# bioinfo-pf-curie/mpiBWA

Hardware: AMD Instinct MI355X
Metric: Mreads/s (whole node) 2x150 bp PE vs GRCh38-size reference; SAM bit-match (higher is better)
Workload: dtype int32

## Files before the change

include/mpibwa_amd.h:

```cpp
#ifndef MPIBWA_AMD_H
#define MPIBWA_AMD_H

#include <stdint.h>
#include <stddef.h>
#include <stdio.h>

#ifdef __cplusplus
extern "C" {
#endif

#define MEM_F_PE             0x2
#define MEM_F_NOPAIRING      0x4
#define MEM_F_ALL            0x8
#define MEM_F_NO_MULTI       0x10
#define MEM_F_NO_RESCUE      0x20
#define MEM_F_REF_HDR        0x100
#define MEM_F_SOFTCLIP       0x200
#define MEM_F_SMARTPE        0x400
#define MEM_F_PRIMARY5       0x800
#define MEM_F_KEEP_SUPP_MAPQ 0x1000

typedef uint64_t bwtint_t;

typedef struct {
	int a, b;
	int o_del, e_del;
	int o_ins, e_ins;
	int pen_unpaired;
	int pen_clip5, pen_clip3;
	int w;
	int zdrop;
	uint64_t max_mem_intv;
	int T;
	int flag;
	int min_seed_len;
	int min_chain_weight;
	int max_chain_extend;
	float split_factor;
	int split_width;
	int max_occ;
	int max_chain_gap;
	int n_threads;
	int chunk_size;
	float mask_level;
	float drop_ratio;
	float XA_drop_ratio;
	float mask_level_redun;
	float mapQ_coef_len;
	int mapQ_coef_fac;
	int max_ins;
	int max_matesw;
	int max_XA_hits, max_XA_hits_alt;
	int8_t mat[25];
} mem_opt_t;

typedef struct {
	int low, high;
	int failed;
	double avg, std;
} mem_pestat_t;

typedef struct {
	int l_seq, id;
	char *name, *comment, *seq, *qual, *sam;
} bseq1_t;

typedef struct {
	bwtint_t primary;
	bwtint_t L2[5];
	bwtint_t seq_len;
	bwtint_t bwt_size;
	uint32_t *bwt;
	uint32_t cnt_table[256];
	int sa_intv;
	bwtint_t n_sa;
	bwtint_t *sa;
} bwt_t;

typedef struct {
	int64_t offset;
	int32_t len;
	int32_t n_ambs;
	uint32_t gi;
	int32_t is_alt;
	char *name, *anno;
} bntann1_t;

typedef struct {
	int64_t offset;
	int32_t len;
	char amb;
} bntamb1_t;

typedef struct {
	int64_t l_pac;
	int32_t n_seqs;
	uint32_t seed;
	bntann1_t *anns;
	int32_t n_holes;
	bntamb1_t *ambs;
	FILE *fp_pac;
} bntseq_t;

typedef struct {
	bwt_t    *bwt;
	bntseq_t *bns;
	uint8_t  *pac;
	int       is_shm;
	int64_t   l_mem;
	uint8_t  *mem;
} bwaidx_t;

void mem_process_seqs(const mem_opt_t *opt, const bwt_t *bwt, const bntseq_t *bns, const uint8_t *pac,
                      int64_t n_processed, int n, bseq1_t *seqs, const mem_pestat_t *pes0);

mem_opt_t *mem_opt_init(void);
void bwa_fill_scmat(int a, int b, int8_t mat[25]);
extern int  bwa_verbose;
extern char bwa_rg_id[256];
char *bwa_set_rg(const char *s);
char *bwa_insert_header(const char *s, char *hdr);

bwaidx_t *bwa_idx_load_from_disk(const char *prefix, int which);
int       bwa_mem2idx(int64_t l_mem, uint8_t *mem, bwaidx_t *idx);
void      bwa_idx_destroy(bwaidx_t *idx);
int       bwa_idx2mem(bwaidx_t *idx);
int       mi355x_write_map(const char *prefix, const char *map_path);


int  mi355x_index_upload(int local_rank, const bwt_t *bwt, const bntseq_t *bns, const uint8_t *pac);
int  mi355x_index_alloc(int local_rank, const bwt_t *bwt_meta, const bntseq_t *bns);
int  mi355x_index_buffers(void **d_bwt, size_t *bwt_bytes, void **d_sa, size_t *sa_bytes, void **d_pac, size_t *pac_bytes);
int  mi355x_index_d2d(int which, void *ext_device_ptr, size_t bytes, int to_index);
int  mi355x_index_commit(void);
void mi355x_finalize(void);

typedef struct {
	int rank, size;
	void (*bcast)(void *buf, size_t bytes, int root, void *user);
	void *user;
} mi355x_comm_t;
int  mi355x_init(int local_rank, const bwaidx_t *idx, const mi355x_comm_t *comm);
int  mi355x_device_count(void);
int  mi355x_device_memory(size_t *free_bytes, size_t *total_bytes);
unsigned long long mi355x_buffer_growths(void);
int  mi355x_rank_host_threads(int *ranks_on_node);
int  mi355x_index_checksums(uint64_t out[3]);
int  mi355x_max_calls(void);
double mi355x_prewarm(const mem_opt_t *opt, const bwt_t *bwt, const bntseq_t *bns, const uint8_t *pac, int n_reads, int read_len, int n_calls);
double mi355x_init_bcast_seconds(void);

int  mi355x_index_build(const char *fasta, const char *prefix);
int  mi355x_index_build_gpu(int device, const uint8_t *pac, int64_t l_pac, const char *prefix, double *seconds);


int mi355x_smem_batch(const mem_opt_t *opt, int n, const uint8_t *seqs, const int64_t *off,
                      int cap, uint64_t *intv_out, int *n_out, double *kernel_ms, uint64_t *algo_bytes);
int mi355x_sa_batch(int n, const uint64_t *k, uint64_t *sa_out, double *kernel_ms, uint64_t *algo_bytes);
int mi355x_sa_batch2(int n, const uint64_t *k, uint64_t *sa_out, double *kernel_ms, int dense);
double mi355x_sa_dense_info(size_t *bytes);
int mi355x_extend_batch(const mem_opt_t *opt, int n, const uint8_t *q, const int64_t *qoff,
                        const uint8_t *t, const int64_t *toff, const int *w, const int *h0,
                        const int *end_bonus, int *out6, double *kernel_ms, uint64_t *cells);

int64_t mi355x_chain_batch(const mem_opt_t *opt, const bntseq_t *bns, int n_reads, const int *lens, const int *l_rep,
                           const int64_t *seed_off, const uint64_t *rbeg, const int32_t *qbeg_len, int which,
                           int64_t *out, int64_t out_cap, int64_t *out_off);

int64_t mi355x_c2a_batch(const mem_opt_t *opt, const bntseq_t *bns, int n_reads, const uint8_t *reads, const int64_t *off,
                         const int *n_chains, const int *chain_rid, const float *chain_frac, const int *chain_nseeds,
                         const int64_t *seed_rbeg, const int *seed_qbeg, const int *seed_len, const int *seed_score,
                         int heavy_t, int early, int layout, int64_t *out, int64_t out_cap, int64_t *out_off,
                         uint64_t *stat4, int *n_units);

int mi355x_global_batch(const mem_opt_t *opt, int64_t l_pac, const uint8_t *pac, int n_reads, const uint8_t *reads,
                        const int64_t *off, int n_req, const int64_t *rb, const int64_t *re, const int *read,
                        const int *qb, const int *qe, const int *w, const int *truesc, int which,
                        int *out_hdr5, uint32_t *cigar_out, int cigar_cap, char *md_out, int md_cap, double *kernel_ms);

int mi355x_pair_maxreg(void);
int mi355x_pair_batch(const mem_opt_t *opt, const bntseq_t *bns, const mem_pestat_t pes[4], int64_t n_processed, int n_pairs,
                      const void *regs, const int *n_regs, int max_len, uint8_t *status, void *desc, void *req);

int mi355x_pair_wave_maxreg(void);
int mi355x_pair_wave_batch(const mem_opt_t *opt, const bntseq_t *bns, const uint8_t *pac, const mem_pestat_t pes[4], int64_t n_processed,
                           int n_pairs, const uint8_t *reads, const int64_t *off, const void *regs, const int *reg_off, uint8_t *status,
                           void *desc, void *req, int *n_align);

int mi355x_pair_wave_xa_cap(void);
int mi355x_pair_wave_xa_batch(const mem_opt_t *opt, const bntseq_t *bns, const uint8_t *pac, const mem_pestat_t pes[4], int64_t n_processed,
                              int n_pairs, const uint8_t *reads, const int64_t *off, const void *regs, const int *reg_off, uint8_t *status,
                              void *desc, void *req, int *n_align, void *xa_req, uint8_t *xa_cnt);

size_t mi355x_sam_arena_bytes(int n_reads, int max_len);
int mi355x_sam_batch(const mem_opt_t *opt, const bntseq_t *bns, const uint8_t *pac, int n_pairs, const uint8_t *reads, const int64_t *off,
                     const uint8_t *quals, const char *names, const int *name_off, const void *desc, const void *reqs, const int *req_base,
                     size_t arena_bytes, int grid_blocks, int *out_len, unsigned long long *out_off, uint8_t *arena_out,
                     unsigned long long *cursor, void *hdr_out);

int mi355x_se_batch(const mem_opt_t *opt, const bntseq_t *bns, int64_t n_processed, int n_reads, const void *regs, const int *n_regs,
                    int max_len, uint8_t *status, void *desc, void *req);

int mi355x_sam_se_batch(const mem_opt_t *opt, const bntseq_t *bns, const uint8_t *pac, int n_reads, const uint8_t *reads, const int64_t *off,
                        const uint8_t *quals, const char *names, const int *name_off, const void *desc, const void *reqs, const int *req_base,
                        size_t arena_bytes, int grid_blocks, int *out_len, unsigned long long *out_off, uint8_t *arena_out,
                        unsigned long long *cursor, void *hdr_out);

int64_t mi355x_seed_batch(int n_reads, int cap, int max_occ, uint64_t *intv, const int *n_intv, int *n_seeds, int *l_rep,
                          int64_t *seed_off, uint64_t *rows, int32_t *qbeg_len, int64_t seed_cap);

int mi355x_matesw_batch(const mem_opt_t *opt, int64_t l_pac, const uint8_t *pac, int n_reads, const uint8_t *reads,
                        const int64_t *off, int n_req, const int64_t *rb, const int64_t *re, const int *read,
                        const int *is_rev, int *out8, double *kernel_ms);

int64_t mi355x_fastq_scan(const char *buf, int64_t len, int64_t cap, int64_t *rec_off, int32_t *rec_bases);
int64_t mi355x_fastq_chunks(const int32_t *bases1, const int32_t *bases2, int64_t n, int64_t maxsiz, int64_t cap,
                            int64_t *chunk_first);
int64_t mi355x_fastq_fill(char *buf1, const int64_t *off1, char *buf2, const int64_t *off2, int64_t first, int64_t count,
                          int copy_comment, int lockstep, bseq1_t *seqs);

typedef struct {
	double total_ms, h2d_ms, smem_ms, sa_ms, chain_ms, ext_ms, regs_ms, pestat_ms, sam_ms;
	double k_smem_ms, k_sa_ms, k_ext_ms;
	uint64_t smem_bytes, sa_bytes, ext_cells;
	uint64_t n_reads, n_intv, n_seeds, n_chains, n_ext;
	double plan_ms, aln_ms, k_aln_ms;
	uint64_t n_aln;
	double phase1_ms;
	double msw_ms, k_msw_ms;
	uint64_t n_msw;
	double emit_ms;
	uint64_t n_sub;
	uint64_t smem_tab_bytes;
	uint64_t n_sam_dev;
	uint64_t n_pair_dev;
	uint64_t n_se_dev;
	uint64_t n_pair_wave_dev;
	uint64_t n_pair_xa_dev;
} mi355x_stats_t;
void mi355x_last_stats(mi355x_stats_t *st);

void mi355x_host_ksw_align2(int qlen, const uint8_t *query, int tlen, const uint8_t *target, const int8_t *mat, int o_del,
                            int e_del, int o_ins, int e_ins, int xtra, int portable, int out7[7]);

int   mi355x_host_sam_pe(const mem_opt_t *opt, const bntseq_t *bns, const uint8_t *pac, const mem_pestat_t pes[4], uint64_t id, bseq1_t s[2],
                         const void *regs0, int n0, const void *regs1, int n1);
int   mi355x_host_sort_dedup_patch(const mem_opt_t *opt, const bntseq_t *bns, const uint8_t *pac, uint8_t *query, void *regs, int n);
void  mi355x_host_reg2sam_se(const mem_opt_t *opt, const bntseq_t *bns, const uint8_t *pac, bseq1_t *s, const void *regs, int n, int64_t id);
void  mi355x_host_pestat(const mem_opt_t *opt, int64_t l_pac, int n, const void *regs, const int *n_regs, mem_pestat_t pes[4], int n_threads);
void  mi355x_host_flt_chained_seeds(const mem_opt_t *opt, const bntseq_t *bns, const uint8_t *pac, int l_query, const uint8_t *query, int n_chains,
                                    void *seeds, int *n_seeds);

int   mi355x_host_cpus(void);
char *mi355x_collect_sam(bseq1_t *seqs, int n, size_t *total_len);
size_t mi355x_collect_sam_into(bseq1_t *seqs, int n, char **buf, size_t *cap);

int     mi355x_fixmate_pair(bseq1_t *s1, bseq1_t *s2, const bntseq_t *bns);
int64_t mi355x_fixmate(bseq1_t *seqs, int n, const bntseq_t *bns);
size_t  mi355x_bgzf_bound(size_t len);
size_t  mi355x_bgzf_compress(const char *text, size_t len, int level, uint8_t *out, size_t cap);
size_t  mi355x_bgzf_eof(uint8_t out[28]);
int64_t mi355x_route_by_chr(const char *sam, size_t len, const bntseq_t *bns, int discordant, char **out_text, size_t *out_len);

#ifdef __cplusplus
}
#endif
#endif
```

mpibwa_amd/api.py:

```python
import ctypes as C
import os

import numpy as np

from . import abi

HERE = os.path.dirname(os.path.abspath(__file__))
_LIB = None

libc = C.CDLL(None if os.environ.get("MPIBWA_SANITIZER_LIB") else "libc.so.6")
libc.free.argtypes = [C.c_void_p]

EXPORTS = [
    "mem_process_seqs", "mem_opt_init", "bwa_fill_scmat", "bwa_idx_load_from_disk", "bwa_mem2idx", "bwa_idx_destroy",
    "mi355x_index_upload", "mi355x_index_alloc", "mi355x_index_buffers", "mi355x_index_d2d", "mi355x_index_commit",
    "mi355x_finalize", "mi355x_index_build", "mi355x_index_build_gpu",
    "mi355x_smem_batch", "mi355x_sa_batch", "mi355x_sa_batch2", "mi355x_sa_dense_info", "mi355x_extend_batch", "mi355x_matesw_batch", "mi355x_chain_batch", "mi355x_c2a_batch", "mi355x_pair_batch", "mi355x_pair_maxreg", "mi355x_fastq_scan", "mi355x_fastq_chunks", "mi355x_fastq_fill", "mi355x_last_stats", "mi355x_host_cpus", "mi355x_collect_sam", "mi355x_collect_sam_into", "mi355x_host_ksw_align2",
    "bwa_set_rg", "bwa_insert_header", "bwa_idx2mem", "mi355x_write_map", "mi355x_init", "mi355x_rank_host_threads", "mi355x_index_checksums", "mi355x_init_bcast_seconds", "mi355x_global_batch", "mi355x_device_count", "mi355x_device_memory", "mi355x_buffer_growths", "mi355x_prewarm", "mi355x_max_calls",
    "mi355x_sam_batch", "mi355x_sam_arena_bytes", "mi355x_se_batch", "mi355x_sam_se_batch", "mi355x_seed_batch", "mi355x_pair_wave_batch", "mi355x_pair_wave_maxreg",
    "mi355x_pair_wave_xa_batch", "mi355x_pair_wave_xa_cap",
]


class mi355x_comm_t(C.Structure):
    BCAST = C.CFUNCTYPE(None, C.c_void_p, C.c_size_t, C.c_int, C.c_void_p)
    _fields_ = [("rank", C.c_int), ("size", C.c_int), ("bcast", BCAST), ("user", C.c_void_p)]



def load_library(build_if_missing=True):
    global _LIB
    if _LIB is not None:
        return _LIB
    path = os.path.join(HERE, "libmpibwa_amd.so")
    host_only = os.environ.get("MPIBWA_SANITIZER_LIB")
    if host_only:
        path = host_only
    if not os.path.exists(path):
        if not build_if_missing or host_only:
            raise RuntimeError("%s is missing: run python -m mpibwa_amd.build" % path)
        from .build import build
        build()
    lib = C.CDLL(path)
    P = C.POINTER

    def sig(name, restype, argtypes):
        try:
            fn = getattr(lib, name)
        except AttributeError:
            if host_only:
                return
            raise
        fn.restype = restype
        fn.argtypes = argtypes

    sig("mem_opt_init", P(abi.mem_opt_t), [])
    sig("bwa_idx_load_from_disk", P(abi.bwaidx_t), [C.c_char_p, C.c_int])
    sig("mi355x_index_build", C.c_int, [C.c_char_p, C.c_char_p])
    sig("mi355x_index_build_gpu", C.c_int, [C.c_int, C.c_void_p, C.c_int64, C.c_char_p, P(C.c_double)])
    sig("mem_process_seqs", None, [P(abi.mem_opt_t), P(abi.bwt_t), P(abi.bntseq_t), P(C.c_uint8), C.c_int64, C.c_int,
                                   P(abi.bseq1_t), P(abi.mem_pestat_t)])
    sig("mi355x_index_upload", C.c_int, [C.c_int, P(abi.bwt_t), P(abi.bntseq_t), P(C.c_uint8)])
    sig("mi355x_index_alloc", C.c_int, [C.c_int, P(abi.bwt_t), P(abi.bntseq_t)])
    sig("mi355x_index_buffers", C.c_int, [P(C.c_void_p), P(C.c_size_t)] * 3)
    sig("mi355x_index_d2d", C.c_int, [C.c_int, C.c_void_p, C.c_size_t, C.c_int])
    sig("mi355x_index_commit", C.c_int, [])
    sig("mi355x_smem_batch", C.c_int, [P(abi.mem_opt_t), C.c_int, C.c_void_p, C.c_void_p, C.c_int, C.c_void_p,
                                       C.c_void_p, P(C.c_double), P(C.c_uint64)])
    sig("mi355x_sa_batch", C.c_int, [C.c_int, C.c_void_p, C.c_void_p, P(C.c_double), P(C.c_uint64)])
    sig("mi355x_sa_batch2", C.c_int, [C.c_int, C.c_void_p, C.c_void_p, P(C.c_double), C.c_int])
    sig("mi355x_sa_dense_info", C.c_double, [P(C.c_size_t)])
    sig("mi355x_extend_batch", C.c_int, [P(abi.mem_opt_t), C.c_int] + [C.c_void_p] * 8 + [P(C.c_double), P(C.c_uint64)])
    sig("mi355x_chain_batch", C.c_int64, [P(abi.mem_opt_t), C.c_void_p, C.c_int] + [C.c_void_p] * 5 + [C.c_int, C.c_void_p, C.c_int64, C.c_void_p])
    sig("mi355x_c2a_batch", C.c_int64, [P(abi.mem_opt_t), C.c_void_p, C.c_int] + [C.c_void_p] * 10 + [C.c_int] * 3 +
        [C.c_void_p, C.c_int64, C.c_void_p, C.c_void_p, C.c_void_p])
    sig("mi355x_fastq_scan", C.c_int64, [C.c_void_p, C.c_int64, C.c_int64, C.c_void_p, C.c_void_p])
    sig("mi355x_fastq_chunks", C.c_int64, [C.c_void_p, C.c_void_p, C.c_int64, C.c_int64, C.c_int64, C.c_void_p])
    sig("mi355x_fastq_fill", C.c_int64, [C.c_void_p, C.c_void_p, C.c_void_p, C.c_void_p, C.c_int64, C.c_int64, C.c_int, C.c_int, C.c_void_p])
    sig("mi355x_matesw_batch", C.c_int, [P(abi.mem_opt_t), C.c_int64, C.c_void_p, C.c_int, C.c_void_p, C.c_void_p, C.c_int] + [C.c_void_p] * 5 + [P(C.c_double)])
    sig("mi355x_last_stats", None, [P(abi.mi355x_stats_t)])
    sig("mi355x_finalize", None, [])
    sig("mi355x_host_ksw_align2", None, [C.c_int, C.c_void_p, C.c_int, C.c_void_p, C.c_void_p] + [C.c_int] * 6 + [C.c_void_p])
    sig("mi355x_host_cpus", C.c_int, [])
    sig("mi355x_host_sort_dedup_patch", C.c_int, [P(abi.mem_opt_t), P(abi.bntseq_t), C.c_void_p, C.c_void_p, C.c_void_p, C.c_int])
    sig("mi355x_host_reg2sam_se", None, [P(abi.mem_opt_t), P(abi.bntseq_t), C.c_void_p, P(abi.bseq1_t), C.c_void_p, C.c_int, C.c_int64])
    sig("mi355x_host_pestat", None, [P(abi.mem_opt_t), C.c_int64, C.c_int, C.c_void_p, C.c_void_p, C.c_void_p, C.c_int])
    sig("mi355x_host_flt_chained_seeds", None, [P(abi.mem_opt_t), P(abi.bntseq_t), C.c_void_p, C.c_int, C.c_void_p, C.c_int, C.c_void_p, C.c_void_p])
    sig("mi355x_host_sam_pe", C.c_int, [P(abi.mem_opt_t), P(abi.bntseq_t), C.c_void_p, C.c_void_p, C.c_uint64, P(abi.bseq1_t), C.c_void_p, C.c_int, C.c_void_p, C.c_int])
    sig("mi355x_collect_sam", C.c_void_p, [P(abi.bseq1_t), C.c_int, P(C.c_size_t)])
    sig("mi355x_fixmate_pair", C.c_int, [P(abi.bseq1_t), P(abi.bseq1_t), P(abi.bntseq_t)])
    sig("mi355x_fixmate", C.c_int64, [P(abi.bseq1_t), C.c_int, P(abi.bntseq_t)])
    sig("mi355x_bgzf_bound", C.c_size_t, [C.c_size_t])
    sig("mi355x_bgzf_compress", C.c_size_t, [C.c_char_p, C.c_size_t, C.c_int, C.c_void_p, C.c_size_t])
    sig("mi355x_bgzf_eof", C.c_size_t, [C.c_void_p])
    sig("mi355x_route_by_chr", C.c_int64, [C.c_char_p, C.c_size_t, P(abi.bntseq_t), C.c_int, P(C.c_void_p), P(C.c_size_t)])
    sig("bwa_set_rg", C.c_void_p, [C.c_char_p])
    sig("bwa_insert_header", C.c_void_p, [C.c_char_p, C.c_void_p])
    sig("bwa_idx2mem", C.c_int, [P(abi.bwaidx_t)])
    sig("bwa_mem2idx", C.c_int, [C.c_int64, C.c_void_p, P(abi.bwaidx_t)])
    sig("bwa_idx_destroy", None, [P(abi.bwaidx_t)])
    sig("mi355x_write_map", C.c_int, [C.c_char_p, C.c_char_p])
    sig("mi355x_init", C.c_int, [C.c_int, P(abi.bwaidx_t), P(mi355x_comm_t)])
    sig("mi355x_init_bcast_seconds", C.c_double, [])
    sig("mi355x_index_checksums", C.c_int, [C.c_void_p])
    sig("mi355x_device_count", C.c_int, [])
    sig("mi355x_device_memory", C.c_int, [P(C.c_size_t), P(C.c_size_t)])
    sig("mi355x_buffer_growths", C.c_ulonglong, [])
    sig("mi355x_pair_batch", C.c_int, [P(abi.mem_opt_t), C.c_void_p, C.c_void_p, C.c_int64, C.c_int, C.c_void_p, C.c_void_p, C.c_int, C.c_void_p, C.c_void_p, C.c_void_p])
    sig("mi355x_pair_wave_maxreg", C.c_int, [])
    sig("mi355x_pair_wave_batch", C.c_int, [P(abi.mem_opt_t), C.c_void_p, C.c_void_p, C.c_void_p, C.c_int64, C.c_int] + [C.c_void_p] * 8)
    sig("mi355x_pair_wave_xa_cap", C.c_int, [])
    sig("mi355x_pair_wave_xa_batch", C.c_int, [P(abi.mem_opt_t), C.c_void_p, C.c_void_p, C.c_void_p, C.c_int64, C.c_int] + [C.c_void_p] * 10)
    sig("mi355x_global_batch", C.c_int, [P(abi.mem_opt_t), C.c_int64, C.c_void_p, C.c_int, C.c_void_p, C.c_void_p, C.c_int] + [C.c_void_p] * 7 +
        [C.c_int, C.c_void_p, C.c_void_p, C.c_int, C.c_void_p, C.c_int, P(C.c_double)])
    sig("mi355x_sam_arena_bytes", C.c_size_t, [C.c_int, C.c_int])
    sig("mi355x_sam_batch", C.c_int, [P(abi.mem_opt_t), C.c_void_p, C.c_void_p, C.c_int] + [C.c_void_p] * 8 + [C.c_size_t, C.c_int] + [C.c_void_p] * 5)
    sig("mi355x_sam_se_batch", C.c_int, [P(abi.mem_opt_t), C.c_void_p, C.c_void_p, C.c_int] + [C.c_void_p] * 8 + [C.c_size_t, C.c_int] + [C.c_void_p] * 5)
    sig("mi355x_se_batch", C.c_int, [P(abi.mem_opt_t), C.c_void_p, C.c_int64, C.c_int, C.c_void_p, C.c_void_p, C.c_int, C.c_void_p, C.c_void_p, C.c_void_p])
    sig("mi355x_seed_batch", C.c_int64, [C.c_int, C.c_int, C.c_int] + [C.c_void_p] * 7 + [C.c_int64])
    _LIB = lib
    return lib


_HIP = None


def _hip():
    global _HIP
    if _HIP is None:
        _HIP = C.CDLL("libamdhip64.so")
        _HIP.hipMemcpy.argtypes = [C.c_void_p, C.c_void_p, C.c_size_t, C.c_int]
    return _HIP


def build_index(fasta, prefix):
    lib = load_library()
    if lib.mi355x_index_build(fasta.encode(), prefix.encode()) != 0:
        raise RuntimeError("index build failed")


class Engine:

    def __init__(self, prefix, device=0, upload=True, dist=None, rank=0, map_path=None, comm=None):
        self.lib = load_library()
        if map_path is not None:
            import numpy as np
            self._map = np.fromfile(map_path, dtype=np.uint8)
            self._idx_obj = abi.bwaidx_t()
            self.lib.bwa_mem2idx(len(self._map), self._map.ctypes.data, C.byref(self._idx_obj))
            self.idx = C.pointer(self._idx_obj)
        else:
            self.idx = self.lib.bwa_idx_load_from_disk(prefix.encode(), 7)
        self.bwt = self.idx.contents.bwt
        self.bns = self.idx.contents.bns
        self.pac = self.idx.contents.pac
        self.uploaded = False
        self.bcast_seconds = None
        if upload and comm is not None:
            if self.lib.mi355x_init(device, self.idx, C.byref(comm)) != 0:
                raise RuntimeError("mi355x_init failed")
            self.uploaded = True
            self.bcast_seconds = self.lib.mi355x_init_bcast_seconds()
        elif upload and dist is None:
            if self.lib.mi355x_index_upload(device, self.bwt, self.bns, self.pac) != 0:
                raise RuntimeError("mi355x_index_upload failed")
            self.uploaded = True
        elif upload:
            self._upload_by_broadcast(device, dist, rank)

    def _upload_by_broadcast(self, device, dist, rank):
        import time
        import torch
        os.environ["MPIBWA_SA_DENSE"] = os.environ.get("MPIBWA_SA_DENSE", "1")
        if self.lib.mi355x_index_alloc(device, self.bwt, self.bns) != 0:
            raise RuntimeError("mi355x_index_alloc failed")
        pv = [C.c_void_p() for _ in range(3)]
        sv = [C.c_size_t() for _ in range(3)]
        self.lib.mi355x_index_buffers(C.byref(pv[0]), C.byref(sv[0]), C.byref(pv[1]), C.byref(sv[1]), C.byref(pv[2]), C.byref(sv[2]))
        if rank == 0:
            HIP = _hip()
            srcs = [(C.cast(self.bwt.contents.bwt, C.c_void_p), int(self.bwt.contents.bwt_size) * 4),
                    (C.cast(self.bwt.contents.sa, C.c_void_p), int(self.bwt.contents.n_sa) * 8),
                    (C.cast(self.pac, C.c_void_p), int(self.bns.contents.l_pac) // 4 + 1)]
            for which, (src, nbytes) in enumerate(srcs):
                if HIP.hipMemcpy(C.c_void_p(pv[which].value), src, C.c_size_t(nbytes), 1) != 0:
                    raise RuntimeError("hipMemcpy H2D failed")

        class _DevView:
            def __init__(self, ptr, nbytes):
                self.__cuda_array_interface__ = {"data": (ptr, False), "shape": (nbytes,), "typestr": "|u1", "version": 2}
        t0 = time.time()
        piece = int(os.environ.get("MPIBWA_BCAST_PIECE_MB", "256")) << 20
        views = []
        for which in range(3):
            v = torch.as_tensor(_DevView(pv[which].value, sv[which].value), device="cuda:%d" % device)
            views.append(v)
            for off in range(0, sv[which].value, piece):
                dist.broadcast(v[off:off + piece], src=0)
        torch.cuda.synchronize(device)
        self.bcast_seconds = time.time() - t0
        del views
        mine = (C.c_uint64 * 3)()
        if self.lib.mi355x_index_checksums(mine) != 0:
            raise RuntimeError("mi355x_index_checksums failed")
        self.index_checksums = [int(x) for x in mine]
        objs = [self.index_checksums if rank == 0 else None]
        dist.broadcast_object_list(objs, src=0)
        if objs[0] != self.index_checksums:
            raise RuntimeError("rank %d received a damaged index by broadcast: checksums %s, rank 0 sent %s" % (rank, self.index_checksums, objs[0]))
        if self.lib.mi355x_index_commit() != 0:
            raise RuntimeError("mi355x_index_commit failed")
        self.uploaded = True

    def opt(self, **kw):
        o = self.lib.mem_opt_init()
        for k, v in kw.items():
            setattr(o.contents, k, v)
        return o

    def process(self, opt, reads, n_processed=0, pes0=None, with_qual=True, comment=None):
        batch = abi.SeqBatch(libc, reads, with_qual=with_qual, comment=comment)
        self.lib.mem_process_seqs(opt, self.bwt, self.bns, self.pac, n_processed, batch.n, batch.arr, pes0)
        return batch.take_sam()

    def prewarm(self, opt, n_reads, read_len=150, n_calls=1):
        self.lib.mi355x_prewarm.restype = C.c_double
        self.lib.mi355x_prewarm.argtypes = [C.c_void_p, C.c_void_p, C.c_void_p, C.c_void_p, C.c_int, C.c_int, C.c_int]
        as_p = lambda x: C.cast(x, C.c_void_p)
        return float(self.lib.mi355x_prewarm(as_p(opt), as_p(self.bwt), as_p(self.bns), as_p(self.pac), int(n_reads), int(read_len), int(n_calls)))

    def process_batch(self, opt, batch, n_processed=0, pes0=None):
        self.lib.mem_process_seqs(opt, self.bwt, self.bns, self.pac, n_processed, batch.n, batch.arr, pes0)

    def collect_sam(self, batch):
        n = C.c_size_t(0)
        p = self.lib.mi355x_collect_sam(batch.arr, batch.n, C.byref(n))
        out = C.string_at(p, n.value)
        libc.free(C.c_void_p(p))
        return out

    def stats(self):
        st = abi.mi355x_stats_t()
        self.lib.mi355x_last_stats(C.byref(st))
        return {k: getattr(st, k) for k, _ in st._fields_}

    def smem(self, opt, seqs, cap=256):
        off = np.zeros(len(seqs) + 1, dtype=np.int64)
        off[1:] = np.cumsum([len(s) for s in seqs])
        flat = np.concatenate(seqs).astype(np.uint8) if len(seqs) else np.zeros(0, np.uint8)
        out = np.zeros((len(seqs), cap, 4), dtype=np.uint64)
        cnt = np.zeros(len(seqs), dtype=np.int32)
        ms = C.c_double(0)
        nbytes = C.c_uint64(0)
        rc = self.lib.mi355x_smem_batch(opt, len(seqs), flat.ctypes.data, off.ctypes.data, cap, out.ctypes.data,
                                        cnt.ctypes.data, C.byref(ms), C.byref(nbytes))
        if rc != 0:
            raise RuntimeError("mi355x_smem_batch overflowed cap=%d" % cap)
        return [out[i, :cnt[i]].copy() for i in range(len(seqs))], ms.value, nbytes.value

    def sa(self, ks):
        ks = np.ascontiguousarray(ks, dtype=np.uint64)
        out = np.zeros(len(ks), dtype=np.uint64)
        ms = C.c_double(0)
        nbytes = C.c_uint64(0)
        self.lib.mi355x_sa_batch(len(ks), ks.ctypes.data, out.ctypes.data, C.byref(ms), C.byref(nbytes))
        return out, ms.value, nbytes.value

    def sa_dense(self, ks):
        ks = np.ascontiguousarray(ks, dtype=np.uint64)
        out = np.zeros(len(ks), dtype=np.uint64)
        ms = C.c_double(0)
        rc = self.lib.mi355x_sa_batch2(len(ks), ks.ctypes.data, out.ctypes.data, C.byref(ms), 1)
        return (out, ms.value) if rc == 0 else None

    def chains(self, opt, lens, l_rep, seeds_per_read, which):
        n = len(seeds_per_read)
        off = np.zeros(n + 1, dtype=np.int64)
        off[1:] = np.cumsum([len(s) for s in seeds_per_read])
        S = int(off[n])
        rbeg = np.zeros(max(S, 1), dtype=np.uint64)
        ql = np.zeros(2 * max(S, 1), dtype=np.int32)
        k = 0
        for s in seeds_per_read:
            for rb, qb, ln in s:
                rbeg[k] = rb; ql[2 * k] = qb; ql[2 * k + 1] = ln
                k += 1
        lens = np.ascontiguousarray(lens, dtype=np.int32)
        l_rep = np.ascontiguousarray(l_rep, dtype=np.int32)
        cap = n + 16 * S + 64 * n + 64
        out = np.zeros(cap, dtype=np.int64)
        out_off = np.zeros(n + 1, dtype=np.int64)
        rc = self.lib.mi355x_chain_batch(opt, C.cast(self.bns, C.c_void_p), n, lens.ctypes.data, l_rep.ctypes.data, off.ctypes.data, rbeg.ctypes.data,
                                         ql.ctypes.data, which, out.ctypes.data, cap, out_off.ctypes.data)
        assert rc >= 0
        res = []
        for r in range(n):
            p = int(out_off[r])
            nc = int(out[p]); p += 1
            if nc < 0:
                res.append(None)
                continue
            chs = []
            for _ in range(nc):
                rid, ns, fb, fe, r0, r1, fr = (int(x) for x in out[p:p + 7]); p += 7
                sd = [tuple(int(x) for x in out[p + 3 * j:p + 3 * j + 3]) for j in range(ns)]
                p += 3 * ns
                chs.append((rid, fb, fe, r0, r1, fr, sd))
            res.append(chs)
        return res

    C2A_FIELDS = ("rb", "re", "qb", "qe", "rid", "score", "truesc", "w", "seedcov", "seedlen0", "frac_rep")

    def chain2aln(self, opt, reads, chains, heavy_t=8, early=1, layout=0):
        n = len(reads)
        off = np.zeros(n + 1, dtype=np.int64)
        off[1:] = np.cumsum([len(r) for r in reads])
        flat = np.concatenate([np.asarray(r, dtype=np.uint8) for r in reads]) if n else np.zeros(0, np.uint8)
        flat = np.ascontiguousarray(np.append(flat, np.zeros(1, np.uint8)))
        n_chains = np.array([len(c) for c in chains], dtype=np.int32)
        ch = [c for per in chains for c in per]
        rid = np.array([c[0] for c in ch] or [0], dtype=np.int32)
        frac = np.array([c[1] for c in ch] or [0], dtype=np.float32)
        nsd = np.array([len(c[2]) for c in ch] or [0], dtype=np.int32)
        sd = np.array([s for c in ch for s in c[2]] or [(0, 0, 0, 0)], dtype=np.int64).reshape(-1, 4)
        rbeg = np.ascontiguousarray(sd[:, 0])
        qbeg, ln, sc = (np.ascontiguousarray(sd[:, k], dtype=np.int32) for k in (1, 2, 3))
        cap = n + 11 * max(int(nsd.sum()), 1) + 64
        out = np.zeros(cap, dtype=np.int64)
        out_off = np.zeros(n + 1, dtype=np.int64)
        stat = np.zeros(4, dtype=np.uint64)
        units = C.c_int(0)
        rc = self.lib.mi355x_c2a_batch(opt, C.cast(self.bns, C.c_void_p), n, flat.ctypes.data, off.ctypes.data, n_chains.ctypes.data, rid.ctypes.data,
                                       frac.ctypes.data, nsd.ctypes.data, rbeg.ctypes.data, qbeg.ctypes.data, ln.ctypes.data, sc.ctypes.data,
                                       int(heavy_t), int(early), int(layout), out.ctypes.data, cap, out_off.ctypes.data, stat.ctypes.data, C.addressof(units))
        assert rc >= 0
        res = []
        for r in range(n):
            p = int(out_off[r])
            m = int(out[p])
            res.append(out[p + 1:p + 1 + 11 * m].reshape(m, 11).copy())
        st = dict(zip(("cells", "n_ext", "n_closed", "n_diff"), (int(x) for x in stat)))
        return res, st, units.value

    REG_DT = np.dtype([("rb", "<i8"), ("re", "<i8"), ("qb", "<i4"), ("qe", "<i4"), ("rid", "<i4"), ("score", "<i4"), ("truesc", "<i4"), ("w", "<i4"),
                       ("seedcov", "<i4"), ("seedlen0", "<i4"), ("frac_rep", "<f4"), ("pad", "<i4")])
    DESC_DT = np.dtype([("rb", "<i8"), ("re", "<i8"), ("qb", "<i4"), ("qe", "<i4"), ("req", "<i4"), ("rid", "<i4"), ("flag", "<i4"), ("mapq", "<i4"),
                        ("score", "<i4"), ("sub", "<i4")])
    AREQ_DT = np.dtype([("rb", "<i8"), ("re", "<i8"), ("read", "<i4"), ("qb", "<i4"), ("qe", "<i4"), ("w2", "<i4"), ("truesc", "<i4"), ("pad", "<i4")])

    def pairs(self, opt, pes, regs, n_regs, max_len=150, n_processed=0):
        regs = np.ascontiguousarray(regs, dtype=self.REG_DT)
        assert regs.shape[1] == self.lib.mi355x_pair_maxreg()
        n_regs = np.ascontiguousarray(n_regs, dtype=np.int32)
        n_pairs = len(n_regs) // 2
        status = np.zeros(n_pairs, dtype=np.uint8)
        desc = np.zeros(2 * n_pairs, dtype=self.DESC_DT)
        req = np.zeros(2 * n_pairs, dtype=self.AREQ_DT)
        rc = self.lib.mi355x_pair_batch(opt, C.cast(self.bns, C.c_void_p), C.cast(pes, C.c_void_p), n_processed, n_pairs, regs.ctypes.data, n_regs.ctypes.data,
                                        max_len, status.ctypes.data, desc.ctypes.data, req.ctypes.data)
        if rc != 0:
            raise RuntimeError("mi355x_pair_batch: the kernel cannot use these insert-size statistics")
        return status, desc, req

    PW_DECIDED_XA = 16

    def pairs_wave_xa(self, opt, pes, reads, regs, n_processed=0):
        return self.pairs_wave(opt, pes, reads, regs, n_processed, xa=True)

    def pairs_wave(self, opt, pes, reads, regs, n_processed=0, xa=False):
        n = len(reads)
        assert n % 2 == 0 and len(regs) == n
        n_pairs = n // 2
        off = np.zeros(n + 1, dtype=np.int64)
        off[1:] = np.cumsum([len(r) for r in reads])
        flat = np.ascontiguousarray(np.concatenate([np.asarray(r, dtype=np.uint8) for r in reads])) if n else np.zeros(1, dtype=np.uint8)
        reg_off = np.zeros(n + 1, dtype=np.int32)
        reg_off[1:] = np.cumsum([len(r) for r in regs])
        allregs = np.zeros(max(1, int(reg_off[-1])), dtype=self.REG_DT)
        for r, a in enumerate(regs):
            allregs[reg_off[r]:reg_off[r + 1]] = np.asarray(a, dtype=self.REG_DT)
        status = np.zeros(n_pairs, dtype=np.uint8)
        desc = np.zeros(n, dtype=self.DESC_DT)
        req = np.zeros(n, dtype=self.AREQ_DT)
        n_align = C.c_int(0)
        args = (opt, C.cast(self.bns, C.c_void_p), C.cast(self.pac, C.c_void_p), C.cast(pes, C.c_void_p), n_processed, n_pairs,
                flat.ctypes.data, off.ctypes.data, allregs.ctypes.data, reg_off.ctypes.data, status.ctypes.data,
                desc.ctypes.data, req.ctypes.data, C.cast(C.byref(n_align), C.c_void_p))
        if xa:
            cap = self.lib.mi355x_pair_wave_xa_cap()
            xa_req = np.zeros((max(n, 1), cap), dtype=self.AREQ_DT)
            xa_cnt = np.zeros(max(n, 1), dtype=np.uint8)
            rc = self.lib.mi355x_pair_wave_xa_batch(*args, xa_req.ctypes.data, xa_cnt.ctypes.data)
        else:
            rc = self.lib.mi355x_pair_wave_batch(*args)
        if rc != 0:
            raise RuntimeError("mi355x_pair_wave_batch: the kernel cannot use these insert-size statistics")
        if xa:
            return status, desc, req, [xa_req[r, :xa_cnt[r]].copy() for r in range(n)], n_align.value
        return status, desc, req, n_align.value

    def singles(self, opt, regs, n_regs, max_len=150, n_processed=0):
        regs = np.ascontiguousarray(regs, dtype=self.REG_DT)
        assert regs.shape[1] == self.lib.mi355x_pair_maxreg()
        n_regs = np.ascontiguousarray(n_regs, dtype=np.int32)
        n = len(n_regs)
        assert regs.shape[0] == n
        status = np.zeros(n, dtype=np.uint8)
        desc = np.zeros(n, dtype=self.DESC_DT)
        req = np.zeros(n, dtype=self.AREQ_DT)
        rc = self.lib.mi355x_se_batch(opt, C.cast(self.bns, C.c_void_p), n_processed, n, regs.ctypes.data, n_regs.ctypes.data, max_len,
                                      status.ctypes.data, desc.ctypes.data, req.ctypes.data)
        assert rc == 0
        return status, desc, req

    HDR_DT = np.dtype([("score", "<i4"), ("NM", "<i4"), ("n_cigar", "<i4"), ("md_len", "<i4"), ("pool_off", "<u4"), ("flags", "<i4")])
    SAM_GUARD = 4096
    SAM_GUARD_BYTE = 0xA5

    def sam_records_se(self, opt, reads, quals, names, desc, reqs, req_base, arena_bytes=0, grid_blocks=0):
        return self.sam_records(opt, reads, quals, names, desc, reqs, req_base, arena_bytes, grid_blocks, ends=1)

    def sam_records(self, opt, reads, quals, names, desc, reqs, req_base, arena_bytes=0, grid_blocks=0, ends=2):
        n = len(reads)
        assert n % ends == 0 and len(names) == n and len(desc) == n and len(req_base) == n // ends + 1
        off = np.zeros(n + 1, dtype=np.int64)
        off[1:] = np.cumsum([len(r) for r in reads])
        flat = np.ascontiguousarray(np.concatenate([np.asarray(r, dtype=np.uint8) for r in reads]))
        fq = None
        if quals is not None:
            fq = np.frombuffer(b"".join(quals), dtype=np.uint8)
            assert len(fq) == len(flat)
        noff = np.zeros(n + 1, dtype=np.int32)
        noff[1:] = np.cumsum([len(x) for x in names])
        nm = np.frombuffer(b"".join(names) + b"\0", dtype=np.uint8)
        desc = np.ascontiguousarray(desc, dtype=self.DESC_DT)
        reqs = np.ascontiguousarray(reqs, dtype=self.AREQ_DT)
        req_base = np.ascontiguousarray(req_base, dtype=np.int32)
        assert int(req_base[-1]) == len(reqs)
        if not arena_bytes:
            arena_bytes = int(self.lib.mi355x_sam_arena_bytes(n, max(len(r) for r in reads)))
        out_len = np.zeros(n, dtype=np.int32)
        out_off = np.zeros(n, dtype=np.uint64)
        arena = np.zeros(arena_bytes + self.SAM_GUARD, dtype=np.uint8)
        cursor = np.zeros(1, dtype=np.uint64)
        hdr = np.zeros(max(len(reqs), 1), dtype=self.HDR_DT)
        fn = self.lib.mi355x_sam_batch if ends == 2 else self.lib.mi355x_sam_se_batch
        rc = fn(opt, C.cast(self.bns, C.c_void_p), C.cast(self.pac, C.c_void_p), n // ends, flat.ctypes.data, off.ctypes.data,
                                       fq.ctypes.data if fq is not None else None, nm.ctypes.data, noff.ctypes.data, desc.ctypes.data,
                                       reqs.ctypes.data if len(reqs) else None, req_base.ctypes.data, arena_bytes, int(grid_blocks), out_len.ctypes.data,
                                       out_off.ctypes.data, arena.ctypes.data, cursor.ctypes.data, hdr.ctypes.data)
        assert rc == 0
        return {"out_len": out_len, "out_off": out_off, "arena": arena[:arena_bytes], "guard": arena[arena_bytes:], "arena_bytes": arena_bytes,
                "cursor": int(cursor[0]), "hdr": hdr[:len(reqs)]}

    def seeds(self, intervals, cap, max_occ):
        n = len(intervals)
        iv = np.zeros((n, cap, 4), dtype=np.uint64)
        cnt = np.zeros(n, dtype=np.int32)
        for r, a in enumerate(intervals):
            a = np.asarray(a, dtype=np.uint64).reshape(-1, 4)
            cnt[r] = len(a)
            iv[r, :min(len(a), cap)] = a[:cap]
        most = int(sum(min(int(s), max_occ) for r in range(n) for s in iv[r, :min(cnt[r], cap), 2]))
        n_seeds = np.zeros(n, dtype=np.int32)
        l_rep = np.zeros(n, dtype=np.int32)
        seed_off = np.zeros(n + 1, dtype=np.int64)
        rows = np.zeros(most + 1, dtype=np.uint64)
        qbl = np.zeros((most + 1, 2), dtype=np.int32)
        S = int(self.lib.mi355x_seed_batch(n, cap, max_occ, iv.ctypes.data, cnt.ctypes.data, n_seeds.ctypes.data, l_rep.ctypes.data,
                                           seed_off.ctypes.data, rows.ctypes.data, qbl.ctypes.data, most))
        if S < 0:
            raise RuntimeError("mi355x_seed_batch: the kernel counts %d seeds, the intervals allow %d" % (-1 - S, most))
        per = [(rows[seed_off[r]:seed_off[r + 1]].copy(), qbl[seed_off[r]:seed_off[r + 1]].copy()) for r in range(n)]
        return [iv[r, :min(cnt[r], cap)].copy() for r in range(n)], n_seeds, l_rep, per

    def matesw(self, opt, l_pac, pac, reads, rb, re, read, is_rev):
        n = len(reads)
        off = np.zeros(n + 1, dtype=np.int64)
        off[1:] = np.cumsum([len(s) for s in reads])
        flat = np.concatenate(reads).astype(np.uint8)
        rb = np.ascontiguousarray(rb, dtype=np.int64)
        re = np.ascontiguousarray(re, dtype=np.int64)
        read = np.ascontiguousarray(read, dtype=np.int32)
        is_rev = np.ascontiguousarray(is_rev, dtype=np.int32)
        pac = np.ascontiguousarray(pac, dtype=np.uint8)
        out = np.zeros((len(rb), 8), dtype=np.int32)
        ms = C.c_double(0)
        self.lib.mi355x_matesw_batch(opt, int(l_pac), pac.ctypes.data, n, flat.ctypes.data, off.ctypes.data, len(rb), rb.ctypes.data,
                                     re.ctypes.data, read.ctypes.data, is_rev.ctypes.data, out.ctypes.data, C.byref(ms))
        return out, ms.value

    def global_align(self, opt, l_pac, pac, reads, rb, re, read, qb, qe, w, truesc, which=0, cigar_cap=128, md_cap=800):
        n = len(reads)
        off = np.zeros(n + 1, dtype=np.int64)
        off[1:] = np.cumsum([len(s) for s in reads])
        flat = np.concatenate(reads).astype(np.uint8)
        arr = lambda x, t: np.ascontiguousarray(x, dtype=t)
        rb, re = arr(rb, np.int64), arr(re, np.int64)
        read, qb, qe, w, truesc = (arr(x, np.int32) for x in (read, qb, qe, w, truesc))
        pac = arr(pac, np.uint8)
        nr = len(rb)
        hdr = np.zeros((nr, 5), dtype=np.int32)
        cig = np.zeros((nr, cigar_cap), dtype=np.uint32)
        md = np.zeros((nr, md_cap), dtype=np.uint8)
        ms = C.c_double(0)
        rc = self.lib.mi355x_global_batch(opt, int(l_pac), pac.ctypes.data, n, flat.ctypes.data, off.ctypes.data, nr, rb.ctypes.data,
                                          re.ctypes.data, read.ctypes.data, qb.ctypes.data, qe.ctypes.data, w.ctypes.data,
                                          truesc.ctypes.data, which, hdr.ctypes.data, cig.ctypes.data, cigar_cap, md.ctypes.data, md_cap,
                                          C.byref(ms))
        if rc != 0:
            raise RuntimeError("mi355x_global_batch: result beyond cigar_cap / md_cap")
        cigs = [cig[i, :hdr[i, 2]].copy() for i in range(nr)]
        mds = [md[i, :hdr[i, 3]].tobytes() for i in range(nr)]
        return hdr, cigs, mds, ms.value

    def extend(self, opt, qs, ts, w, h0, end_bonus):
        n = len(qs)
        qoff = np.zeros(n + 1, dtype=np.int64)
        qoff[1:] = np.cumsum([len(s) for s in qs])
        toff = np.zeros(n + 1, dtype=np.int64)
        toff[1:] = np.cumsum([len(s) for s in ts])
        qf = np.concatenate(qs).astype(np.uint8)
        tf = np.concatenate(ts).astype(np.uint8)
        w = np.ascontiguousarray(w, dtype=np.int32)
        h0 = np.ascontiguousarray(h0, dtype=np.int32)
        eb = np.ascontiguousarray(end_bonus, dtype=np.int32)
        out = np.zeros((n, 6), dtype=np.int32)
        ms = C.c_double(0)
        cells = C.c_uint64(0)
        self.lib.mi355x_extend_batch(opt, n, qf.ctypes.data, qoff.ctypes.data, tf.ctypes.data, toff.ctypes.data,
                                     w.ctypes.data, h0.ctypes.data, eb.ctypes.data, out.ctypes.data, C.byref(ms),
                                     C.byref(cells))
        return out, ms.value, cells.value
```

mpibwa_amd/csrc/aln_kernel.hip:

```cpp
#include <hip/hip_runtime.h>
#include <algorithm>
#include "device.h"
#include "wave_ext.cuh"

namespace mbw {

#define ALN_WAVES 1
__host__ __device__ inline int aln_zcap(int max_len) { int z = 80 * (max_len + 32); z = (z + 255) & ~255; return z < 12288 ? 12288 : z; }
__host__ __device__ inline int aln_zcap_small(int max_len) { int z = 32 * (max_len + 32); return (z + 255) & ~255; }
#define ALN_MDCAP 768
#define ALN_CIGCAP 96
#define ALN_NEG (-0x40000000)

__device__ __forceinline__ int wave_sum_int(int v)
{
	for (int o = 32; o > 0; o >>= 1) v += __shfl_xor(v, o);
	return v;
}

struct AlnLds {
	int *H, *E, *dummy;
	uint8_t *q, *t, *z, *md;
	uint32_t *cig;
};
// ... 43 lines not shown
		unsigned long long base = 0;
		if ((threadIdx.x & 63) == __ffsll((long long)m) - 1) base = atomicAdd(&counters[ALN_CNT + kind], (unsigned long long)__popcll(m));
		base = __shfl(base, __ffsll((long long)m) - 1);
		if (mine) lists[(size_t)kind * n_req + base + __popcll(m & below)] = rq;
	}
}

template <int KIND>
__device__ __forceinline__ void aln_one(int rq, const AlnParams &P, const WxParams &X, int n_req, const AlnReq *__restrict__ reqs,
                                        const uint8_t *__restrict__ seq, const int64_t *__restrict__ off, const uint8_t *__restrict__ pac,
                                        const int *__restrict__ gaptab, AlnHdr *__restrict__ hdr, uint8_t *__restrict__ pool,
                                        unsigned long long *counters, unsigned long long pool_bytes, int max_len, int tcap, int *lists, int dp_kind,
                                        unsigned long long &slab_at, unsigned &slab_left)
{
	extern __shared__ int lds_raw[];
	const int wave = threadIdx.x >> 6, lane = threadIdx.x & 63;
	constexpr bool FAST = KIND == 0;
	const int ALN_ZCAP = KIND == 1 ? aln_zcap_small(max_len) : aln_zcap(max_len);
	AlnLds L;
	if (FAST) {
		const size_t per_wave = (size_t)2 * ((max_len + 3) & ~3) + ALN_MDCAP + 16;
		uint8_t *base = (uint8_t *)lds_raw + (size_t)wave * per_wave;
		L.H = L.E = L.dummy = nullptr; L.z = nullptr;
		L.cig = (uint32_t *)base;
		L.q = base + 16;
		L.t = L.q + ((max_len + 3) & ~3);
		L.md = L.t + ((max_len + 3) & ~3);
	} else {
		const size_t per_wave = (size_t)2 * (max_len + 2 + ALN_PAD) * 4 + 4 + ((max_len + 3) & ~3) + ((tcap + 3) & ~3) + ALN_ZCAP + ALN_MDCAP + ALN_CIGCAP * 4;
		uint8_t *base = (uint8_t *)lds_raw + (size_t)wave * per_wave;
		L.H = (int *)base; L.E = L.H + (max_len + 2 + ALN_PAD);
		L.dummy = L.E + (max_len + 2 + ALN_PAD);
		L.cig = (uint32_t *)(L.dummy + 1);
		L.q = (uint8_t *)(L.cig + ALN_CIGCAP);
		L.t = L.q + ((max_len + 3) & ~3);
		L.z = L.t + ((tcap + 3) & ~3);
		L.md = L.z + ALN_ZCAP;
	}

	AlnReq R = reqs[rq];
	if (KIND != 0) {
		const unsigned long long rb = (unsigned long long)R.rb, re = (unsigned long long)R.re;
		R.rb = (int64_t)((unsigned long long)(unsigned)__builtin_amdgcn_readfirstlane((int)(rb >> 32)) << 32 |
		                 (unsigned)__builtin_amdgcn_readfirstlane((int)rb));
		R.re = (int64_t)((unsigned long long)(unsigned)__builtin_amdgcn_readfirstlane((int)(re >> 32)) << 32 |
		                 (unsigned)__builtin_amdgcn_readfirstlane((int)re));
		R.read = __builtin_amdgcn_readfirstlane(R.read); R.qb = __builtin_amdgcn_readfirstlane(R.qb);
		R.qe = __builtin_amdgcn_readfirstlane(R.qe); R.w2 = __builtin_amdgcn_readfirstlane(R.w2);
		R.truesc = __builtin_amdgcn_readfirstlane(R.truesc);
	}
	const int lq = R.qe - R.qb;
	const long long rlen64 = R.re - R.rb;
	AlnHdr out;
	out.score = 0; out.NM = -1; out.n_cigar = 0; out.md_len = 0; out.pool_off = 0; out.flags = 0;
	const bool invalid = aln_invalid(P, R, max_len, tcap);
	if (invalid) {
		out.flags = 1;
		if (lane == 0) hdr[rq] = out;
		return;
	}
	const int rlen = (int)rlen64;
	const bool rev = R.rb >= P.l_pac;
	const uint8_t *rd = seq + off[R.read];
	for (int j = lane; j < lq; j += 64) L.q[j] = rev ? rd[R.qe - 1 - j] : rd[R.qb + j];
	{
		const long long f0 = rev ? (P.l_pac << 1) - R.re : R.rb;
		for (int i = lane; i < rlen; i += 64) {
			long long f = f0 + i;
			int b = (pac[f >> 2] >> ((~f & 3) << 1)) & 3;
			L.t[i] = rev ? 3 - b : b;
		}
	}
	__builtin_amdgcn_wave_barrier();

	const int oe_del = X.o_del + X.e_del, oe_ins = X.o_ins + X.e_ins, e_del = X.e_del, e_ins = X.e_ins;
	uint32_t plo[5], phi[5];
#pragma unroll
	for (int t = 0; t < 5; ++t) {
		plo[t] = (uint32_t)(uint8_t)X.mat[t * 5] | (uint32_t)(uint8_t)X.mat[t * 5 + 1] << 8 | (uint32_t)(uint8_t)X.mat[t * 5 + 2] << 16 |
		         (uint32_t)(uint8_t)X.mat[t * 5 + 3] << 24;
		phi[t] = (uint32_t)(uint8_t)X.mat[t * 5 + 4];
	}
	const int wmax4 = P.w << 2;
	int w2 = R.w2, last_sc = -(1 << 30), score = 0, n_cig = 0;
	bool fallback = false;
	for (int it = 0;; ) {
		w2 = w2 < wmax4 ? w2 : wmax4;
		if (FAST) {
			int s = 0;
			for (int i = lane; i < lq; i += 64) s += X.mat[L.t[i] * 5 + L.q[i]];
			score = wave_sum_int(s);
			if (w2 != 0) {
				int amax = X.mat[0];
				for (int k = 1; k < 25; ++k) amax = X.mat[k] > amax ? X.mat[k] : amax;
				if (amax <= 0 || (long long)lq * amax - score > (long long)amax + oe_del + oe_ins) {
					if (lane == 0) lists[(size_t)dp_kind * n_req + atomicAdd(&counters[ALN_CNT + dp_kind], 1ull)] = rq;
					return;
				}
			}
			n_cig = 1;
			if (lane == 0) L.cig[0] = (uint32_t)lq << 4;
			__builtin_amdgcn_fence(__ATOMIC_RELEASE, "wavefront");
			__builtin_amdgcn_wave_barrier();
			__builtin_amdgcn_fence(__ATOMIC_ACQUIRE, "wavefront");
			break;
		} else {
			int d_len = rlen - lq; d_len = d_len < 0 ? -d_len : d_len;
			int w = (gaptab[lq] + d_len + 1) >> 1;
			w = w < w2 ? w : w2;
			const int min_w = d_len + 3;
			w = w > min_w ? w : min_w;
			const int n_col = lq < 2 * w + 1 ? lq : 2 * w + 1;
			if ((long long)n_col * rlen > ALN_ZCAP) { fallback = true; break; }
			for (int j = lane; j <= lq; j += 64) {
				L.H[j] = j == 0 ? 0 : (j <= w ? -(X.o_ins + e_ins * j) : ALN_NEG);
				L.E[j] = ALN_NEG;
			}
			__builtin_amdgcn_wave_barrier();
			int vslo = 0, vshi = 0;
			for (int i = 0; i < rlen; ++i) {
				if ((i & 63) == 0) {
					const int tb = i + lane < rlen ? (int)L.t[i + lane] : 4;
					vslo = (int)(tb == 0 ? plo[0] : tb == 1 ? plo[1] : tb == 2 ? plo[2] : tb == 3 ? plo[3] : plo[4]);
					vshi = (int)(tb == 0 ? phi[0] : tb == 1 ? phi[1] : tb == 2 ? phi[2] : tb == 3 ? phi[3] : phi[4]);
				}
				const uint32_t slo = (uint32_t)__builtin_amdgcn_readlane(vslo, i & 63), shi = (uint32_t)__builtin_amdgcn_readlane(vshi, i & 63);
				const int beg = i > w ? i - w : 0, end = i + w + 1 < lq ? i + w + 1 : lq;
				const int hleft0 = beg == 0 ? -(X.o_del + e_del * (i + 1)) : ALN_NEG;
				const int n_row = end - beg;
				int A = ALN_NEG;
				int h_carry = hleft0;
				uint8_t *zi = L.z + (size_t)i * n_col;
				for (int s0 = 0; s0 <= n_row; s0 += 64) {
					const int j = beg + s0 + lane;
					const bool act = s0 + lane < n_row, wr = s0 + lane <= n_row;
					const int diag = L.H[j], e = L.E[j];
					const int qraw = (int)L.q[j];
					const int qb = act ? qraw : 4;
					const int sc = (int)(int8_t)__builtin_amdgcn_perm(shi, slo, (uint32_t)qb | 0x0c0c0c00u);
					const int m = diag + sc;
					const int g = act ? m - oe_ins + j * e_ins : ALN_NEG - (1 << 28);
					const int incl = wx_scan_max(g);
					const int excl = wx_dpp<0x138, 0xf>(ALN_NEG - (1 << 28), incl);
					const int f = max(A, excl + e_ins) - j * e_ins;
					uint8_t d = m >= e ? 0 : 1;
					int h = m >= e ? m : e;
					if (h < f) { d = 2; h = f; }
					int t = m - oe_del;
					int e2 = e - e_del;
					if (e2 > t) d |= 1 << 2; else e2 = t;
					t = m - oe_ins;
					if (f - e_ins > t) d |= 2 << 4;
					const int h_prev = wx_dpp<0x138, 0xf>(h_carry, h);
					(wr ? L.H + j : L.dummy)[0] = h_prev;
					(wr ? L.E + j : L.dummy)[0] = act ? e2 : ALN_NEG;
					(act ? zi + (j - beg) : (uint8_t *)L.dummy)[0] = d;
					A = max(A, __builtin_amdgcn_readlane(incl, 63) + e_ins);
					h_carry = __builtin_amdgcn_readlane(h, 63);
				}
				if (n_row < 0 && lane == 0) { L.H[end] = hleft0; L.E[end] = ALN_NEG; }
				__builtin_amdgcn_wave_barrier();
			}
			score = L.H[lq];
			{
				int which = 0, i = rlen - 1, k = (i + w + 1 < lq ? i + w + 1 : lq) - 1, n = 0;
				uint32_t cur = 0;
				bool ovf = false;
				auto push = [&](uint32_t op, uint32_t len) {
					if (cur && (cur & 0xf) == op) cur += len << 4;
					else {
						if (cur) { if (n < ALN_CIGCAP) { if (lane == 0) L.cig[n] = cur; } else ovf = true; ++n; }
						cur = len << 4 | op;
					}
				};
				while (i >= 0 && k >= 0) {
					which = __builtin_amdgcn_readfirstlane((int)L.z[(size_t)i * n_col + (k - (i > w ? i - w : 0))]) >> (which << 1) & 3;
					if (which == 0) { push(0, 1); --i; --k; }
					else if (which == 1) { push(2, 1); --i; }
					else { push(1, 1); --k; }
				}
				if (i >= 0) push(2, i + 1);
				if (k >= 0) push(1, k + 1);
				if (cur) { if (n < ALN_CIGCAP) { if (lane == 0) L.cig[n] = cur; } else ovf = true; ++n; }
				if (ovf) { fallback = true; break; }
				__builtin_amdgcn_wave_barrier();
				for (int a = lane; a < n / 2; a += 64) { uint32_t x = L.cig[a]; L.cig[a] = L.cig[n - 1 - a]; L.cig[n - 1 - a] = x; }
				__builtin_amdgcn_wave_barrier();
				n_cig = n;
			}
		}
		if (score == last_sc || w2 == wmax4) break;
		last_sc = score;
		w2 <<= 1;
		if (!(++it < 3 && score < R.truesc - P.a)) break;
	}
	if (fallback) {
		if (KIND == 1) {
			if (lane == 0) lists[(size_t)2 * n_req + atomicAdd(&counters[ALN_CNT + 2], 1ull)] = rq;
			return;
		}
		out.flags = 1;
		if (lane == 0) hdr[rq] = out;
		return;
	}
	int md_len = 0, n_mm = 0, n_gap = 0;
	{
		const char *int2base = rev ? "TGCAN" : "ACGTN";
		int x = 0, y = 0, u = 0;
		for (int k = 0; k < n_cig; ++k) {
			const uint32_t c = L.cig[k];
			const int op = c & 0xf, len = (int)(c >> 4);
			if (op == 0) {
				for (int i0 = 0; i0 < len; i0 += 64) {
					const int i = i0 + lane;
					unsigned long long mm = __ballot(i < len && L.q[x + i] != L.t[y + i]);
					int cur = 0;
					const int chunk = len - i0 < 64 ? len - i0 : 64;
					while (mm) {
						const int p = __ffsll((long long)mm) - 1;
						mm &= mm - 1;
						u += p - cur;
						md_len = put_num(L.md, md_len, u, lane);
						if (lane == 0 && md_len < ALN_MDCAP) L.md[md_len] = int2base[L.t[y + i0 + p]];
						++md_len; ++n_mm; u = 0; cur = p + 1;
					}
					u += chunk - cur;
				}
				x += len; y += len;
			} else if (op == 2) {
				if (k > 0 && k < n_cig - 1) {
					md_len = put_num(L.md, md_len, u, lane);
					if (lane == 0 && md_len < ALN_MDCAP) L.md[md_len] = '^';
					++md_len;
					for (int i = lane; i < len; i += 64)
						if (md_len + i < ALN_MDCAP) L.md[md_len + i] = int2base[L.t[y + i]];
					md_len += len;
					u = 0; n_gap += len;
				}
				y += len;
			} else { x += len; n_gap += len; }
		}
		md_len = put_num(L.md, md_len, u, lane);
	}
	if (md_len > ALN_MDCAP) {
		out.flags = 1;
		if (lane == 0) hdr[rq] = out;
		return;
	}
	__builtin_amdgcn_wave_barrier();
	const unsigned need = (unsigned)n_cig * 4 + (((unsigned)md_len + 3) & ~3u);
	unsigned long long at = 0;
	if (need <= slab_left) { at = slab_at; slab_at += need; slab_left -= need; }
	else {
		const unsigned take = need > ALN_SLAB ? need : ALN_SLAB;
		if (lane == 0) at = atomicAdd(&counters[0], (unsigned long long)take);
		at = __shfl(at, 0);
		slab_at = at + need; slab_left = take - need;
	}
	if (at + need > pool_bytes) {
		out.flags = 1;
		if (lane == 0) hdr[rq] = out;
		return;
	}
	uint32_t *pc = (uint32_t *)(pool + at);
	for (int k = lane; k < n_cig; k += 64) pc[k] = L.cig[k];
	uint8_t *pm = pool + at + (size_t)n_cig * 4;
	for (int k = lane; k < md_len; k += 64) pm[k] = L.md[k];
	out.score = score; out.NM = n_mm + n_gap; out.n_cigar = n_cig; out.md_len = md_len; out.pool_off = (uint32_t)(at >> 2); out.flags = 0;
	if (lane == 0) hdr[rq] = out;
}

template <int KIND>
__global__ void __launch_bounds__(64 * ALN_WAVES)
aln_kernel(AlnParams P, WxParams X, int n_req, const AlnReq *__restrict__ reqs, const uint8_t *__restrict__ seq,
           const int64_t *__restrict__ off, const uint8_t *__restrict__ pac, const int *__restrict__ gaptab, AlnHdr *__restrict__ hdr,
           uint8_t *__restrict__ pool, unsigned long long *counters, unsigned long long pool_bytes, int max_len, int tcap, int *lists, int dp_kind)
{
	const int wave = threadIdx.x >> 6;
	const int n = (int)counters[ALN_CNT + KIND];
	const int *mine = lists + (size_t)KIND * n_req;
	unsigned long long slab_at = 0;
	unsigned slab_left = 0;
	for (int k = blockIdx.x * ALN_WAVES + wave; k < n; k += gridDim.x * ALN_WAVES) {
		aln_one<KIND>(KIND != 0 ? __builtin_amdgcn_readfirstlane(mine[k]) : mine[k], P, X, n_req, reqs, seq, off, pac, gaptab, hdr, pool, counters, pool_bytes, max_len, tcap, lists, dp_kind,
		              slab_at, slab_left);
		__builtin_amdgcn_fence(__ATOMIC_RELEASE, "wavefront");
		__builtin_amdgcn_wave_barrier();
		__builtin_amdgcn_fence(__ATOMIC_ACQUIRE, "wavefront");
	}
}

size_t aln_lds_per_block(int max_len, int tcap)
{
	const int ALN_ZCAP = aln_zcap(max_len);
	size_t per_wave = (size_t)2 * (max_len + 2 + ALN_PAD) * 4 + 4 + ((max_len + 3) & ~3) + ((tcap + 3) & ~3) + ALN_ZCAP + ALN_MDCAP + ALN_CIGCAP * 4;
	return per_wave * ALN_WAVES;
}

void launch_aln(void *stream, const AlnParams &P, const ExtParams &ep, int n_req, const AlnReq *d_req, const uint8_t *d_seq,
                const int64_t *d_off, const uint8_t *d_pac, const int *d_gaptab, AlnHdr *d_hdr, uint8_t *d_pool,
                unsigned long long *d_counters, size_t pool_bytes, int max_len, int tcap, int *d_lists, bool wide_only)
{
	if (n_req <= 0) return;
	WxParams X;
	for (int i = 0; i < 25; ++i) X.mat[i] = ep.mat[i];
	X.o_del = ep.o_del; X.e_del = ep.e_del; X.o_ins = ep.o_ins; X.e_ins = ep.e_ins; X.zdrop = ep.zdrop;
	const size_t shmem = aln_lds_per_block(max_len, tcap);
	const size_t shmem_small = shmem - (size_t)(aln_zcap(max_len) - aln_zcap_small(max_len)) * ALN_WAVES;
	const size_t shmem_fast = ((size_t)2 * ((max_len + 3) & ~3) + ALN_MDCAP + 16) * ALN_WAVES;
	if (shmem > 64 * 1024 && hipFuncSetAttribute((const void *)aln_kernel<2>, hipFuncAttributeMaxDynamicSharedMemorySize, (int)shmem) != hipSuccess)
		die("aln_kernel: cannot reserve %zu bytes of LDS", shmem);
	if (shmem_small > 64 * 1024 && hipFuncSetAttribute((const void *)aln_kernel<1>, hipFuncAttributeMaxDynamicSharedMemorySize, (int)shmem_small) != hipSuccess)
		die("aln_kernel: cannot reserve %zu bytes of LDS", shmem_small);
	if (shmem_fast > 64 * 1024) die("aln_kernel: reads of %d bp do not fit the LDS staging buffers", max_len);
	static int s_cus = 0;
	if (!s_cus) {
		int dev = 0;
		hipDeviceProp_t prop;
		if (hipGetDevice(&dev) != hipSuccess || hipGetDeviceProperties(&prop, dev) != hipSuccess) die("aln_kernel: cannot query the device");
		s_cus = prop.multiProcessorCount > 0 ? prop.multiProcessorCount : 256;
	}
	auto grid_for = [&](size_t lds) {
		long long per_cu = (long long)(160 * 1024 / std::max<size_t>(lds, 1));
		per_cu = std::max(1ll, std::min(per_cu, 32ll / ALN_WAVES));
		return dim3((unsigned)std::min<long long>((long long)s_cus * per_cu * 2, ((long long)n_req + ALN_WAVES - 1) / ALN_WAVES));
	};
	const dim3 block(64 * ALN_WAVES);
	hipStream_t st = (hipStream_t)stream;
	hipLaunchKernelGGL(aln_classify_kernel, dim3((n_req + 255) / 256), dim3(256), 0, st, P, n_req, d_req, max_len, tcap, d_lists, d_counters,
	                   wide_only ? 2 : 1);
	hipLaunchKernelGGL(aln_kernel<0>, grid_for(shmem_fast), block, shmem_fast, st, P, X, n_req, d_req, d_seq, d_off, d_pac, d_gaptab, d_hdr, d_pool,
	                   d_counters, (unsigned long long)pool_bytes, max_len, tcap, d_lists, wide_only ? 2 : 1);
	hipLaunchKernelGGL(aln_kernel<1>, grid_for(shmem_small), block, shmem_small, st, P, X, n_req, d_req, d_seq, d_off, d_pac, d_gaptab, d_hdr, d_pool,
	                   d_counters, (unsigned long long)pool_bytes, max_len, tcap, d_lists, wide_only ? 2 : 1);
	hipLaunchKernelGGL(aln_kernel<2>, grid_for(shmem), block, shmem, st, P, X, n_req, d_req, d_seq, d_off, d_pac, d_gaptab, d_hdr, d_pool,
	                   d_counters, (unsigned long long)pool_bytes, max_len, tcap, d_lists, wide_only ? 2 : 1);
	if (hipGetLastError() != hipSuccess) die("aln_kernel: launch failed");
}

}
```

mpibwa_amd/csrc/c2a_kernel.hip:

```cpp
#include <hip/hip_runtime.h>
#include "device.h"
#include "wave_ext.cuh"

namespace mbw {

typedef long long i64;

__device__ __forceinline__ i64 wave_min_i64(i64 v)
{
	for (int o = 32; o > 0; o >>= 1) { i64 t = __shfl_xor(v, o); v = t < v ? t : v; }
	return v;
}
__device__ __forceinline__ i64 wave_max_i64(i64 v)
{
	for (int o = 32; o > 0; o >>= 1) { i64 t = __shfl_xor(v, o); v = t > v ? t : v; }
	return v;
}
__device__ __forceinline__ int wave_sum_i32(int v)
{
	for (int o = 32; o > 0; o >>= 1) v += __shfl_xor(v, o);
	return v;
}

__device__ __forceinline__ int ref_base(const uint8_t *pac, i64 l_pac, i64 p)
{
	if (p >= l_pac) {
		i64 f = (l_pac << 1) - 1 - p;
		return 3 - ((pac[f >> 2] >> ((~f & 3) << 1)) & 3);
	}
	return (pac[p >> 2] >> ((~p & 3) << 1)) & 3;
}

__device__ __forceinline__ int uni(int v) { return __builtin_amdgcn_readfirstlane(v); }
__device__ __forceinline__ i64 uni64(i64 v)
{
	const unsigned long long u = (unsigned long long)v;
	return (i64)((unsigned long long)(unsigned)__builtin_amdgcn_readfirstlane((int)(u >> 32)) << 32 | (unsigned)__builtin_amdgcn_readfirstlane((int)u));
}

#define C2A_WAVES 1
#define SRT_MARK 0xFFFFFFFFu

#define C2A_CAP_C 8
#define C2A_CAP_S 64
#define C2A_CAP_R 8
__host__ __device__ inline int c2a_win_cap(int max_len) { return (3 * max_len + 128 + 15) & ~15; }
__host__ __device__ inline size_t c2a_lds_bytes(int max_len)
{
	return (((size_t)wx_lds_ints(max_len) * 4 + 15) & ~(size_t)15) + ((max_len + 15) & ~15) + C2A_CAP_C * sizeof(DevChain) + C2A_CAP_S * (sizeof(DevSeed) + 4) +
	       C2A_CAP_R * sizeof(DevReg) + c2a_win_cap(max_len);
}

__global__ void __launch_bounds__(64 * C2A_WAVES)
c2a_kernel(C2aParams P, WxParams X, int n_reads, const uint8_t *__restrict__ seq, const int64_t *__restrict__ off,
           const int *__restrict__ lens, const int *__restrict__ chain_beg, const int *__restrict__ chain_cnt, const DevChain *__restrict__ chains,
           const DevSeed *__restrict__ seeds, unsigned int *srt, const int *__restrict__ reg_beg, DevReg *regs, int *n_regs, const int *__restrict__ tab,
           int tab_stride, const uint8_t *__restrict__ pac, unsigned long long *counters, int max_len, const int *__restrict__ order, C2aUnits U)
{
	extern __shared__ int lds[];
	const int wave = threadIdx.x >> 6, lane = threadIdx.x & 63;
	int slot = blockIdx.x * C2A_WAVES + wave;
	const bool unit_mode = slot < U.max_units;
	int u_beg = 0, u_cnt = 0, u_av = 0;
	int rd;
	if (unit_mode) {
		if ((unsigned)slot >= *U.n_units) return;
		u_beg = uni(U.ustart[slot]); u_cnt = uni(U.ustart[slot + 1]) - u_beg;
		rd = uni(U.unit_rd[slot]); u_av = uni(U.unit_av[slot]);
	} else {
		slot -= U.max_units;
		if (slot >= n_reads) return;
		rd = uni(order ? order[slot] : slot);
		if (U.max_units > 0 && chain_cnt[rd] > U.heavy_t) return;
	}
	uint8_t *const lbase = (uint8_t *)lds + (size_t)wave * c2a_lds_bytes(max_len);
	const WxLds L = wx_lds((int *)lbase, max_len);
	uint8_t *const rdl = lbase + (((size_t)wx_lds_ints(max_len) * 4 + 15) & ~(size_t)15);
	DevChain *const chl = (DevChain *)(rdl + ((max_len + 15) & ~15));
	DevSeed *const sdl = (DevSeed *)(chl + C2A_CAP_C);
	unsigned int *const ordl = (unsigned int *)(sdl + C2A_CAP_S);
	DevReg *const avl = (DevReg *)(ordl + C2A_CAP_S);
	uint8_t *const winl = (uint8_t *)(avl + C2A_CAP_R);
	const int win_cap = c2a_win_cap(max_len);
	const int *gap = tab, *bound5 = tab + tab_stride, *bound3 = tab + 2 * tab_stride, *ceil95 = tab + 3 * tab_stride,
	          *thr10 = tab + 4 * tab_stride;
	const uint8_t *qg = seq + off[rd];
	const int lq = uni(lens[rd]);
	DevReg *av = regs + (unit_mode ? u_av : reg_beg[rd]);
	const int ci_beg = unit_mode ? 0 : uni(chain_beg[rd]), ci_cnt = unit_mode ? u_cnt : uni(chain_cnt[rd]);
	const int ci_end = ci_beg + (ci_cnt > 0 ? ci_cnt : 0);
	auto CI = [&](int t) -> int { return unit_mode ? uni(U.clist[u_beg + t]) : t; };
	for (int j = lane * 4; j < lq; j += 256) *(uint32_t *)(rdl + j) = *(const uint32_t *)(qg + j);
	const bool st_c = ci_cnt > 0 && ci_cnt <= C2A_CAP_C;
	if (st_c) {
		if (unit_mode) {
			const int W = (int)(sizeof(DevChain) / 4);
			for (int k = lane; k < ci_cnt * W; k += 64) ((uint32_t *)chl)[k] = ((const uint32_t *)(chains + U.clist[u_beg + k / W]))[k % W];
		} else
			for (int k = lane; k < ci_cnt * (int)(sizeof(DevChain) / 4); k += 64) ((uint32_t *)chl)[k] = ((const uint32_t *)(chains + ci_beg))[k];
	}
	__builtin_amdgcn_fence(__ATOMIC_RELEASE, "wavefront");
	__builtin_amdgcn_wave_barrier();
	__builtin_amdgcn_fence(__ATOMIC_ACQUIRE, "wavefront");
	const uint8_t *q = rdl;
	int s0 = 0, n_tot = 0;
	bool st_s = false;
	if (st_c) {
		s0 = uni(chl[0].seed_beg);
		int sum = 0;
		bool contiguous = true;
		for (int k = 0; k < ci_cnt; ++k) {
			const int sb = uni(chl[k].seed_beg), sn = uni(chl[k].n_seeds);
			contiguous = contiguous && sb == s0 + sum;
			sum += sn;
		}
		n_tot = sum;
		st_s = contiguous && n_tot <= C2A_CAP_S;
		if (st_s && lane < n_tot) { sdl[lane] = seeds[s0 + lane]; ordl[lane] = srt[s0 + lane]; }
		__builtin_amdgcn_fence(__ATOMIC_RELEASE, "wavefront");
		__builtin_amdgcn_wave_barrier();
		__builtin_amdgcn_fence(__ATOMIC_ACQUIRE, "wavefront");
	}
	int nav = 0;
	unsigned long long cells = 0, n_ext = 0, n_diff = 0, n_closed = 0;
	const i64 l_pac = P.l_pac;
	int max_sc = 1;
	for (int t = 0; t < 25; ++t) max_sc = X.mat[t] > max_sc ? X.mat[t] : max_sc;

	const int sc_a = X.mat[0], sc_b = -X.mat[1];
	bool plain = sc_a > 0 && sc_b > 0;
	for (int i = 0; i < 4; ++i)
		for (int j = 0; j < 4; ++j) plain = plain && X.mat[i * 5 + j] == (i == j ? sc_a : -sc_b);
	const int g1 = (X.o_del < X.o_ins ? X.o_del : X.o_ins) + (X.e_del < X.e_ins ? X.e_del : X.e_ins);
	auto ungapped = [&](int qlen, int tlen, auto tf, int h0, WxResult &r) -> bool {
		if (!plain || tlen < qlen || qlen <= 0) return false;
		int mm = 0, p = -1;
		bool bad = false;
		for (int j0 = 0; j0 < qlen && !bad && mm <= 1; j0 += 64) {
			const int j = j0 + lane;
			int qb = 0, tb = 0;
			if (j < qlen) { qb = (int)L.Qs[j]; tb = (int)tf(j); }
			bad = __ballot(qb > 3 || tb > 3) != 0;
			const unsigned long long mis = __ballot(qb != tb);
			if (mis) {
				if (p < 0) p = j0 + __ffsll((long long)mis) - 1;
				mm += __popcll(mis);
			}
		}
		if (bad || mm > 1) return false;
		if (mm == 1 && !(sc_a + sc_b < g1 && h0 > sc_b && (X.zdrop <= 0 || sc_a + sc_b <= X.zdrop))) return false;
		const int end = h0 + sc_a * qlen - (mm ? sc_a + sc_b : 0);
		int best = h0, bl = 0;
		if (mm == 0) { best = end; bl = qlen; }
		else {
			if (p > 0) { best = h0 + sc_a * p; bl = p; }
			if (end > best) { best = end; bl = qlen; }
		}
		r.score = best; r.qle = bl; r.tle = bl; r.gtle = qlen; r.gscore = end; r.max_off = 0;
		return true;
	};

	auto extend = [&](int qlen, auto qf, int tlen, auto tf, int wc, int h0, int clip) -> WxResult {
		++n_ext;
		for (int j = lane; j < qlen; j += 64) L.Qs[j] = (uint8_t)qf(j);
		__builtin_amdgcn_wave_barrier();
		if (P.early == 0) return wave_extend<false>(qlen, tlen, tf, X, wc, h0, L, cells, max_sc);
		WxResult r;
		const bool closed = ungapped(qlen, tlen, tf, h0, r);
		if (closed) ++n_closed;
		else r = wave_extend<true>(qlen, tlen, tf, X, wc, h0, L, cells, max_sc, clip);
		if (P.early == 2) {
			unsigned long long c2 = 0;
			const WxResult f = wave_extend<false>(qlen, tlen, tf, X, wc, h0, L, c2, max_sc);
			const bool loc_r = r.gscore <= 0 || r.gscore <= r.score - clip, loc_f = f.gscore <= 0 || f.gscore <= f.score - clip;
			bool same = f.score == r.score && f.qle == r.qle && f.tle == r.tle && f.max_off == r.max_off && loc_r == loc_f;
			if (same && (!loc_f || closed)) same = f.gtle == r.gtle && f.gscore == r.gscore;
			if (!same) ++n_diff;
		}
		return r;
	};

	for (int ct = ci_beg; ct < ci_end; ++ct) {
		const int ci = CI(ct);
		DevChain C = st_c ? chl[ct - ci_beg] : chains[ci];
		C.n_seeds = uni(C.n_seeds); C.seed_beg = uni(C.seed_beg); C.rid = uni(C.rid);
		C.far_beg = uni64(C.far_beg); C.far_end = uni64(C.far_end);
		const int n = C.n_seeds;
		const int nav0 = nav;
		if (unit_mode && lane == 0) { U.c_rabs[ci] = u_av + nav0; U.c_rcnt[ci] = 0; }
		if (n == 0) continue;
		const DevSeed *sdg = seeds + C.seed_beg;
		unsigned int *ordg = srt + C.seed_beg;
		int sl = C.seed_beg - s0;
		bool st_sc = st_s;
		if (unit_mode && !st_s && n <= C2A_CAP_S) {
			if (lane < n) { sdl[lane] = sdg[lane]; ordl[lane] = ordg[lane]; }
			__builtin_amdgcn_fence(__ATOMIC_RELEASE, "wavefront");
			__builtin_amdgcn_wave_barrier();
			__builtin_amdgcn_fence(__ATOMIC_ACQUIRE, "wavefront");
			st_sc = true; sl = 0;
		}
		auto SD = [&](int i) -> DevSeed { return st_sc ? sdl[sl + i] : sdg[i]; };
		auto ORD = [&](int i) -> unsigned int { return st_sc ? ordl[sl + i] : ordg[i]; };
		const i64 rmax0 = uni64(C.rmax0), rmax1 = uni64(C.rmax1);
		const int wlen = (int)(rmax1 - rmax0);
		const bool st_w = wlen <= win_cap;
		if (st_w) {
			for (int t = lane; t < wlen; t += 64) winl[t] = (uint8_t)ref_base(pac, l_pac, rmax0 + t);
			__builtin_amdgcn_fence(__ATOMIC_RELEASE, "wavefront");
			__builtin_amdgcn_wave_barrier();
			__builtin_amdgcn_fence(__ATOMIC_ACQUIRE, "wavefront");
		}
		auto TB = [&](i64 pos) -> int { return st_w ? (int)winl[pos - rmax0] : ref_base(pac, l_pac, pos); };

		for (int k = n - 1; k >= 0; --k) {
			DevSeed s = SD(uni((int)ORD(k)));
			s.rbeg = uni64(s.rbeg); s.qbeg = uni(s.qbeg); s.len = uni(s.len);
			bool hit = false;
			for (int i0 = 0; i0 < nav && !hit; i0 += 64) {
				int i = i0 + lane;
				bool h = false;
				if (i < nav) {
					const DevReg p = i < C2A_CAP_R ? avl[i] : av[i];
					if (!(s.rbeg < p.rb || s.rbeg + s.len > p.re || s.qbeg < p.qb || s.qbeg + s.len > p.qe) &&
					    !(s.len - p.seedlen0 > thr10[lq])) {
						int qd = s.qbeg - p.qb; i64 rd_ = s.rbeg - p.rb;
						int mg = gap[qd < rd_ ? qd : (int)rd_];
						int w = mg < p.w ? mg : p.w;
						if (qd - rd_ < w && rd_ - qd < w) h = true;
						else {
							qd = p.qe - (s.qbeg + s.len); rd_ = p.re - (s.rbeg + s.len);
							mg = gap[qd < rd_ ? qd : (int)rd_];
							w = mg < p.w ? mg : p.w;
							if (qd - rd_ < w && rd_ - qd < w) h = true;
						}
					}
				}
				hit = __ballot(h) != 0;
			}
			if (hit) {
				bool other = false;
				for (int i0 = k + 1; i0 < n && !other; i0 += 64) {
					int i = i0 + lane;
					bool h = false;
					if (i < n && ORD(i) != SRT_MARK) {
						const DevSeed t = SD((int)ORD(i));
						if (!(t.len < ceil95[s.len])) {
							if (s.qbeg <= t.qbeg && s.qbeg + s.len - t.qbeg >= s.len >> 2 && t.qbeg - s.qbeg != t.rbeg - s.rbeg) h = true;
							if (t.qbeg <= s.qbeg && t.qbeg + t.len - s.qbeg >= s.len >> 2 && s.qbeg - t.qbeg != s.rbeg - t.rbeg) h = true;
						}
					}
					other = __ballot(h) != 0;
				}
				if (!other) {
					if (lane == 0) { if (st_sc) ordl[sl + k] = SRT_MARK; else ordg[k] = SRT_MARK; }
					__builtin_amdgcn_fence(__ATOMIC_RELEASE, "wavefront");
					__builtin_amdgcn_wave_barrier();
					__builtin_amdgcn_fence(__ATOMIC_ACQUIRE, "wavefront");
					continue;
				}
			}
			DevReg a;
			a.rb = a.re = 0; a.qb = a.qe = 0;
			a.rid = C.rid; a.score = a.truesc = -1; a.w = P.w; a.seedcov = 0; a.seedlen0 = s.len; a.frac_rep = C.frac_rep;
			int aw0 = P.w, aw1 = P.w;
			if (s.qbeg) {
				const int qlen = s.qbeg;
				const i64 tlen64 = s.rbeg - rmax0;
				const int tlen = (int)tlen64;
				WxResult r{};
				for (int i = 0; i < 2; ++i) {
					int prev = a.score;
					aw0 = P.w << i;
					int wc = aw0 < bound5[qlen] ? aw0 : bound5[qlen];
					r = extend(qlen, [&](int j) { return q[s.qbeg - 1 - j]; }, tlen, [&](int t) { return TB(s.rbeg - 1 - t); }, wc, s.len * P.a, P.pen_clip5);
					a.score = r.score;
					if (a.score == prev || r.max_off < (aw0 >> 1) + (aw0 >> 2)) break;
				}
				if (r.gscore <= 0 || r.gscore <= a.score - P.pen_clip5) {
					a.qb = s.qbeg - r.qle; a.rb = s.rbeg - r.tle; a.truesc = a.score;
				} else {
					a.qb = 0; a.rb = s.rbeg - r.gtle; a.truesc = r.gscore;
				}
			} else { a.score = a.truesc = s.len * P.a; a.qb = 0; a.rb = s.rbeg; }
			if (s.qbeg + s.len != lq) {
				const int sc0 = a.score, qe = s.qbeg + s.len;
				const i64 re = s.rbeg + s.len - rmax0;
				const int qlen = lq - qe, tlen = (int)(rmax1 - rmax0 - re);
				WxResult r{};
				for (int i = 0; i < 2; ++i) {
					int prev = a.score;
					aw1 = P.w << i;
					int wc = aw1 < bound3[qlen] ? aw1 : bound3[qlen];
					r = extend(qlen, [&](int j) { return q[qe + j]; }, tlen, [&](int t) { return TB(s.rbeg + s.len + t); }, wc, sc0, P.pen_clip3);
					a.score = r.score;
					if (a.score == prev || r.max_off < (aw1 >> 1) + (aw1 >> 2)) break;
				}
				if (r.gscore <= 0 || r.gscore <= a.score - P.pen_clip3) {
					a.qe = qe + r.qle; a.re = rmax0 + re + r.tle; a.truesc += a.score - sc0;
				} else {
					a.qe = lq; a.re = rmax0 + re + r.gtle; a.truesc += r.gscore - sc0;
				}
			} else { a.qe = lq; a.re = s.rbeg + s.len; }
			int cov = 0;
			for (int i = lane; i < n; i += 64) {
				const DevSeed t = SD(i);
				if (t.qbeg >= a.qb && t.qbeg + t.len <= a.qe && t.rbeg >= a.rb && t.rbeg + t.len <= a.re) cov += t.len;
			}
			a.seedcov = wave_sum_i32(cov);
			a.w = aw0 > aw1 ? aw0 : aw1;
			if (lane == 0) { av[nav] = a; if (nav < C2A_CAP_R) avl[nav] = a; }
			++nav;
			__builtin_amdgcn_wave_barrier();
		}
		if (unit_mode && lane == 0) U.c_rcnt[ci] = nav - nav0;
	}
	if (lane == 0) {
		if (unit_mode) { if (nav) atomicAdd(&n_regs[rd], nav); }
		else n_regs[rd] = nav;
		unsigned long long *st = counters + (size_t)(blockIdx.x % C2A_STAT_SLOTS) * 8;
		if (cells) atomicAdd(&st[0], cells);
		if (n_ext) atomicAdd(&st[1], n_ext);
		if (n_closed) atomicAdd(&st[2], n_closed);
		if (n_diff) atomicAdd(&st[3], n_diff);
	}
}

void launch_c2a(void *stream, const C2aParams &P, const ExtParams &ep, int n_reads, const uint8_t *d_seq, const int64_t *d_off,
                const int *d_len, const int *d_chain_beg, const int *d_chain_cnt, const DevChain *d_chains, const DevSeed *d_seeds, unsigned int *d_srt,
                const int *d_reg_beg, DevReg *d_regs, int *d_nregs, const int *d_tab, int tab_stride, const uint8_t *d_pac, unsigned long long *d_counters,
                int max_len, const int *d_order, const C2aUnits *units)
{
	C2aUnits U;
	if (units) U = *units;
	WxParams X;
	for (int i = 0; i < 25; ++i) X.mat[i] = ep.mat[i];
	X.o_del = ep.o_del; X.e_del = ep.e_del; X.o_ins = ep.o_ins; X.e_ins = ep.e_ins; X.zdrop = ep.zdrop;
	size_t shmem = (size_t)C2A_WAVES * c2a_lds_bytes(max_len);
	if (shmem > 64 * 1024 && hipFuncSetAttribute((const void *)c2a_kernel, hipFuncAttributeMaxDynamicSharedMemorySize, (int)shmem) != hipSuccess)
		die("c2a_kernel: cannot reserve %zu bytes of LDS", shmem);
	int n_blocks = (U.max_units + n_reads + C2A_WAVES - 1) / C2A_WAVES;
	hipLaunchKernelGGL(c2a_kernel, dim3(n_blocks), dim3(64 * C2A_WAVES), shmem, (hipStream_t)stream, P, X, n_reads, d_seq, d_off,
	                   d_len, d_chain_beg, d_chain_cnt, d_chains, d_seeds, d_srt, d_reg_beg, d_regs, d_nregs, d_tab, tab_stride, d_pac, d_counters,
	                   max_len, d_order, U);
}

}
```

mpibwa_amd/csrc/device.h:

```cpp
#ifndef MBW_DEVICE_H
#define MBW_DEVICE_H
#include "internal.h"
#include <mutex>
#include <vector>

namespace mbw {

struct FmDev {
	const void *blk;
	const void *occ32;
	const void *occ_sb;
	const uint64_t *sa;
	const uint64_t *sa_full;
	uint64_t primary, seq_len;
	uint64_t L2[5];
	int sa_shift;
	const void *p3tab;
	int p3_k;
	const void *kmt;
	int kmt_k;
};

struct DevIndex {
	int device = -1;
	bool ready = false;
	FmDev fm{};
	void *d_blk = nullptr; size_t blk_bytes = 0;
	void *d_occ32 = nullptr; size_t occ32_bytes = 0;
	void *d_sa = nullptr;  size_t sa_bytes = 0;
	void *d_pac = nullptr; size_t pac_bytes = 0;
	void *d_sa_full = nullptr; size_t sa_full_bytes = 0; double sa_expand_ms = 0;
	void *d_p3tab = nullptr;
	void *d_kmt = nullptr; size_t kmt_bytes = 0;
	int64_t l_pac = 0;
	uint64_t id_primary = 0, id_seq_len = 0, id_L2[5] = {0, 0, 0, 0, 0};
	int id_n_seqs = 0;
	uint64_t id_hash = 0;
};
DevIndex &dev_index();
bool index_matches(const bwt_t *bwt, const bntseq_t *bns, const char **what);
int calls_in_flight();
void expect_calls_in_flight(int n);
std::recursive_mutex &index_mutex();
void note_buffer_growth(size_t from, size_t to, const char *kind);

struct SmemParams {
	int min_seed_len, split_len, split_width, max_mem_intv;
};

struct DevBuf;
extern std::vector<DevBuf *> *g_devbuf_owner;
struct DevBuf {
	void *p = nullptr; size_t cap = 0;
	DevBuf() { if (g_devbuf_owner) g_devbuf_owner->push_back(this); }
	DevBuf(const DevBuf &) = delete;
	DevBuf &operator=(const DevBuf &) = delete;
	void *ensure(size_t bytes);
	void release();
};
struct PinBuf {
	void *p = nullptr; size_t cap = 0;
	void *ensure(size_t bytes);
};
bool device_memory_pressure(size_t wanted);
void release_idle_work_buffers();

void launch_smem(void *stream, const FmDev &fm, const SmemParams &sp, int n_reads, const uint8_t *d_seq,
                 const int64_t *d_off, const int *d_len, int cap, uint64_t *d_out, int *d_nout, int max_len,
                 unsigned long long *d_counters ,
                 void *d_scratch, size_t scratch_bytes_per_quad, int n_quads,
                 bool count_blocks );
size_t occ32_bytes(uint64_t seq_len);
size_t kmt_bytes(int k);
void launch_kmt_build(void *stream, const FmDev &fm, int k, void *d_tab);
void launch_occ32_build(void *stream, FmDev &fm, void *d_buf);
int  smem_grid_quads(int max_len, size_t *scratch_per_quad);
void launch_smem_p3(void *stream, const FmDev &fm, const SmemParams &sp, int n_reads, const uint8_t *d_seq, const int64_t *d_off,
                    const int *d_len, int cap, uint64_t *d_out, int *d_nout, unsigned long long *d_counters);
void launch_p3_build(void *stream, const FmDev &fm, int k, void *d_tab);

void launch_sa(void *stream, const FmDev &fm, int n, const uint64_t *d_k, uint64_t *d_out,
               unsigned long long *d_counters );
void launch_sa_dense(void *stream, const FmDev &fm, int n, const uint64_t *d_k, uint64_t *d_out);
void launch_sa_expand(void *stream, const FmDev &fm, uint64_t *full, unsigned long long *d_counters);

struct ExtParams {
	int8_t mat[25];
	int o_del, e_del, o_ins, e_ins, zdrop;
};
void launch_extend(void *stream, const ExtParams &ep, int n, const uint8_t *d_q, const int64_t *d_qoff,
                   const uint8_t *d_t, const int64_t *d_toff, const int *d_w, const int *d_h0, const int *d_eb,
                   int *d_out6, unsigned long long *d_cells, int max_qlen);

struct DevSeed { int64_t rbeg; int32_t qbeg, len; };
struct DevChain {
	int64_t far_beg, far_end;
	int32_t seed_beg, n_seeds;
	int32_t rid;
	float frac_rep;
	int64_t rmax0, rmax1;
};
struct DevReg {
	int64_t rb, re;
	int32_t qb, qe, rid, score, truesc, w, seedcov, seedlen0;
	float frac_rep;
	int32_t pad;
};
struct C2aParams {
	int64_t l_pac;
	int a, w, pen_clip5, pen_clip3;
	int early;
};
struct C2aUnits {
	int max_units = 0, heavy_t = 0;
	const unsigned int *n_units = nullptr;
	const int *ustart = nullptr;
	const int *unit_rd = nullptr, *unit_av = nullptr;
	const int *clist = nullptr;
	int *c_rabs = nullptr, *c_rcnt = nullptr;
};
struct C2aGroupBufs {
	PinBuf h_heavy, h_hoff, h_nunits;
	DevBuf heavy, hoff, scratch, clist, ustart, unit_rd, unit_av, nunits, c_rabs, c_rcnt;
};
C2aUnits c2a_prepare_units(void *stream, C2aGroupBufs &B, int heavy_t, int n, const int *chain_cnt, size_t n_chain_slots, const int *d_chain_beg,
                           const int *d_reg_beg, const DevChain *d_chains, int *d_nregs, void (*wait)(void *stream) = nullptr);
void c2a_launch_order(int n, const int *nseeds, int *order);
void c2a_length_tables(const mem_opt_t *opt, int max_len, std::vector<int> &tab);
void c2a_params(const mem_opt_t *opt, int64_t l_pac, int early, C2aParams &cp, ExtParams &ep);
size_t c2a_groups_scratch_bytes(int n_el);
void launch_c2a_groups(void *stream, int n_el, int n_heavy, const int *d_hoff, const int *d_heavy, const int *d_chain_beg, const int *d_reg_beg,
                       const DevChain *d_chains, void *d_scratch, int *d_clist, int *d_ustart, int *d_unit_rd, int *d_unit_av, unsigned int *d_n_units);
#define C2A_STAT_SLOTS 256
void launch_c2a(void *stream, const C2aParams &P, const ExtParams &ep, int n_reads, const uint8_t *d_seq, const int64_t *d_off,
                const int *d_len, const int *d_chain_beg, const int *d_chain_cnt, const DevChain *d_chains, const DevSeed *d_seeds, unsigned int *d_srt,
                const int *d_reg_beg, DevReg *d_regs, int *d_nregs, const int *d_tab, int tab_stride, const uint8_t *d_pac, unsigned long long *d_counters,
                int max_len, const int *d_order = nullptr, const C2aUnits *units = nullptr );

struct ChainParams {
	int64_t l_pac;
	int w, max_chain_gap, min_chain_weight, min_seed_len, max_chain_extend;
	float mask_level, drop_ratio;
};
ChainParams chain_params(const mem_opt_t *opt, int64_t l_pac);
void contig_table(const bntseq_t *bns, std::vector<int64_t> &ann_off, std::vector<uint8_t> &ann_alt);
void launch_chain(void *stream, const ChainParams &P, int n_reads, const int *d_len, const int *d_nseeds, const int *d_lrep,
                  const int64_t *d_seed_off, const uint64_t *d_sa, const int32_t *d_qbl, const int64_t *d_ann_off, const uint8_t *d_ann_alt,
                  int n_seqs, const int *d_tab, int tab_stride, DevChain *d_chains, DevSeed *d_seeds, unsigned int *d_srt, int *d_nchains,
                  void *d_scratch);
size_t chain_scratch_bytes(int n_reads);

size_t reg_pack_tmp_bytes(int n_reads);
void launch_reg_pack(void *stream, int n_reads, const int *d_reg_beg, const int *d_nregs, int *d_reg_pos, const DevReg *d_regs, DevReg *d_packed,
                     void *d_tmp, size_t tmp_bytes, const C2aUnits *units = nullptr, const int *d_chain_beg = nullptr, const int *d_chain_cnt = nullptr);

struct AlnReq {
	int64_t rb, re;
	int32_t read, qb, qe, w2, truesc, pad;
};
struct AlnHdr {
	int32_t score, NM, n_cigar, md_len;
	uint32_t pool_off;
	int32_t flags;
};
struct AlnParams { int64_t l_pac; int a, w; };
void aln_params(const mem_opt_t *opt, int64_t l_pac, AlnParams &ap, ExtParams &ep);
inline size_t aln_pool_bytes(size_t n_req) { return n_req * 96 + ((size_t)48 << 20); }
void cigar_gap_table(const mem_opt_t *opt, int max_len, std::vector<int> &tab);
size_t aln_lds_per_block(int max_len, int tcap);
void launch_aln(void *stream, const AlnParams &P, const ExtParams &ep, int n_req, const AlnReq *d_req, const uint8_t *d_seq,
                const int64_t *d_off, const uint8_t *d_pac, const int *d_gaptab, AlnHdr *d_hdr, uint8_t *d_pool,
                unsigned long long *d_counters, size_t pool_bytes, int max_len, int tcap, int *d_lists ,
                bool wide_only = false );

struct SamDesc {
	int64_t rb, re;
	int32_t qb, qe;
	int32_t req;
	int32_t rid, flag, mapq, score, sub;
};
#define SAM_XA_SHIFT 16
#define SAM_XA_MASK 15
struct SamParams {
	int64_t l_pac;
	int has_qual, rg_len;
	char rg[256];
};
SamParams sam_params(int64_t l_pac, bool has_qual);
void contig_names(const bntseq_t *bns, std::vector<char> &names, std::vector<int> &name_off);
size_t sam_arena_bytes(int n_reads, int max_len);
struct ChunkDev {
	const uint8_t *d_seq = nullptr; const int64_t *d_off = nullptr; const int *d_len = nullptr; int max_len = 0;
	const uint8_t *d_pac = nullptr; const int *d_gap = nullptr;
	const uint8_t *d_qual = nullptr, *d_names = nullptr; const int *d_noff = nullptr;
	const int64_t *d_ann_off = nullptr; const uint8_t *d_ann_alt = nullptr; const char *d_ann_names = nullptr; const int *d_ann_noff = nullptr;
};
struct AlnSamJob {
	int n_req = 0; const AlnReq *d_req = nullptr; AlnHdr *d_hdr = nullptr; uint8_t *d_pool = nullptr; size_t pool_bytes = 0;
	unsigned long long *d_cnt = nullptr; int *d_lists = nullptr;
	int ends = 2, r0 = 0, n_reads = 0;
	const SamDesc *h_desc = nullptr;
	SamDesc *d_desc = nullptr;
	const int *h_base = nullptr; int *d_base = nullptr;
	uint8_t *d_arena = nullptr; size_t arena_bytes = 0; unsigned long long *d_used = nullptr, *d_ooff = nullptr; int *d_olen = nullptr;
	int grid_blocks = 0;
};
void queue_aln_sam(void *stream, const mem_opt_t *opt, int64_t l_pac, const ChunkDev &D, const SamParams &sp, const AlnSamJob &J,
                   void *ev_a = nullptr, void *ev_b = nullptr);
void launch_sam_emit(void *stream, const SamParams &P, int n_reads, const SamDesc *d_desc, const int *d_req_base, const AlnReq *d_req, const AlnHdr *d_hdr,
                     const uint8_t *d_pool, const uint8_t *d_seq, const int64_t *d_off, const int *d_len, const uint8_t *d_qual,
                     const uint8_t *d_names, const int *d_name_off, const int64_t *d_ann_off, const char *d_ann_names, const int *d_ann_name_off,
                     uint8_t *d_arena, size_t arena_bytes, unsigned long long *d_arena_used, unsigned long long *d_out_off, int *d_out_len,
                     int grid_blocks = 0);
void launch_sam_emit_se(void *stream, const SamParams &P, int n_reads, const SamDesc *d_desc, const int *d_req_base, const AlnReq *d_req, const AlnHdr *d_hdr,
                        const uint8_t *d_pool, const uint8_t *d_seq, const int64_t *d_off, const int *d_len, const uint8_t *d_qual,
                        const uint8_t *d_names, const int *d_name_off, const int64_t *d_ann_off, const char *d_ann_names, const int *d_ann_name_off,
                        uint8_t *d_arena, size_t arena_bytes, unsigned long long *d_arena_used, unsigned long long *d_out_off, int *d_out_len,
                        int grid_blocks = 0);

struct MswReq;
struct MswRes;
#define PR_MAXREG 8
extern "C" int mi355x_pair_maxreg(void);
struct PairParams {
	int64_t l_pac;
	int a, b, pen_unpaired, min_seed_len, w, o_del, e_del, o_ins, e_ins, max_chain_gap, T, max_matesw;
	float mask_level_redun, mask_level, XA_drop_ratio;
	uint64_t id0;
	int lnq[40];
	int no_rescue;
	int low[4], high[4], failed[4];
	int tab_off[4];
	int ltab_n;
	int max_XA_hits;
};
bool pair_params(const mem_opt_t *opt, int64_t l_pac, const mem_pestat_t pes[4], int64_t n_processed, int max_len, PairParams &P, size_t *n_tab);
void pair_tables(const mem_opt_t *opt, const mem_pestat_t pes[4], const PairParams &P, size_t n_tab, double *tab);
void launch_first_reg(void *stream, int n, const int *d_reg_pos, const int *d_nregs, const DevReg *d_packed, DevReg *d_first, int *d_nfirst);
void launch_pair_simple(void *stream, const PairParams &P, int n_pairs, const DevReg *d_first, const int *d_nfirst, const uint8_t *d_ok,
                        const int64_t *d_ann_off, const uint8_t *d_ann_alt, const double *d_ptab, const double *d_ltab, uint8_t *d_status,
                        AlnReq *d_reqs, SamDesc *d_desc);

#define PW_MAXREG 64
extern "C" int mi355x_pair_wave_maxreg(void);
#define PW_HOST_LENGTH 6
#define PW_HOST_NO_PAIR 8
#define PW_HOST_SCORE 9
#define PW_HOST_SUPP 10
#define PW_HOST_XA 11
#define PW_HOST_NO_RESULT 12
#define PW_HOST_FULL 13
#define PW_HOST_TIE 14
#define PW_DECIDED_XA 16
#define PW_XA_CAP 8
extern "C" int mi355x_pair_wave_xa_cap(void);
#define PW_TAG_NO_WINDOW (-1)
#define PW_TAG_HOST (-2)
void launch_pair_wave(void *stream, const PairParams &P, int n_work, const int *d_work, const DevReg *d_lists, const int *d_loff, const int *d_len,
                      const MswReq *d_mreq, const MswRes *d_mres, const unsigned *d_mfirst, const short *d_tags, const int *d_toff,
                      const int64_t *d_ann_off, const double *d_ptab, const double *d_ltab, uint8_t *d_wstatus, AlnReq *d_reqs, SamDesc *d_desc,
                      AlnReq *d_xa_reqs = nullptr, uint8_t *d_xa_cnt = nullptr);
void launch_pair_wave_xa_scatter(void *stream, int n_work, const int *d_work, const int *d_dst, const AlnReq *d_w_reqs, const SamDesc *d_w_desc,
                                 const AlnReq *d_xa_reqs, const uint8_t *d_xa_cnt, AlnReq *d_reqs, SamDesc *d_desc, int clear_r0, int clear_n);
void launch_pair_wave_scatter(void *stream, int n_work, const int *d_work, const uint8_t *d_wstatus, const AlnReq *d_w_reqs, const SamDesc *d_w_desc,
                              AlnReq *d_reqs, SamDesc *d_desc, int clear_r0, int clear_n);

#define SE_HOST 0
#define SE_DECIDED 1
#define SE_HOST_COMMENT 2
#define SE_HOST_MAXREG 3
#define SE_HOST_PATCH 4
#define SE_HOST_LENGTH 5
#define SE_HOST_ALT 6
#define SE_HOST_SUPP 10
#define SE_HOST_XA 11
void se_params(const mem_opt_t *opt, int64_t l_pac, int64_t n_processed, int max_len, PairParams &P, mem_pestat_t pes[4]);
void launch_se_simple(void *stream, const PairParams &P, int n_reads, const DevReg *d_first, const int *d_nfirst, const uint8_t *d_ok,
                      const uint8_t *d_ann_alt, const double *d_ltab, uint8_t *d_status, AlnReq *d_reqs, SamDesc *d_desc);

struct MswReq {
	int64_t rb, re;
	int32_t read;
	int32_t is_rev;
};
struct MswRes { int32_t score, te, qe, score2, te2, tb, qb, flags; };
struct MswParams {
	int64_t l_pac;
	uint32_t slo[4];
	int s4[4];
	int o_del, e_del, o_ins, e_ins;
	int a, min_seed_len;
	int max_sc, shift;
};
size_t msw_lds_bytes(int max_len);
void launch_msw(void *stream, const MswParams &P, int n_req, const MswReq *d_req, const uint8_t *d_seq, const int64_t *d_off, const int *d_len,
                const uint8_t *d_pac, MswRes *d_res, uint16_t *d_rows, int max_len, const MswReq *h_req = nullptr, const int *h_len = nullptr,
                int *h_list = nullptr, int *d_list = nullptr, int *d_tail = nullptr);
#define MSW_TAIL_BUCKETS 9
inline size_t msw_tail_ints(size_t n_req) { return 16 + MSW_TAIL_BUCKETS * n_req; }
MswParams msw_params(const mem_opt_t *opt, int64_t l_pac);

void launch_seed_prep(void *stream, int n_reads, int cap, uint64_t *d_intv, const int *d_nintv, int max_occ, int *d_nseeds, int *d_lrep);
void launch_seed_enum(void *stream, int n_reads, int cap, const uint64_t *d_intv, const int *d_nintv, int max_occ,
                      const int64_t *d_seed_off, uint64_t *d_rows, int32_t *d_qbeg_len);

SmemParams smem_params(const mem_opt_t *opt);
int clamp_band(const mem_opt_t *opt, int qlen, int w, int end_bonus);

}
#endif
```

mpibwa_amd/csrc/device.hip:

```cpp
#include <hip/hip_runtime.h>
#include <atomic>
#include <algorithm>
#include <cstdio>
#include <cstdlib>
#include <cstring>
#include <vector>
#include "device.h"
#include "host.h"
#include <cmath>

namespace mbw {

#define HIP_OK(call)                                                                                             \
	do {                                                                                                         \
		hipError_t e_ = (call);                                                                                  \
		if (e_ != hipSuccess) die("%s failed: %s (%s:%d)", #call, hipGetErrorString(e_), __FILE__, __LINE__);    \
	} while (0)

static DevIndex g_idx;
DevIndex &dev_index() { return g_idx; }
static std::atomic<unsigned long long> g_buf_growths(0);
void note_buffer_growth(size_t from, size_t to, const char *kind)
{
	++g_buf_growths;
// ... 577 lines not shown
	const int n_reads = 2 * n_pairs;
	memset(status, 0, (size_t)n_pairs);
	memset(desc, 0xff, (size_t)n_reads * sizeof(SamDesc));
	memset(req, 0xff, (size_t)n_reads * sizeof(AlnReq));
	if (xa_req) { memset(xa_req, 0xff, (size_t)n_reads * PW_XA_CAP * sizeof(AlnReq)); memset(xa_cnt, 0, (size_t)n_reads); }
	if ((opt->flag & (MEM_F_NOPAIRING | MEM_F_ALL | MEM_F_REF_HDR | MEM_F_PRIMARY5)) || !(opt->mapQ_coef_len > 0)) return 0;
	const int64_t l_pac = bns->l_pac;
	std::vector<int64_t> slot(n_reads + 1);
	std::vector<int> lens(n_reads);
	int max_len = 1;
	slot[0] = 0;
	for (int i = 0; i < n_reads; ++i) {
		lens[i] = (int)(off[i + 1] - off[i]);
		slot[i + 1] = slot[i] + ((lens[i] + 15) & ~15);
		max_len = std::max(max_len, lens[i]);
	}
	if ((int64_t)max_len * opt->a >= 8192 || msw_lds_bytes(max_len) > 160 * 1024) die("mate-rescue kernel: reads too long for the device path");
	PairParams pp;
	size_t n_tab = 0;
	if (!pair_params(opt, l_pac, pes, n_processed, max_len, pp, &n_tab)) return -1;
	std::vector<double> tab(n_tab + (size_t)pp.ltab_n);
	pair_tables(opt, pes, pp, n_tab, tab.data());
	std::vector<int64_t> ann_off;
	std::vector<uint8_t> ann_alt;
	contig_table(bns, ann_off, ann_alt);
	const DevReg *hr = (const DevReg *)regs;
	std::vector<int> work, loff(1, 0), toff;
	std::vector<unsigned> mfirst;
	std::vector<DevReg> lists;
	std::vector<MswReqH> mreq;
	std::vector<int16_t> tags;
	std::vector<bseq1_t> s(2);
	for (int k = 0; k < n_pairs; ++k) {
		status[k] = 0;
		HRegV a[2];
		bool ok = true;
		for (int e = 0; e < 2 && ok; ++e) {
			for (int j = reg_off[2 * k + e]; j < reg_off[2 * k + e + 1]; ++j) {
				const DevReg &d = hr[j];
				if (d.rid < 0 || d.rid >= bns->n_seqs) die("%s: bad contig in a region of pair %d", who, k);
				HReg h;
				h.rb = d.rb; h.re = d.re; h.qb = d.qb; h.qe = d.qe; h.rid = d.rid; h.score = d.score; h.truesc = d.truesc; h.w = d.w;
				h.seedcov = d.seedcov; h.seedlen0 = d.seedlen0; h.frac_rep = d.frac_rep; h.secondary = -1; h.is_alt = bns->anns[d.rid].is_alt;
				a[e].push_back(h);
			}
			HRegV c;
			for (size_t j = 0; j < a[e].size(); ++j) c.push_back(a[e][j]);
			sort_dedup_patch(opt, 0, 0, 0, c);
			ok = c.size() == a[e].size() && c.settled;
			for (size_t j = 0; j < c.size() && ok; ++j) ok = c[j].rb == a[e][j].rb && c[j].re == a[e][j].re && c[j].qb == a[e][j].qb && c[j].score == a[e][j].score;
			a[e].settled = ok;
		}
		if (!ok || !pair_wave_eligible(a, PW_MAXREG)) continue;
		s[0].l_seq = lens[2 * k]; s[1].l_seq = lens[2 * k + 1];
		work.push_back(k);
		mfirst.push_back((unsigned)mreq.size());
		toff.push_back((int)tags.size());
		sam_pe_msw_collect_tagged(opt, bns, pes, s.data(), a, 2 * k, 4096, mreq, tags);
		for (int e = 0; e < 2; ++e) {
			lists.insert(lists.end(), hr + reg_off[2 * k + e], hr + reg_off[2 * k + e + 1]);
			loff.push_back((int)lists.size());
		}
	}
	const int n_work = (int)work.size();
	toff.push_back((int)tags.size());
	const size_t n_mreq = mreq.size();
	if (n_align) *n_align = (int)n_mreq;
	if (n_work == 0) return 0;
	hipStream_t st = 0;
	std::vector<uint8_t> flat(slot[n_reads] + 16, 4);
	for (int i = 0; i < n_reads; ++i) memcpy(flat.data() + slot[i], reads + off[i], lens[i]);
	int max_t = 1;
	for (size_t i = 0; i < n_mreq; ++i) max_t = std::max(max_t, (int)(mreq[i].re - mreq[i].rb));
	std::vector<void *> owned;
	auto up = [&](const void *h, size_t bytes) -> void * {
		void *d = nullptr;
		HIP_OK(hipMalloc(&d, bytes + 64));
		owned.push_back(d);
		if (h && bytes) HIP_OK(hipMemcpy(d, h, bytes, hipMemcpyHostToDevice));
		return d;
	};
	uint8_t *d_seq = (uint8_t *)up(flat.data(), flat.size());
	uint8_t *d_pac = (uint8_t *)up(pac, (size_t)(l_pac / 4 + 1));
	int64_t *d_off = (int64_t *)up(slot.data(), (size_t)(n_reads + 1) * 8);
	int *d_len = (int *)up(lens.data(), (size_t)n_reads * 4);
	MswReq *d_mreq = (MswReq *)up(mreq.data(), n_mreq * sizeof(MswReq));
	MswRes *d_mres = (MswRes *)up(nullptr, n_mreq * sizeof(MswRes));
	if (n_mreq) {
		uint16_t *d_rows = (uint16_t *)up(nullptr, n_mreq * (size_t)max_t * 2);
		std::vector<int> h_list(2 * n_mreq + 16);
		int *d_list = (int *)up(nullptr, (2 * n_mreq + 16) * sizeof(int));
		int *d_tail = (int *)up(nullptr, msw_tail_ints(n_mreq) * sizeof(int));
		launch_msw(st, msw_params(opt, l_pac), (int)n_mreq, d_mreq, d_seq, d_off, d_len, d_pac, d_mres, d_rows, max_len, (const MswReq *)mreq.data(), lens.data(),
		           h_list.data(), d_list, d_tail);
		HIP_OK(hipStreamSynchronize(st));
	}
	int *d_work = (int *)up(work.data(), (size_t)n_work * 4);
	DevReg *d_lists = (DevReg *)up(lists.data(), lists.size() * sizeof(DevReg));
	int *d_loff = (int *)up(loff.data(), loff.size() * 4);
	unsigned *d_mfirst = (unsigned *)up(mfirst.data(), mfirst.size() * 4);
	short *d_tags = (short *)up(tags.data(), tags.size() * 2);
	int *d_toff = (int *)up(toff.data(), toff.size() * 4);
	int64_t *d_ao = (int64_t *)up(ann_off.data(), ann_off.size() * 8);
	double *d_tab = (double *)up(tab.data(), tab.size() * 8);
	uint8_t *d_ws = (uint8_t *)up(nullptr, (size_t)n_work);
	AlnReq *d_rq = (AlnReq *)up(nullptr, (size_t)2 * n_work * sizeof(AlnReq));
	SamDesc *d_ds = (SamDesc *)up(nullptr, (size_t)2 * n_work * sizeof(SamDesc));
	AlnReq *d_xr = xa_req ? (AlnReq *)up(nullptr, (size_t)2 * n_work * PW_XA_CAP * sizeof(AlnReq)) : nullptr;
	uint8_t *d_xc = xa_req ? (uint8_t *)up(nullptr, (size_t)2 * n_work) : nullptr;
	HIP_OK(hipMemset(d_ws, 0, (size_t)n_work));
	if (d_xc) HIP_OK(hipMemset(d_xc, 0, (size_t)2 * n_work));
	launch_pair_wave(st, pp, n_work, d_work, d_lists, d_loff, d_len, d_mreq, d_mres, d_mfirst, d_tags, d_toff, d_ao, d_tab, d_tab + n_tab, d_ws, d_rq, d_ds,
	                 d_xr, d_xc);
	HIP_OK(hipDeviceSynchronize());
	HIP_OK(hipGetLastError());
	std::vector<uint8_t> ws((size_t)n_work);
	HIP_OK(hipMemcpy(ws.data(), d_ws, (size_t)n_work, hipMemcpyDeviceToHost));
	std::vector<SamDesc> w_ds((size_t)2 * n_work);
	std::vector<AlnReq> w_rq((size_t)2 * n_work);
	HIP_OK(hipMemcpy(w_ds.data(), d_ds, w_ds.size() * sizeof(SamDesc), hipMemcpyDeviceToHost));
	HIP_OK(hipMemcpy(w_rq.data(), d_rq, w_rq.size() * sizeof(AlnReq), hipMemcpyDeviceToHost));
	std::vector<AlnReq> w_xr(xa_req ? (size_t)2 * n_work * PW_XA_CAP : 0);
	std::vector<uint8_t> w_xc(xa_req ? (size_t)2 * n_work : 0);
	if (xa_req) {
		HIP_OK(hipMemcpy(w_xr.data(), d_xr, w_xr.size() * sizeof(AlnReq), hipMemcpyDeviceToHost));
		HIP_OK(hipMemcpy(w_xc.data(), d_xc, w_xc.size(), hipMemcpyDeviceToHost));
	}
	for (int t = 0; t < n_work; ++t) {
		status[work[t]] = ws[t];
		if (ws[t] != 1 && ws[t] != PW_DECIDED_XA) continue;
		for (int e = 0; e < 2; ++e) { ((SamDesc *)desc)[2 * work[t] + e] = w_ds[2 * t + e]; ((AlnReq *)req)[2 * work[t] + e] = w_rq[2 * t + e]; }
		if (ws[t] != PW_DECIDED_XA) continue;
		for (int e = 0; e < 2; ++e) {
			const int c = std::min<int>(w_xc[2 * t + e], PW_XA_CAP);
			xa_cnt[2 * work[t] + e] = (uint8_t)c;
			memcpy((AlnReq *)xa_req + (size_t)(2 * work[t] + e) * PW_XA_CAP, &w_xr[(size_t)(2 * t + e) * PW_XA_CAP], (size_t)c * sizeof(AlnReq));
		}
	}
	for (void *d : owned) (void)hipFree(d);
	return 0;
}
extern "C" int mi355x_pair_wave_batch(const mem_opt_t *opt, const bntseq_t *bns, const uint8_t *pac, const mem_pestat_t pes[4], int64_t n_processed,
                                      int n_pairs, const uint8_t *reads, const int64_t *off, const void *regs, const int *reg_off, uint8_t *status,
                                      void *desc, void *req, int *n_align)
{
	return pair_wave_batch("mi355x_pair_wave_batch", opt, bns, pac, pes, n_processed, n_pairs, reads, off, regs, reg_off, status, desc, req, n_align, nullptr,
	                       nullptr);
}
extern "C" int mi355x_pair_wave_xa_batch(const mem_opt_t *opt, const bntseq_t *bns, const uint8_t *pac, const mem_pestat_t pes[4], int64_t n_processed,
                                         int n_pairs, const uint8_t *reads, const int64_t *off, const void *regs, const int *reg_off, uint8_t *status,
                                         void *desc, void *req, int *n_align, void *xa_req, uint8_t *xa_cnt)
{
	if (!xa_req || !xa_cnt) die("mi355x_pair_wave_xa_batch: no room for the XA requests");
	return pair_wave_batch("mi355x_pair_wave_xa_batch", opt, bns, pac, pes, n_processed, n_pairs, reads, off, regs, reg_off, status, desc, req, n_align, xa_req,
	                       xa_cnt);
}

extern "C" int mi355x_smem_batch(const mem_opt_t *opt, int n, const uint8_t *seqs, const int64_t *off, int cap,
                                 uint64_t *intv_out, int *n_out, double *kernel_ms, uint64_t *algo_bytes)
{
	need_index();
	if (n <= 0) return 0;
	hipStream_t st = 0;
	int max_len = 0;
	std::vector<int64_t> poff(n + 1);
	std::vector<int> lens(n);
	poff[0] = 0;
	for (int i = 0; i < n; ++i) {
		lens[i] = (int)(off[i + 1] - off[i]);
		max_len = std::max(max_len, lens[i]);
		poff[i + 1] = poff[i] + ((lens[i] + 15) & ~15);
	}
	size_t total = off[n];
	std::vector<uint8_t> packed(poff[n] + 16, 0);
	for (int i = 0; i < n; ++i) memcpy(packed.data() + poff[i], seqs + off[i], lens[i]);
	uint8_t *d_seq; int64_t *d_off; uint64_t *d_out; int *d_nout, *d_len; unsigned long long *d_cnt; void *d_scr;
	HIP_OK(hipMalloc(&d_seq, packed.size()));
	HIP_OK(hipMalloc(&d_len, (size_t)n * 4));
	HIP_OK(hipMalloc(&d_off, (size_t)(n + 1) * 8));
	HIP_OK(hipMalloc(&d_out, (size_t)n * cap * 32));
	HIP_OK(hipMalloc(&d_nout, (size_t)n * 4));
	HIP_OK(hipMalloc(&d_cnt, 256));
	size_t per_quad = 0;
	int n_quads = smem_grid_quads(max_len, &per_quad);
	HIP_OK(hipMalloc(&d_scr, per_quad * n_quads));
	HIP_OK(hipMemcpy(d_seq, packed.data(), packed.size(), hipMemcpyHostToDevice));
	HIP_OK(hipMemcpy(d_off, poff.data(), (size_t)(n + 1) * 8, hipMemcpyHostToDevice));
	HIP_OK(hipMemcpy(d_len, lens.data(), (size_t)n * 4, hipMemcpyHostToDevice));
	HIP_OK(hipMemset(d_cnt, 0, 256));
	HIP_OK(hipMemset(d_nout, 0, (size_t)n * 4));
	Timer tm;
	tm.start(st);
	const char *ce = getenv("MPIBWA_SMEM_COUNT");
	const bool count_blocks = !(ce && atoi(ce) == 0);
	launch_smem(st, g_idx.fm, smem_params(opt), n, d_seq, d_off, d_len, cap, d_out, d_nout, max_len, d_cnt, d_scr, per_quad, n_quads, count_blocks);
	double ms = tm.stop(st);
	HIP_OK(hipGetLastError());
	unsigned long long cnt[32];
	HIP_OK(hipMemcpy(cnt, d_cnt, 256, hipMemcpyDeviceToHost));
	HIP_OK(hipMemcpy(n_out, d_nout, (size_t)n * 4, hipMemcpyDeviceToHost));
	HIP_OK(hipMemcpy(intv_out, d_out, (size_t)n * cap * 32, hipMemcpyDeviceToHost));
	(void)hipFree(d_seq); (void)hipFree(d_off); (void)hipFree(d_out); (void)hipFree(d_nout); (void)hipFree(d_cnt);
	(void)hipFree(d_scr); (void)hipFree(d_len);
	uint64_t n_intv = 0;
	for (int i = 0; i < n; ++i) {
		int m = std::min(n_out[i], cap);
		Intv *a = (Intv *)(intv_out + (size_t)i * cap * 4);
		std::sort(a, a + m, [](const Intv &x, const Intv &y) { return x.info < y.info; });
		n_intv += m;
	}
	if (kernel_ms) *kernel_ms = ms;
	if (algo_bytes) *algo_bytes = count_blocks ? cnt[1] * 64 + total + n_intv * 32 : 0;
	return cnt[2] ? -1 : 0;
}

extern "C" int mi355x_sa_batch2(int n, const uint64_t *k, uint64_t *sa_out, double *kernel_ms, int dense)
{
	need_index();
	if (!dense) return mi355x_sa_batch(n, k, sa_out, kernel_ms, nullptr);
	if (!g_idx.fm.sa_full) return -1;
	if (n <= 0) return 0;
	uint64_t *d_k, *d_o;
	HIP_OK(hipMalloc(&d_k, (size_t)n * 8)); HIP_OK(hipMalloc(&d_o, (size_t)n * 8));
	HIP_OK(hipMemcpy(d_k, k, (size_t)n * 8, hipMemcpyHostToDevice));
	Timer tm;
	tm.start(0);
	launch_sa_dense(0, g_idx.fm, n, d_k, d_o);
	double ms = tm.stop(0);
	HIP_OK(hipGetLastError());
	HIP_OK(hipMemcpy(sa_out, d_o, (size_t)n * 8, hipMemcpyDeviceToHost));
	(void)hipFree(d_k); (void)hipFree(d_o);
	if (kernel_ms) *kernel_ms = ms;
	return 0;
}
extern "C" double mi355x_sa_dense_info(size_t *bytes) { if (bytes) *bytes = g_idx.sa_full_bytes; return g_idx.sa_expand_ms; }

extern "C" int mi355x_sa_batch(int n, const uint64_t *k, uint64_t *sa_out, double *kernel_ms, uint64_t *algo_bytes)
{
	need_index();
	if (n <= 0) return 0;
	hipStream_t st = 0;
	uint64_t *d_k, *d_o; unsigned long long *d_cnt;
	HIP_OK(hipMalloc(&d_k, (size_t)n * 8));
	HIP_OK(hipMalloc(&d_o, (size_t)n * 8));
	HIP_OK(hipMalloc(&d_cnt, 64));
	HIP_OK(hipMemcpy(d_k, k, (size_t)n * 8, hipMemcpyHostToDevice));
	HIP_OK(hipMemset(d_cnt, 0, 64));
	Timer tm;
	tm.start(st);
	launch_sa(st, g_idx.fm, n, d_k, d_o, d_cnt);
	double ms = tm.stop(st);
	HIP_OK(hipGetLastError());
	unsigned long long cnt[8];
	HIP_OK(hipMemcpy(cnt, d_cnt, 64, hipMemcpyDeviceToHost));
	HIP_OK(hipMemcpy(sa_out, d_o, (size_t)n * 8, hipMemcpyDeviceToHost));
	(void)hipFree(d_k); (void)hipFree(d_o); (void)hipFree(d_cnt);
	if (kernel_ms) *kernel_ms = ms;
	if (algo_bytes) *algo_bytes = cnt[1] * 64 + (uint64_t)n * 8;
	return 0;
}

extern "C" int mi355x_extend_batch(const mem_opt_t *opt, int n, const uint8_t *q, const int64_t *qoff, const uint8_t *t,
                                   const int64_t *toff, const int *w, const int *h0, const int *end_bonus, int *out6,
                                   double *kernel_ms, uint64_t *cells)
{
	int nd = 0;
	if (hipGetDeviceCount(&nd) != hipSuccess || nd == 0) die("no HIP device visible (no CPU fallback)");
	if (n <= 0) return 0;
	hipStream_t st = 0;
	std::vector<int> wc(n);
	int max_qlen = 0;
	for (int i = 0; i < n; ++i) {
		int ql = (int)(qoff[i + 1] - qoff[i]);
		max_qlen = std::max(max_qlen, ql);
		wc[i] = clamp_band(opt, ql, w[i], end_bonus[i]);
	}
	uint8_t *d_q, *d_t; int64_t *d_qo, *d_to; int *d_w, *d_h0, *d_out; unsigned long long *d_cells;
	HIP_OK(hipMalloc(&d_q, qoff[n] + 16)); HIP_OK(hipMalloc(&d_t, toff[n] + 16));
	HIP_OK(hipMalloc(&d_qo, (size_t)(n + 1) * 8)); HIP_OK(hipMalloc(&d_to, (size_t)(n + 1) * 8));
	HIP_OK(hipMalloc(&d_w, (size_t)n * 4)); HIP_OK(hipMalloc(&d_h0, (size_t)n * 4));
	HIP_OK(hipMalloc(&d_out, (size_t)n * 24)); HIP_OK(hipMalloc(&d_cells, 8));
	HIP_OK(hipMemcpy(d_q, q, qoff[n], hipMemcpyHostToDevice));
	HIP_OK(hipMemcpy(d_t, t, toff[n], hipMemcpyHostToDevice));
	HIP_OK(hipMemcpy(d_qo, qoff, (size_t)(n + 1) * 8, hipMemcpyHostToDevice));
	HIP_OK(hipMemcpy(d_to, toff, (size_t)(n + 1) * 8, hipMemcpyHostToDevice));
	HIP_OK(hipMemcpy(d_w, wc.data(), (size_t)n * 4, hipMemcpyHostToDevice));
	HIP_OK(hipMemcpy(d_h0, h0, (size_t)n * 4, hipMemcpyHostToDevice));
	HIP_OK(hipMemset(d_cells, 0, 8));
	ExtParams ep;
	memcpy(ep.mat, opt->mat, 25);
	ep.o_del = opt->o_del; ep.e_del = opt->e_del; ep.o_ins = opt->o_ins; ep.e_ins = opt->e_ins; ep.zdrop = opt->zdrop;
	Timer tm;
	tm.start(st);
	launch_extend(st, ep, n, d_q, d_qo, d_t, d_to, d_w, d_h0, nullptr, d_out, d_cells, max_qlen);
	double ms = tm.stop(st);
	HIP_OK(hipGetLastError());
	unsigned long long c = 0;
	HIP_OK(hipMemcpy(&c, d_cells, 8, hipMemcpyDeviceToHost));
	HIP_OK(hipMemcpy(out6, d_out, (size_t)n * 24, hipMemcpyDeviceToHost));
	(void)hipFree(d_q); (void)hipFree(d_t); (void)hipFree(d_qo); (void)hipFree(d_to); (void)hipFree(d_w);
	(void)hipFree(d_h0); (void)hipFree(d_out); (void)hipFree(d_cells);
	if (kernel_ms) *kernel_ms = ms;
	if (cells) *cells = c;
	return 0;
}

namespace mbw {
MswParams msw_params(const mem_opt_t *opt, int64_t l_pac)
{
	MswParams P;
	P.l_pac = l_pac;
	int8_t mn = 127, mx = 0;
	for (int i = 0; i < 25; ++i) {
		if (opt->mat[i] < mn) mn = opt->mat[i];
		if (opt->mat[i] > mx) mx = opt->mat[i];
	}
	for (int t = 0; t < 4; ++t) {
		P.slo[t] = 0;
		for (int q = 0; q < 4; ++q) P.slo[t] |= (uint32_t)(uint8_t)opt->mat[t * 5 + q] << (8 * q);
		P.s4[t] = opt->mat[t * 5 + 4];
	}
	P.o_del = opt->o_del; P.e_del = opt->e_del; P.o_ins = opt->o_ins; P.e_ins = opt->e_ins;
	P.a = opt->a; P.min_seed_len = opt->min_seed_len;
	P.max_sc = mx > 0 ? mx : 1;
	P.shift = (uint8_t)(256 - (uint8_t)mn);
	return P;
}
}

extern "C" int mi355x_matesw_batch(const mem_opt_t *opt, int64_t l_pac, const uint8_t *pac, int n_reads, const uint8_t *reads, const int64_t *off,
                                   int n_req, const int64_t *rb, const int64_t *re, const int *read, const int *is_rev, int *out8,
                                   double *kernel_ms)
{
	int nd = 0;
	if (hipGetDeviceCount(&nd) != hipSuccess || nd == 0) die("no HIP device visible (no CPU fallback)");
	if (n_req <= 0) return 0;
	hipStream_t st = 0;
	std::vector<int64_t> slot(n_reads + 1);
	std::vector<int> lens(n_reads);
	int max_len = 0;
	slot[0] = 0;
	for (int i = 0; i < n_reads; ++i) {
		lens[i] = (int)(off[i + 1] - off[i]);
		slot[i + 1] = slot[i] + ((lens[i] + 15) & ~15);
		max_len = std::max(max_len, lens[i]);
	}
	if ((int64_t)max_len * opt->a >= 8192 || msw_lds_bytes(max_len) > 160 * 1024) die("mate-rescue kernel: reads too long for the device path");
	std::vector<uint8_t> flat(slot[n_reads] + 16, 4);
	for (int i = 0; i < n_reads; ++i) memcpy(flat.data() + slot[i], reads + off[i], lens[i]);
	std::vector<MswReq> rq(n_req);
	int max_t = 1;
	for (int i = 0; i < n_req; ++i) {
		rq[i].rb = rb[i]; rq[i].re = re[i]; rq[i].read = read[i]; rq[i].is_rev = is_rev[i];
		if (re[i] < rb[i] || re[i] > 2 * l_pac || rb[i] < 0 || read[i] < 0 || read[i] >= n_reads) die("mi355x_matesw_batch: bad request %d", i);
		max_t = std::max(max_t, (int)(re[i] - rb[i]));
	}
	uint8_t *d_seq, *d_pac; int64_t *d_off; int *d_len; MswReq *d_req; MswRes *d_res; uint16_t *d_rows;
	HIP_OK(hipMalloc(&d_seq, flat.size())); HIP_OK(hipMalloc(&d_pac, l_pac / 4 + 16));
	HIP_OK(hipMalloc(&d_off, (size_t)(n_reads + 1) * 8)); HIP_OK(hipMalloc(&d_len, (size_t)n_reads * 4));
	HIP_OK(hipMalloc(&d_req, (size_t)n_req * sizeof(MswReq))); HIP_OK(hipMalloc(&d_res, (size_t)n_req * sizeof(MswRes)));
	HIP_OK(hipMalloc(&d_rows, (size_t)n_req * max_t * 2));
	HIP_OK(hipMemcpy(d_seq, flat.data(), flat.size(), hipMemcpyHostToDevice));
	HIP_OK(hipMemcpy(d_pac, pac, l_pac / 4 + 1, hipMemcpyHostToDevice));
	HIP_OK(hipMemcpy(d_off, slot.data(), (size_t)(n_reads + 1) * 8, hipMemcpyHostToDevice));
	HIP_OK(hipMemcpy(d_len, lens.data(), (size_t)n_reads * 4, hipMemcpyHostToDevice));
	HIP_OK(hipMemcpy(d_req, rq.data(), (size_t)n_req * sizeof(MswReq), hipMemcpyHostToDevice));
	Timer tm;
	tm.start(st);
	std::vector<int> h_list(2 * (size_t)n_req + 16);
	int *d_list, *d_tail;
	HIP_OK(hipMalloc(&d_list, (2 * (size_t)n_req + 16) * sizeof(int)));
	HIP_OK(hipMalloc(&d_tail, msw_tail_ints(n_req) * sizeof(int)));
	launch_msw(st, msw_params(opt, l_pac), n_req, d_req, d_seq, d_off, d_len, d_pac, d_res, d_rows, max_len, rq.data(), lens.data(), h_list.data(), d_list,
	           d_tail);
	double ms = tm.stop(st);
	HIP_OK(hipGetLastError());
	static_assert(sizeof(MswRes) == 32, "MswRes layout");
	HIP_OK(hipMemcpy(out8, d_res, (size_t)n_req * sizeof(MswRes), hipMemcpyDeviceToHost));
	(void)hipFree(d_seq); (void)hipFree(d_pac); (void)hipFree(d_off); (void)hipFree(d_len); (void)hipFree(d_req); (void)hipFree(d_res);
	(void)hipFree(d_rows); (void)hipFree(d_list); (void)hipFree(d_tail);
	if (kernel_ms) *kernel_ms = ms;
	return 0;
}

extern "C" int64_t mi355x_chain_batch(const mem_opt_t *opt, const bntseq_t *bns, int n_reads, const int *lens, const int *l_rep,
                                      const int64_t *seed_off, const uint64_t *rbeg, const int32_t *qbeg_len, int which, int64_t *out,
                                      int64_t out_cap, int64_t *out_off)
{
	using namespace mbw;
	const int64_t S = seed_off[n_reads];
	int max_len = 0;
	for (int i = 0; i < n_reads; ++i) max_len = std::max(max_len, lens[i]);
	const int TS = max_len + 2;
	std::vector<int> tab;
	c2a_length_tables(opt, max_len, tab);
	std::vector<int> nseeds(n_reads);
	for (int i = 0; i < n_reads; ++i) nseeds[i] = (int)(seed_off[i + 1] - seed_off[i]);
	std::vector<int> nch(n_reads, 0);
	std::vector<DevChain> chains(std::max<int64_t>(S, 1));
	std::vector<DevSeed> seeds(std::max<int64_t>(S, 1));
	if (which == 0) {
		int nd = 0;
		if (hipGetDeviceCount(&nd) != hipSuccess || nd == 0) die("no HIP device visible (no CPU fallback)");
		std::vector<int64_t> ann_off;
		std::vector<uint8_t> ann_alt;
		contig_table(bns, ann_off, ann_alt);
		int *d_len, *d_ns, *d_lrep, *d_tab, *d_nch; int64_t *d_so, *d_ao; uint64_t *d_sa; int32_t *d_qbl; uint8_t *d_aa;
		DevChain *d_ch; DevSeed *d_sd; unsigned int *d_srt;
		HIP_OK(hipMalloc(&d_len, n_reads * 4 + 4)); HIP_OK(hipMalloc(&d_ns, n_reads * 4 + 4)); HIP_OK(hipMalloc(&d_lrep, n_reads * 4 + 4));
		HIP_OK(hipMalloc(&d_tab, tab.size() * 4)); HIP_OK(hipMalloc(&d_nch, n_reads * 4 + 4)); HIP_OK(hipMalloc(&d_so, (n_reads + 1) * 8));
		HIP_OK(hipMalloc(&d_ao, ann_off.size() * 8)); HIP_OK(hipMalloc(&d_aa, ann_alt.size())); HIP_OK(hipMalloc(&d_sa, S * 8 + 8));
		HIP_OK(hipMalloc(&d_qbl, S * 8 + 8)); HIP_OK(hipMalloc(&d_ch, (S + 1) * sizeof(DevChain))); HIP_OK(hipMalloc(&d_sd, (S + 1) * sizeof(DevSeed)));
		HIP_OK(hipMalloc(&d_srt, (S + 1) * 4));
		HIP_OK(hipMemcpy(d_len, lens, n_reads * 4, hipMemcpyHostToDevice)); HIP_OK(hipMemcpy(d_ns, nseeds.data(), n_reads * 4, hipMemcpyHostToDevice));
		HIP_OK(hipMemcpy(d_lrep, l_rep, n_reads * 4, hipMemcpyHostToDevice)); HIP_OK(hipMemcpy(d_tab, tab.data(), tab.size() * 4, hipMemcpyHostToDevice));
		HIP_OK(hipMemcpy(d_so, seed_off, (n_reads + 1) * 8, hipMemcpyHostToDevice)); HIP_OK(hipMemcpy(d_ao, ann_off.data(), ann_off.size() * 8, hipMemcpyHostToDevice));
		HIP_OK(hipMemcpy(d_aa, ann_alt.data(), ann_alt.size(), hipMemcpyHostToDevice)); HIP_OK(hipMemcpy(d_sa, rbeg, S * 8, hipMemcpyHostToDevice));
		HIP_OK(hipMemcpy(d_qbl, qbeg_len, S * 8, hipMemcpyHostToDevice));
		void *d_scr = nullptr;
		HIP_OK(hipMalloc(&d_scr, chain_scratch_bytes(n_reads)));
		launch_chain(0, chain_params(opt, bns->l_pac), n_reads, d_len, d_ns, d_lrep, d_so, d_sa, d_qbl, d_ao, d_aa, bns->n_seqs, d_tab, TS, d_ch, d_sd, d_srt, d_nch, d_scr);
		HIP_OK(hipDeviceSynchronize());
		(void)hipFree(d_scr);
		HIP_OK(hipMemcpy(nch.data(), d_nch, n_reads * 4, hipMemcpyDeviceToHost));
		HIP_OK(hipMemcpy((void *)chains.data(), d_ch, S * sizeof(DevChain), hipMemcpyDeviceToHost));
		HIP_OK(hipMemcpy((void *)seeds.data(), d_sd, S * sizeof(DevSeed), hipMemcpyDeviceToHost));
		(void)hipFree(d_len); (void)hipFree(d_ns); (void)hipFree(d_lrep); (void)hipFree(d_tab); (void)hipFree(d_nch); (void)hipFree(d_so); (void)hipFree(d_ao);
		(void)hipFree(d_aa); (void)hipFree(d_sa); (void)hipFree(d_qbl); (void)hipFree(d_ch); (void)hipFree(d_sd); (void)hipFree(d_srt);
	} else {
		ChainScratch scr;
		std::vector<HSeed> hs;
		std::vector<HChain *> ch;
		std::vector<uint64_t> key;
		for (int i = 0; i < n_reads; ++i) {
			const int ns = nseeds[i];
			if (ns == 0) continue;
			hs.resize(ns);
			for (int k = 0; k < ns; ++k) {
				const int64_t so = seed_off[i] + k;
				hs[k].rbeg = (int64_t)rbeg[so]; hs[k].qbeg = qbeg_len[2 * so]; hs[k].len = hs[k].score = qbeg_len[2 * so + 1];
			}
			chains_from_seeds(opt, bns, lens[i], hs.data(), ns, l_rep[i], scr, ch);
			chain_filter(opt, scr, ch);
			int64_t cur = seed_off[i];
			int c = 0;
			for (const HChain *cp : ch) {
				DevChain &d = chains[seed_off[i] + c];
				pack_chain_for_device(bns, *cp, lens[i], tab.data(), key, d, seeds.data() + cur);
				d.seed_beg = (int)cur;
				cur += d.n_seeds;
				++c;
			}
			nch[i] = c;
		}
	}
	int64_t at = 0;
	for (int i = 0; i < n_reads; ++i) {
		out_off[i] = at;
		if (at + 1 > out_cap) return -1;
		out[at++] = nch[i];
		for (int c = 0; c < nch[i]; ++c) {
			const DevChain &d = chains[seed_off[i] + c];
			if (at + 7 + 3 * (int64_t)d.n_seeds > out_cap) return -1;
			uint32_t fb;
			memcpy(&fb, &d.frac_rep, 4);
			out[at++] = d.rid; out[at++] = d.n_seeds; out[at++] = d.far_beg; out[at++] = d.far_end; out[at++] = d.rmax0; out[at++] = d.rmax1; out[at++] = fb;
			for (int k = 0; k < d.n_seeds; ++k) {
				const DevSeed &s = seeds[d.seed_beg + k];
				out[at++] = s.rbeg; out[at++] = s.qbeg; out[at++] = s.len;
			}
		}
	}
	out_off[n_reads] = at;
	return at;
}

extern "C" int64_t mi355x_c2a_batch(const mem_opt_t *opt, const bntseq_t *bns, int n_reads, const uint8_t *reads, const int64_t *off,
                                    const int *n_chains, const int *chain_rid, const float *chain_frac, const int *chain_nseeds,
                                    const int64_t *seed_rbeg, const int *seed_qbeg, const int *seed_len, const int *seed_score,
                                    int heavy_t, int early, int layout, int64_t *out, int64_t out_cap, int64_t *out_off,
                                    uint64_t *stat4, int *n_units)
{
	using namespace mbw;
	need_index();
	if (bns->l_pac != g_idx.l_pac) die("mi355x_c2a_batch: the index given is not the resident one");
	if (layout != 0 && layout != 1) die("mi355x_c2a_batch: layout %d", layout);
	if (n_reads <= 0) return 0;
	const int64_t l_pac = bns->l_pac;
	int max_len = 0;
	std::vector<int> lens(n_reads);
	for (int i = 0; i < n_reads; ++i) { lens[i] = (int)(off[i + 1] - off[i]); max_len = std::max(max_len, lens[i]); }
	std::vector<int> tab;
	c2a_length_tables(opt, max_len, tab);
	const int TS = max_len + 2;
	std::vector<int> cbeg(n_reads + 1, 0), sbeg(n_reads + 1, 0), nseeds(n_reads, 0);
	int64_t NC = 0, NS = 0;
	for (int i = 0; i < n_reads; ++i) {
		cbeg[i] = (int)NC; sbeg[i] = (int)NS;
		for (int c = 0; c < n_chains[i]; ++c) nseeds[i] += chain_nseeds[NC + c];
		NC += n_chains[i]; NS += nseeds[i];
	}
	cbeg[n_reads] = (int)NC; sbeg[n_reads] = (int)NS;
	std::vector<DevChain> pch(std::max<int64_t>(NC, 1));
	std::vector<DevSeed> psd(std::max<int64_t>(NS, 1));
	{
		HChain ch;
		std::vector<uint64_t> key;
		int64_t s = 0;
		for (int i = 0; i < n_reads; ++i)
			for (int c = cbeg[i]; c < cbeg[i + 1]; ++c) {
				ch.rid = chain_rid[c]; ch.frac_rep = chain_frac[c];
				ch.seeds.resize(chain_nseeds[c]);
				if (ch.rid < 0 || ch.rid >= bns->n_seqs) die("mi355x_c2a_batch: chain %d: rid %d", c, ch.rid);
				for (int k = 0; k < chain_nseeds[c]; ++k, ++s) {
					HSeed &h = ch.seeds[k];
					h.rbeg = seed_rbeg[s]; h.qbeg = seed_qbeg[s]; h.len = seed_len[s]; h.score = seed_score[s];
					if (h.len <= 0 || h.qbeg < 0 || h.qbeg + h.len > lens[i] || h.rbeg < 0 || h.rbeg + h.len > 2 * l_pac)
						die("mi355x_c2a_batch: read %d, chain %d: seed %d out of bounds", i, c, k);
				}
				DevChain &d = pch[c];
				pack_chain_for_device(bns, ch, lens[i], tab.data(), key, d, psd.data() + (s - chain_nseeds[c]));
				for (int k = 0; k < chain_nseeds[c]; ++k) {
					const DevSeed &t = psd[s - chain_nseeds[c] + k];
					if (t.rbeg < d.rmax0 || t.rbeg + t.len > d.rmax1) die("mi355x_c2a_batch: read %d, chain %d: a seed leaves the chain's contig or strand", i, c);
				}
			}
	}
	std::vector<int> chain_beg(n_reads), chain_cnt(n_reads), reg_beg(n_reads);
	std::vector<int64_t> seed_at(n_reads);
	int64_t n_slots = 0, n_chain_slots = 0;
	if (layout == 0) {
		int64_t so = 0;
		for (int i = 0; i < n_reads; ++i) {
			chain_beg[i] = reg_beg[i] = (int)so; seed_at[i] = so;
			so += std::max(nseeds[i], n_chains[i]) + (i % 3);
		}
		n_slots = n_chain_slots = so;
	} else {
		const int64_t base = NS + 5;
		for (int i = 0; i < n_reads; ++i) { chain_beg[i] = (int)(base + cbeg[i]); reg_beg[i] = (int)(base + sbeg[i]); seed_at[i] = base + sbeg[i]; }
		n_slots = base + NS; n_chain_slots = base + NC;
	}
	if (n_slots > 0x7fffffff) die("mi355x_c2a_batch: too many seeds");
	std::vector<DevChain> hch(std::max<int64_t>(n_chain_slots, 1));
	std::vector<DevSeed> hsd(std::max<int64_t>(n_slots, 1));
	std::vector<unsigned int> hsrt(std::max<int64_t>(n_slots, 1), 0);
	for (int i = 0; i < n_reads; ++i) {
		chain_cnt[i] = n_chains[i];
		int64_t at = seed_at[i];
		for (int c = 0; c < n_chains[i]; ++c) {
			DevChain d = pch[cbeg[i] + c];
			const int64_t from = sbeg[i] + (at - seed_at[i]);
			for (int k = 0; k < d.n_seeds; ++k) { hsd[at + k] = psd[from + k]; hsrt[at + k] = (unsigned int)k; }
			d.seed_beg = (int)at;
			at += d.n_seeds;
			hch[chain_beg[i] + c] = d;
		}
	}
	std::vector<int64_t> slot(n_reads + 1, 0);
	for (int i = 0; i < n_reads; ++i) slot[i + 1] = slot[i] + ((lens[i] + 15) & ~15);
	std::vector<uint8_t> flat(slot[n_reads] + 16, 4);
	for (int i = 0; i < n_reads; ++i) memcpy(flat.data() + slot[i], reads + off[i], (size_t)lens[i]);
	std::vector<int> order(n_reads);
	c2a_launch_order(n_reads, nseeds.data(), order.data());

	hipStream_t st = 0;
	uint8_t *d_seq; int64_t *d_off; int *d_len, *d_cbeg, *d_ccnt, *d_rbeg, *d_nregs, *d_tab, *d_order, *d_reg_pos;
	DevChain *d_ch; DevSeed *d_sd; unsigned int *d_srt; DevReg *d_regs, *d_packed; unsigned long long *d_stat;
	HIP_OK(hipMalloc(&d_seq, flat.size())); HIP_OK(hipMalloc(&d_off, (size_t)(n_reads + 1) * 8)); HIP_OK(hipMalloc(&d_len, (size_t)n_reads * 4));
	HIP_OK(hipMalloc(&d_cbeg, (size_t)n_reads * 4)); HIP_OK(hipMalloc(&d_ccnt, (size_t)n_reads * 4)); HIP_OK(hipMalloc(&d_rbeg, (size_t)n_reads * 4));
	HIP_OK(hipMalloc(&d_nregs, (size_t)(n_reads + 1) * 4)); HIP_OK(hipMalloc(&d_tab, tab.size() * 4)); HIP_OK(hipMalloc(&d_order, (size_t)n_reads * 4));
	HIP_OK(hipMalloc(&d_reg_pos, (size_t)(n_reads + 1) * 4));
	HIP_OK(hipMalloc(&d_ch, hch.size() * sizeof(DevChain))); HIP_OK(hipMalloc(&d_sd, hsd.size() * sizeof(DevSeed)));
	HIP_OK(hipMalloc(&d_srt, hsrt.size() * 4)); HIP_OK(hipMalloc(&d_regs, hsd.size() * sizeof(DevReg)));
	HIP_OK(hipMalloc(&d_packed, hsd.size() * sizeof(DevReg))); HIP_OK(hipMalloc(&d_stat, C2A_STAT_SLOTS * 64));
	const size_t tmp_bytes = reg_pack_tmp_bytes(n_reads);
	void *d_tmp;
	HIP_OK(hipMalloc(&d_tmp, tmp_bytes));
	HIP_OK(hipMemcpy(d_seq, flat.data(), flat.size(), hipMemcpyHostToDevice));
	HIP_OK(hipMemcpy(d_off, slot.data(), (size_t)(n_reads + 1) * 8, hipMemcpyHostToDevice));
	HIP_OK(hipMemcpy(d_len, lens.data(), (size_t)n_reads * 4, hipMemcpyHostToDevice));
	HIP_OK(hipMemcpy(d_cbeg, chain_beg.data(), (size_t)n_reads * 4, hipMemcpyHostToDevice));
	HIP_OK(hipMemcpy(d_ccnt, chain_cnt.data(), (size_t)n_reads * 4, hipMemcpyHostToDevice));
	HIP_OK(hipMemcpy(d_rbeg, reg_beg.data(), (size_t)n_reads * 4, hipMemcpyHostToDevice));
	HIP_OK(hipMemcpy(d_tab, tab.data(), tab.size() * 4, hipMemcpyHostToDevice));
	HIP_OK(hipMemcpy(d_order, order.data(), (size_t)n_reads * 4, hipMemcpyHostToDevice));
	HIP_OK(hipMemcpy(d_ch, hch.data(), hch.size() * sizeof(DevChain), hipMemcpyHostToDevice));
	HIP_OK(hipMemcpy(d_sd, hsd.data(), hsd.size() * sizeof(DevSeed), hipMemcpyHostToDevice));
	HIP_OK(hipMemcpy(d_srt, hsrt.data(), hsrt.size() * 4, hipMemcpyHostToDevice));
	HIP_OK(hipMemset(d_stat, 0, C2A_STAT_SLOTS * 64));
	{
		C2aGroupBufs B;
		const C2aUnits units = c2a_prepare_units(st, B, heavy_t, n_reads, chain_cnt.data(), (size_t)std::max<int64_t>(n_chain_slots, 1), d_cbeg, d_rbeg,
		                                         d_ch, d_nregs);
		C2aParams cp;
		ExtParams ep;
		c2a_params(opt, l_pac, early, cp, ep);
		launch_c2a(st, cp, ep, n_reads, d_seq, d_off, d_len, d_cbeg, d_ccnt, d_ch, d_sd, d_srt, d_rbeg, d_regs, d_nregs, d_tab, TS,
		           (const uint8_t *)g_idx.d_pac, d_stat, max_len, d_order, units.max_units > 0 ? &units : nullptr);
		launch_reg_pack(st, n_reads, d_rbeg, d_nregs, d_reg_pos, d_regs, d_packed, d_tmp, tmp_bytes, units.max_units > 0 ? &units : nullptr, d_cbeg, d_ccnt);
		HIP_OK(hipStreamSynchronize(st));
		HIP_OK(hipGetLastError());
		if (n_units) *n_units = units.max_units;
		B.heavy.release(); B.hoff.release(); B.scratch.release(); B.clist.release(); B.ustart.release(); B.unit_rd.release();
		B.unit_av.release(); B.nunits.release(); B.c_rabs.release(); B.c_rcnt.release();
		if (B.h_heavy.p) HIP_OK(hipHostFree(B.h_heavy.p));
// ... 282 lines not shown
```

mpibwa_amd/csrc/ext_kernels.hip:

```cpp
#include <hip/hip_runtime.h>
#include "device.h"
#include "wave_ext.cuh"

namespace mbw {

#define EXT_WAVES 4

__global__ void __launch_bounds__(64 * EXT_WAVES)
extend_kernel(WxParams P, int n, const uint8_t *__restrict__ q, const int64_t *__restrict__ qoff,
              const uint8_t *__restrict__ t, const int64_t *__restrict__ toff, const int *__restrict__ w,
              const int *__restrict__ h0, int *__restrict__ out6, unsigned long long *cells_total, int max_qlen)
{
	extern __shared__ int lds[];
	const int wave = threadIdx.x >> 6, lane = threadIdx.x & 63;
	const int job = blockIdx.x * EXT_WAVES + wave;
	if (job >= n) return;
	const WxLds L = wx_lds(lds + (size_t)wave * wx_lds_ints(max_qlen), max_qlen);
	const uint8_t *qs = q + qoff[job];
	const uint8_t *ts = t + toff[job];
	const int qlen = (int)(qoff[job + 1] - qoff[job]), tlen = (int)(toff[job + 1] - toff[job]);
	unsigned long long cells = 0;
	for (int j = lane; j < qlen; j += 64) L.Qs[j] = qs[j];
	__builtin_amdgcn_wave_barrier();
	WxResult r = wave_extend(qlen, tlen, [&](int i) { return ts[i]; }, P, w[job], h0[job], L, cells);
	if (lane == 0) {
		int *o = out6 + (size_t)job * 6;
		o[0] = r.score; o[1] = r.qle; o[2] = r.tle; o[3] = r.gtle; o[4] = r.gscore; o[5] = r.max_off;
		atomicAdd(cells_total, cells);
	}
}

void launch_extend(void *stream, const ExtParams &ep, int n, const uint8_t *d_q, const int64_t *d_qoff,
                   const uint8_t *d_t, const int64_t *d_toff, const int *d_w, const int *d_h0, const int *d_eb,
                   int *d_out6, unsigned long long *d_cells, int max_qlen)
{
	(void)d_eb;
	WxParams P;
	for (int i = 0; i < 25; ++i) P.mat[i] = ep.mat[i];
	P.o_del = ep.o_del; P.e_del = ep.e_del; P.o_ins = ep.o_ins; P.e_ins = ep.e_ins; P.zdrop = ep.zdrop;
	size_t shmem = (size_t)EXT_WAVES * wx_lds_ints(max_qlen) * sizeof(int);
	int n_blocks = (n + EXT_WAVES - 1) / EXT_WAVES;
	hipLaunchKernelGGL(extend_kernel, dim3(n_blocks), dim3(64 * EXT_WAVES), shmem, (hipStream_t)stream, P, n, d_q, d_qoff,
	                   d_t, d_toff, d_w, d_h0, d_out6, d_cells, max_qlen);
}

}
```

mpibwa_amd/csrc/wave_ext.cuh:

```cuda
#ifndef MBW_WAVE_EXT_CUH
#define MBW_WAVE_EXT_CUH
#include <hip/hip_runtime.h>

namespace mbw {

#define WX_NEG (-(1 << 29))

template <int CTRL, int ROW_MASK>
__device__ __forceinline__ int wx_dpp(int old, int v)
{
	return __builtin_amdgcn_update_dpp(old, v, CTRL, ROW_MASK, 0xf, false);
}

__device__ __forceinline__ int wx_scan_max(int v)
{
	asm volatile("s_nop 1\n\tv_max_i32_dpp %0, %0, %0 row_shr:1 row_mask:0xf bank_mask:0xf\n\t"
	             "s_nop 1\n\tv_max_i32_dpp %0, %0, %0 row_shr:2 row_mask:0xf bank_mask:0xf\n\t"
	             "s_nop 1\n\tv_max_i32_dpp %0, %0, %0 row_shr:4 row_mask:0xf bank_mask:0xf\n\t"
	             "s_nop 1\n\tv_max_i32_dpp %0, %0, %0 row_shr:8 row_mask:0xf bank_mask:0xf\n\t"
	             "s_nop 1\n\tv_max_i32_dpp %0, %0, %0 row_bcast:15 row_mask:0xa bank_mask:0xf\n\t"
	             "s_nop 1\n\tv_max_i32_dpp %0, %0, %0 row_bcast:31 row_mask:0xc bank_mask:0xf\n\t"
	             "s_nop 1"
	             : "+v"(v));
	return v;
}
__device__ __forceinline__ int wx_smin(int a, int b)
{
	int r;
	asm("s_min_i32 %0, %1, %2" : "=s"(r) : "s"(a), "s"(b) : "scc");
	return r;
}
__device__ __forceinline__ int wx_prev_lane(int v, int first)
{
	return wx_dpp<0x138, 0xf>(first, v);
}

struct WxParams {
	int8_t mat[25];
	int o_del, e_del, o_ins, e_ins, zdrop;
};

struct WxResult { int score, qle, tle, gtle, gscore, max_off; };

struct WxLds { int2 *HE; uint8_t *Qs; int2 *dummy; };
__host__ __device__ inline int wx_lds_ints(int max_qlen) { return 2 * (max_qlen + 2 + 64) + (((max_qlen + 64 + 7) & ~7) >> 2) + 2; }
__device__ __forceinline__ WxLds wx_lds(int *base, int max_qlen)
{
	WxLds L;
	L.HE = (int2 *)base;
	L.Qs = (uint8_t *)(L.HE + (max_qlen + 2 + 64));
	L.dummy = (int2 *)(L.Qs + ((max_qlen + 64 + 7) & ~7));
	return L;
}

template <bool EARLY = false, typename TF>
__device__ __forceinline__ WxResult wave_extend(int qlen, int tlen, TF tf, const WxParams &P, int w, int h0, const WxLds &L,
                                                unsigned long long &cells, int max_sc = 1, int clip = 0x3fffffff)
{
	const int lane = threadIdx.x & 63;
	int2 *const HE = L.HE;
	const uint8_t *const Qs = L.Qs;
	qlen = __builtin_amdgcn_readfirstlane(qlen);
	tlen = __builtin_amdgcn_readfirstlane(tlen);
	w = __builtin_amdgcn_readfirstlane(w);
	h0 = __builtin_amdgcn_readfirstlane(h0);
	max_sc = __builtin_amdgcn_readfirstlane(max_sc);
	clip = __builtin_amdgcn_readfirstlane(clip);
	const int oe_del = P.o_del + P.e_del, oe_ins = P.o_ins + P.e_ins, e_del = P.e_del, e_ins = P.e_ins;
	int lane_e = lane * e_ins;
	asm volatile("" : "+v"(lane_e));
	for (int j = lane; j <= qlen; j += 64) {
		int v = 0;
		if (j == 0) v = h0;
		else {
			int t = h0 - oe_ins - (j - 1) * e_ins;
			int h1 = h0 > oe_ins ? h0 - oe_ins : 0;
			if (j == 1) v = h1;
			else v = (h1 - (j - 2) * e_ins > e_ins) ? t : 0;
		}
		HE[j] = make_int2(v, 0);
	}
	__builtin_amdgcn_wave_barrier();
	int best = h0, best_i = -1, best_j = -1, best_ie = -1, gscore = -1, max_off = 0;
	int beg = 0, end = qlen;
	int tv_base = -64;
	int vslo = 0, vshi = 0;
	uint32_t plo[5], phi[5];
#pragma unroll
	for (int t = 0; t < 5; ++t) {
		plo[t] = (uint32_t)(uint8_t)P.mat[t * 5] | (uint32_t)(uint8_t)P.mat[t * 5 + 1] << 8 | (uint32_t)(uint8_t)P.mat[t * 5 + 2] << 16 |
		         (uint32_t)(uint8_t)P.mat[t * 5 + 3] << 24;
		phi[t] = (uint32_t)(uint8_t)P.mat[t * 5 + 4];
	}
	for (int i = 0; i < tlen; ++i) {
		if (i - tv_base >= 64) {
			tv_base = i;
			const int tb = (i + lane < tlen) ? (int)tf(i + lane) : 4;
			vslo = (int)(tb == 0 ? plo[0] : tb == 1 ? plo[1] : tb == 2 ? plo[2] : tb == 3 ? plo[3] : plo[4]);
			vshi = (int)(tb == 0 ? phi[0] : tb == 1 ? phi[1] : tb == 2 ? phi[2] : tb == 3 ? phi[3] : phi[4]);
		}
		const uint32_t slo = (uint32_t)__builtin_amdgcn_readlane(vslo, i - tv_base), shi = (uint32_t)__builtin_amdgcn_readlane(vshi, i - tv_base);
		if (beg < i - w) beg = i - w;
		end = wx_smin(wx_smin(end, i + w + 1), qlen);
		int hleft0 = 0;
		if (beg == 0) { hleft0 = h0 - (P.o_del + e_del * (i + 1)); if (hleft0 < 0) hleft0 = 0; }
		const int n_col = end - beg;
		int lanekey = -1;
		int A = beg * e_ins;
		int h_carry = hleft0, h_cin = hleft0;
		int h_strip = 0;
		int first_nz = end, last_nz = -1;
		const int jb = beg + lane;
		int je = lane_e + beg * e_ins;
		for (int s0 = 0; s0 <= n_col; s0 += 64, je += 64 * e_ins) {
			const int j = jb + s0;
			const bool act = j < end, wr = j <= end;
			const int2 he = HE[j];
			const int diag = he.x, e = he.y;
			const int sc = (int)(int8_t)__builtin_amdgcn_perm(shi, slo, (uint32_t)Qs[j] | 0x0c0c0c00u);
			const int M = (act && diag) ? diag + sc : 0;
			int tI = M - oe_ins; tI = tI > 0 ? tI : 0;
			const int g = tI + je;
			const int incl = wx_scan_max(g);
			const int excl = wx_prev_lane(incl, WX_NEG);
			const int f = max(A, excl + e_ins) - je;
			const int h = act ? max(max(M, e), f) : 0;
			int tD = M - oe_del; tD = tD > 0 ? tD : 0;
			const int en = act ? max(e - e_del, tD) : 0;
			const int h_prev = wx_prev_lane(h, h_carry);
			*(wr ? HE + j : L.dummy) = make_int2(h_prev, en);
			A = max(A, __builtin_amdgcn_readlane(incl, 63) + e_ins);
			lanekey = max(lanekey, h << 13 | j);
			const unsigned long long nz = __builtin_amdgcn_ballot_w64((h_prev | en) != 0);
			if (nz) {
				const int lo = beg + s0 + __ffsll((long long)nz) - 1, hi = beg + s0 + 63 - __clzll(nz);
				if (lo < end && lo < first_nz) first_nz = lo;
				if (hi > last_nz) last_nz = hi;
			}
			h_cin = h_carry;
			h_carry = __builtin_amdgcn_readlane(h, 63);
			h_strip = h;
		}
		const int h_last = (n_col > 0 && (n_col & 63)) ? __builtin_amdgcn_readlane(h_strip, (n_col - 1) & 63) : n_col > 0 ? h_cin : hleft0;
		int rowkey = -1;
		if (n_col > 0) {
			rowkey = __builtin_amdgcn_readlane(wx_scan_max(lanekey), 63);
			cells += (unsigned long long)n_col;
		} else if (n_col < 0) {
			if (lane == 0) HE[end] = make_int2(hleft0, 0);
		}
		__builtin_amdgcn_wave_barrier();
		const int jfin = n_col > 0 ? end : beg;
		if (jfin == qlen) {
			if (h_last >= gscore) best_ie = i;
			if (h_last > gscore) gscore = h_last;
		}
		const int rowmax = rowkey < 0 ? 0 : rowkey >> 13, rowmax_j = rowkey < 0 ? -1 : rowkey & 8191;
		if (rowmax == 0) break;
		if (rowmax > best) {
			best = rowmax; best_i = i; best_j = rowmax_j;
			int d = rowmax_j - i; d = d < 0 ? -d : d;
			if (d > max_off) max_off = d;
		} else if (P.zdrop > 0) {
			int di = i - best_i, dj = rowmax_j - best_j;
			if (di > dj) { if (best - rowmax - (di - dj) * e_del > P.zdrop) break; }
			else { if (best - rowmax - (dj - di) * e_ins > P.zdrop) break; }
		}
		const int nb = first_nz;
		const int ne = last_nz >= nb ? last_nz : nb - 1;
		beg = nb;
		end = ne + 2 < qlen ? ne + 2 : qlen;
		if (EARLY && (i & 3) == 3 && (gscore >= 0 || rowmax + (qlen - 1 - rowmax_j) * max_sc <= best - clip)) {
			int b = WX_NEG;
			for (int j = lane; j <= qlen; j += 64) {
				const int2 he = HE[j];
				const int hv = j < qlen ? he.x + (qlen - j) * max_sc : WX_NEG;
				const int ev = he.y + (qlen - 1 - j) * max_sc;
				b = max(b, max(hv, ev));
			}
			b = __builtin_amdgcn_readlane(wx_scan_max(b), 63);
			if (gscore >= 0 && b < gscore && b <= best) break;
			if (b <= best - clip && gscore <= best - clip) break;
		}
	}
	WxResult r;
	r.score = best; r.qle = best_j + 1; r.tle = best_i + 1; r.gtle = best_ie + 1; r.gscore = gscore; r.max_off = max_off;
	return r;
}

}
#endif
```

Before: 6.532.

## Specialize narrow-band wave extension and precompute scoring params in WxParams

Adds a single-strip fast path in the wavefront extension for bands narrower than a wavefront, removing the strip loop and its running carries. Row-level control flow becomes branchless selects with one combined break test. Scoring constants (max score, plain-matrix check, gap minimum, packed score tables) move into a precomputed WxParams, and the c2a caller passes concrete functor types instead of a runtime-branching lambda. Cell counters shrink to 32-bit and are returned in the result. It also adds an extend2 test entry point, and the restructured break and z-drop logic risks subtle SAM mismatches.

```diff
diff --git a/include/mpibwa_amd.h b/include/mpibwa_amd.h
--- a/include/mpibwa_amd.h
+++ b/include/mpibwa_amd.h
@@ -162,6 +162,10 @@
 int mi355x_extend_batch(const mem_opt_t *opt, int n, const uint8_t *q, const int64_t *qoff,
                         const uint8_t *t, const int64_t *toff, const int *w, const int *h0,
                         const int *end_bonus, int *out6, double *kernel_ms, uint64_t *cells);
+int mi355x_extend_batch2(const mem_opt_t *opt, int n, const uint8_t *q, const int64_t *qoff,
+                         const uint8_t *t, const int64_t *toff, const int *w, const int *h0,
+                         const int *end_bonus, const int *early, const int *clip, int *out6,
+                         uint64_t *cells, double *kernel_ms);
 
 int64_t mi355x_chain_batch(const mem_opt_t *opt, const bntseq_t *bns, int n_reads, const int *lens, const int *l_rep,
                            const int64_t *seed_off, const uint64_t *rbeg, const int32_t *qbeg_len, int which,
diff --git a/mpibwa_amd/api.py b/mpibwa_amd/api.py
--- a/mpibwa_amd/api.py
+++ b/mpibwa_amd/api.py
@@ -15,7 +15,7 @@
     "mem_process_seqs", "mem_opt_init", "bwa_fill_scmat", "bwa_idx_load_from_disk", "bwa_mem2idx", "bwa_idx_destroy",
     "mi355x_index_upload", "mi355x_index_alloc", "mi355x_index_buffers", "mi355x_index_d2d", "mi355x_index_commit",
     "mi355x_finalize", "mi355x_index_build", "mi355x_index_build_gpu",
-    "mi355x_smem_batch", "mi355x_sa_batch", "mi355x_sa_batch2", "mi355x_sa_dense_info", "mi355x_extend_batch", "mi355x_matesw_batch", "mi355x_chain_batch", "mi355x_c2a_batch", "mi355x_pair_batch", "mi355x_pair_maxreg", "mi355x_fastq_scan", "mi355x_fastq_chunks", "mi355x_fastq_fill", "mi355x_last_stats", "mi355x_host_cpus", "mi355x_collect_sam", "mi355x_collect_sam_into", "mi355x_host_ksw_align2",
+    "mi355x_smem_batch", "mi355x_sa_batch", "mi355x_sa_batch2", "mi355x_sa_dense_info", "mi355x_extend_batch", "mi355x_extend_batch2", "mi355x_matesw_batch", "mi355x_chain_batch", "mi355x_c2a_batch", "mi355x_pair_batch", "mi355x_pair_maxreg", "mi355x_fastq_scan", "mi355x_fastq_chunks", "mi355x_fastq_fill", "mi355x_last_stats", "mi355x_host_cpus", "mi355x_collect_sam", "mi355x_collect_sam_into", "mi355x_host_ksw_align2",
     "bwa_set_rg", "bwa_insert_header", "bwa_idx2mem", "mi355x_write_map", "mi355x_init", "mi355x_rank_host_threads", "mi355x_index_checksums", "mi355x_init_bcast_seconds", "mi355x_global_batch", "mi355x_device_count", "mi355x_device_memory", "mi355x_buffer_growths", "mi355x_prewarm", "mi355x_max_calls",
     "mi355x_sam_batch", "mi355x_sam_arena_bytes", "mi355x_se_batch", "mi355x_sam_se_batch", "mi355x_seed_batch", "mi355x_pair_wave_batch", "mi355x_pair_wave_maxreg",
     "mi355x_pair_wave_xa_batch", "mi355x_pair_wave_xa_cap",
@@ -71,6 +71,7 @@
     sig("mi355x_sa_batch2", C.c_int, [C.c_int, C.c_void_p, C.c_void_p, P(C.c_double), C.c_int])
     sig("mi355x_sa_dense_info", C.c_double, [P(C.c_size_t)])
     sig("mi355x_extend_batch", C.c_int, [P(abi.mem_opt_t), C.c_int] + [C.c_void_p] * 8 + [P(C.c_double), P(C.c_uint64)])
+    sig("mi355x_extend_batch2", C.c_int, [P(abi.mem_opt_t), C.c_int] + [C.c_void_p] * 11 + [P(C.c_double)])
     sig("mi355x_chain_batch", C.c_int64, [P(abi.mem_opt_t), C.c_void_p, C.c_int] + [C.c_void_p] * 5 + [C.c_int, C.c_void_p, C.c_int64, C.c_void_p])
     sig("mi355x_c2a_batch", C.c_int64, [P(abi.mem_opt_t), C.c_void_p, C.c_int] + [C.c_void_p] * 10 + [C.c_int] * 3 +
         [C.c_void_p, C.c_int64, C.c_void_p, C.c_void_p, C.c_void_p])
@@ -532,3 +533,24 @@
                                      w.ctypes.data, h0.ctypes.data, eb.ctypes.data, out.ctypes.data, C.byref(ms),
                                      C.byref(cells))
         return out, ms.value, cells.value
+
+    def extend2(self, opt, qs, ts, w, h0, end_bonus, early, clip):
+        n = len(qs)
+        qoff = np.zeros(n + 1, dtype=np.int64)
+        qoff[1:] = np.cumsum([len(s) for s in qs])
+        toff = np.zeros(n + 1, dtype=np.int64)
+        toff[1:] = np.cumsum([len(s) for s in ts])
+        qf = np.concatenate(qs).astype(np.uint8)
+        tf = np.concatenate(ts).astype(np.uint8)
+        w = np.ascontiguousarray(w, dtype=np.int32)
+        h0 = np.ascontiguousarray(h0, dtype=np.int32)
+        eb = np.ascontiguousarray(end_bonus, dtype=np.int32)
+        early = np.ascontiguousarray(np.broadcast_to(np.asarray(early, dtype=np.int32), (n,)))
+        clip = np.ascontiguousarray(np.broadcast_to(np.asarray(clip, dtype=np.int32), (n,)))
+        out = np.zeros((n, 6), dtype=np.int32)
+        cells = np.zeros(n, dtype=np.uint64)
+        ms = C.c_double(0)
+        self.lib.mi355x_extend_batch2(opt, n, qf.ctypes.data, qoff.ctypes.data, tf.ctypes.data, toff.ctypes.data,
+                                      w.ctypes.data, h0.ctypes.data, eb.ctypes.data, early.ctypes.data, clip.ctypes.data,
+                                      out.ctypes.data, cells.ctypes.data, C.byref(ms))
+        return out, ms.value, cells
diff --git a/mpibwa_amd/csrc/aln_kernel.hip b/mpibwa_amd/csrc/aln_kernel.hip
--- a/mpibwa_amd/csrc/aln_kernel.hip
+++ b/mpibwa_amd/csrc/aln_kernel.hip
@@ -369,9 +369,7 @@
                 unsigned long long *d_counters, size_t pool_bytes, int max_len, int tcap, int *d_lists, bool wide_only)
 {
 	if (n_req <= 0) return;
-	WxParams X;
-	for (int i = 0; i < 25; ++i) X.mat[i] = ep.mat[i];
-	X.o_del = ep.o_del; X.e_del = ep.e_del; X.o_ins = ep.o_ins; X.e_ins = ep.e_ins; X.zdrop = ep.zdrop;
+	const WxParams X = wx_params(ep);
 	const size_t shmem = aln_lds_per_block(max_len, tcap);
 	const size_t shmem_small = shmem - (size_t)(aln_zcap(max_len) - aln_zcap_small(max_len)) * ALN_WAVES;
 	const size_t shmem_fast = ((size_t)2 * ((max_len + 3) & ~3) + ALN_MDCAP + 16) * ALN_WAVES;
diff --git a/mpibwa_amd/csrc/c2a_kernel.hip b/mpibwa_amd/csrc/c2a_kernel.hip
--- a/mpibwa_amd/csrc/c2a_kernel.hip
+++ b/mpibwa_amd/csrc/c2a_kernel.hip
@@ -37,6 +37,13 @@
 	const unsigned long long u = (unsigned long long)v;
 	return (i64)((unsigned long long)(unsigned)__builtin_amdgcn_readfirstlane((int)(u >> 32)) << 32 | (unsigned)__builtin_amdgcn_readfirstlane((int)u));
 }
+
+struct QBase { const uint8_t *p; int dir; __device__ __forceinline__ int operator()(int j) const { return p[dir * j]; } };
+struct WinBase { const uint8_t *p; int dir; __device__ __forceinline__ int operator()(int t) const { return p[dir * t]; } };
+struct PacBase {
+	const uint8_t *pac; i64 l_pac, p0; int dir;
+	__device__ __forceinline__ int operator()(int t) const { return ref_base(pac, l_pac, p0 + dir * t); }
+};
 
 #define C2A_WAVES 1
 #define SRT_MARK 0xFFFFFFFFu
@@ -122,16 +129,11 @@
 		__builtin_amdgcn_fence(__ATOMIC_ACQUIRE, "wavefront");
 	}
 	int nav = 0;
-	unsigned long long cells = 0, n_ext = 0, n_diff = 0, n_closed = 0;
+	unsigned int cells = 0, n_ext = 0, n_diff = 0, n_closed = 0;
 	const i64 l_pac = P.l_pac;
-	int max_sc = 1;
-	for (int t = 0; t < 25; ++t) max_sc = X.mat[t] > max_sc ? X.mat[t] : max_sc;
-
-	const int sc_a = X.mat[0], sc_b = -X.mat[1];
-	bool plain = sc_a > 0 && sc_b > 0;
-	for (int i = 0; i < 4; ++i)
-		for (int j = 0; j < 4; ++j) plain = plain && X.mat[i * 5 + j] == (i == j ? sc_a : -sc_b);
-	const int g1 = (X.o_del < X.o_ins ? X.o_del : X.o_ins) + (X.e_del < X.e_ins ? X.e_del : X.e_ins);
+
+	const int sc_a = X.sc_a, sc_b = X.sc_b, g1 = X.g1;
+	const bool plain = X.plain != 0;
 	auto ungapped = [&](int qlen, int tlen, auto tf, int h0, WxResult &r) -> bool {
 		if (!plain || tlen < qlen || qlen <= 0) return false;
 		int mm = 0, p = -1;
@@ -160,23 +162,25 @@
 		return true;
 	};
 
-	auto extend = [&](int qlen, auto qf, int tlen, auto tf, int wc, int h0, int clip) -> WxResult {
-		++n_ext;
+	auto extend = [&](int qlen, auto qf, int tlen, auto tf, int wc, int h0, int clip) __attribute__((always_inline)) -> WxResult {
 		for (int j = lane; j < qlen; j += 64) L.Qs[j] = (uint8_t)qf(j);
 		__builtin_amdgcn_wave_barrier();
-		if (P.early == 0) return wave_extend<false>(qlen, tlen, tf, X, wc, h0, L, cells, max_sc);
 		WxResult r;
-		const bool closed = ungapped(qlen, tlen, tf, h0, r);
-		if (closed) ++n_closed;
-		else r = wave_extend<true>(qlen, tlen, tf, X, wc, h0, L, cells, max_sc, clip);
-		if (P.early == 2) {
-			unsigned long long c2 = 0;
-			const WxResult f = wave_extend<false>(qlen, tlen, tf, X, wc, h0, L, c2, max_sc);
-			const bool loc_r = r.gscore <= 0 || r.gscore <= r.score - clip, loc_f = f.gscore <= 0 || f.gscore <= f.score - clip;
-			bool same = f.score == r.score && f.qle == r.qle && f.tle == r.tle && f.max_off == r.max_off && loc_r == loc_f;
-			if (same && (!loc_f || closed)) same = f.gtle == r.gtle && f.gscore == r.gscore;
-			if (!same) ++n_diff;
-		}
+		r.cells = 0;
+		bool closed = false, differ = false;
+		if (P.early == 0) r = wave_extend<false>(qlen, tlen, tf, X, wc, h0, L);
+		else {
+			closed = ungapped(qlen, tlen, tf, h0, r);
+			if (!closed) r = wave_extend<true>(qlen, tlen, tf, X, wc, h0, L, clip);
+			if (P.early == 2) {
+				const WxResult f = wave_extend<false>(qlen, tlen, tf, X, wc, h0, L);
+				const bool loc_r = r.gscore <= 0 || r.gscore <= r.score - clip, loc_f = f.gscore <= 0 || f.gscore <= f.score - clip;
+				bool same = f.score == r.score && f.qle == r.qle && f.tle == r.tle && f.max_off == r.max_off && loc_r == loc_f;
+				if (same && (!loc_f || closed)) same = f.gtle == r.gtle && f.gscore == r.gscore;
+				differ = !same;
+			}
+		}
+		++n_ext; cells += r.cells; n_closed += closed; n_diff += differ;
 		return r;
 	};
 
@@ -211,7 +215,6 @@
 			__builtin_amdgcn_wave_barrier();
 			__builtin_amdgcn_fence(__ATOMIC_ACQUIRE, "wavefront");
 		}
-		auto TB = [&](i64 pos) -> int { return st_w ? (int)winl[pos - rmax0] : ref_base(pac, l_pac, pos); };
 
 		for (int k = n - 1; k >= 0; --k) {
 			DevSeed s = SD(uni((int)ORD(k)));
@@ -273,7 +276,9 @@
 					int prev = a.score;
 					aw0 = P.w << i;
 					int wc = aw0 < bound5[qlen] ? aw0 : bound5[qlen];
-					r = extend(qlen, [&](int j) { return q[s.qbeg - 1 - j]; }, tlen, [&](int t) { return TB(s.rbeg - 1 - t); }, wc, s.len * P.a, P.pen_clip5);
+					const QBase qf{q + s.qbeg - 1, -1};
+					r = st_w ? extend(qlen, qf, tlen, WinBase{winl + (int)tlen64 - 1, -1}, wc, s.len * P.a, P.pen_clip5)
+					         : extend(qlen, qf, tlen, PacBase{pac, l_pac, s.rbeg - 1, -1}, wc, s.len * P.a, P.pen_clip5);
 					a.score = r.score;
 					if (a.score == prev || r.max_off < (aw0 >> 1) + (aw0 >> 2)) break;
 				}
@@ -292,7 +297,9 @@
 					int prev = a.score;
 					aw1 = P.w << i;
 					int wc = aw1 < bound3[qlen] ? aw1 : bound3[qlen];
-					r = extend(qlen, [&](int j) { return q[qe + j]; }, tlen, [&](int t) { return TB(s.rbeg + s.len + t); }, wc, sc0, P.pen_clip3);
+					const QBase qf{q + qe, 1};
+					r = st_w ? extend(qlen, qf, tlen, WinBase{winl + (int)re, 1}, wc, sc0, P.pen_clip3)
+					         : extend(qlen, qf, tlen, PacBase{pac, l_pac, s.rbeg + s.len, 1}, wc, sc0, P.pen_clip3);
 					a.score = r.score;
 					if (a.score == prev || r.max_off < (aw1 >> 1) + (aw1 >> 2)) break;
 				}
@@ -319,10 +326,10 @@
 		if (unit_mode) { if (nav) atomicAdd(&n_regs[rd], nav); }
 		else n_regs[rd] = nav;
 		unsigned long long *st = counters + (size_t)(blockIdx.x % C2A_STAT_SLOTS) * 8;
-		if (cells) atomicAdd(&st[0], cells);
-		if (n_ext) atomicAdd(&st[1], n_ext);
-		if (n_closed) atomicAdd(&st[2], n_closed);
-		if (n_diff) atomicAdd(&st[3], n_diff);
+		if (cells) atomicAdd(&st[0], (unsigned long long)cells);
+		if (n_ext) atomicAdd(&st[1], (unsigned long long)n_ext);
+		if (n_closed) atomicAdd(&st[2], (unsigned long long)n_closed);
+		if (n_diff) atomicAdd(&st[3], (unsigned long long)n_diff);
 	}
 }
 
@@ -333,9 +340,7 @@
 {
 	C2aUnits U;
 	if (units) U = *units;
-	WxParams X;
-	for (int i = 0; i < 25; ++i) X.mat[i] = ep.mat[i];
-	X.o_del = ep.o_del; X.e_del = ep.e_del; X.o_ins = ep.o_ins; X.e_ins = ep.e_ins; X.zdrop = ep.zdrop;
+	const WxParams X = wx_params(ep);
 	size_t shmem = (size_t)C2A_WAVES * c2a_lds_bytes(max_len);
 	if (shmem > 64 * 1024 && hipFuncSetAttribute((const void *)c2a_kernel, hipFuncAttributeMaxDynamicSharedMemorySize, (int)shmem) != hipSuccess)
 		die("c2a_kernel: cannot reserve %zu bytes of LDS", shmem);
diff --git a/mpibwa_amd/csrc/device.h b/mpibwa_amd/csrc/device.h
--- a/mpibwa_amd/csrc/device.h
+++ b/mpibwa_amd/csrc/device.h
@@ -91,6 +91,9 @@
 void launch_extend(void *stream, const ExtParams &ep, int n, const uint8_t *d_q, const int64_t *d_qoff,
                    const uint8_t *d_t, const int64_t *d_toff, const int *d_w, const int *d_h0, const int *d_eb,
                    int *d_out6, unsigned long long *d_cells, int max_qlen);
+void launch_extend2(void *stream, const ExtParams &ep, int n, const uint8_t *d_q, const int64_t *d_qoff,
+                    const uint8_t *d_t, const int64_t *d_toff, const int *d_w, const int *d_h0, const int *d_early, const int *d_clip,
+                    int *d_out6, unsigned long long *d_cells, int max_qlen);
 
 struct DevSeed { int64_t rbeg; int32_t qbeg, len; };
 struct DevChain {
diff --git a/mpibwa_amd/csrc/device.hip b/mpibwa_amd/csrc/device.hip
--- a/mpibwa_amd/csrc/device.hip
+++ b/mpibwa_amd/csrc/device.hip
@@ -903,6 +903,52 @@
 	(void)hipFree(d_h0); (void)hipFree(d_out); (void)hipFree(d_cells);
 	if (kernel_ms) *kernel_ms = ms;
 	if (cells) *cells = c;
+	return 0;
+}
+
+extern "C" int mi355x_extend_batch2(const mem_opt_t *opt, int n, const uint8_t *q, const int64_t *qoff, const uint8_t *t,
+                                    const int64_t *toff, const int *w, const int *h0, const int *end_bonus, const int *early,
+                                    const int *clip, int *out6, uint64_t *cells, double *kernel_ms)
+{
+	int nd = 0;
+	if (hipGetDeviceCount(&nd) != hipSuccess || nd == 0) die("no HIP device visible (no CPU fallback)");
+	if (n <= 0) return 0;
+	hipStream_t st = 0;
+	std::vector<int> wc(n);
+	int max_qlen = 0;
+	for (int i = 0; i < n; ++i) {
+		int ql = (int)(qoff[i + 1] - qoff[i]);
+		max_qlen = std::max(max_qlen, ql);
+		wc[i] = clamp_band(opt, ql, w[i], end_bonus[i]);
+	}
+	uint8_t *d_q, *d_t; int64_t *d_qo, *d_to; int *d_w, *d_h0, *d_early, *d_clip, *d_out; unsigned long long *d_cells;
+	HIP_OK(hipMalloc(&d_q, qoff[n] + 16)); HIP_OK(hipMalloc(&d_t, toff[n] + 16));
+	HIP_OK(hipMalloc(&d_qo, (size_t)(n + 1) * 8)); HIP_OK(hipMalloc(&d_to, (size_t)(n + 1) * 8));
+	HIP_OK(hipMalloc(&d_w, (size_t)n * 4)); HIP_OK(hipMalloc(&d_h0, (size_t)n * 4));
+	HIP_OK(hipMalloc(&d_early, (size_t)n * 4)); HIP_OK(hipMalloc(&d_clip, (size_t)n * 4));
+	HIP_OK(hipMalloc(&d_out, (size_t)n * 24)); HIP_OK(hipMalloc(&d_cells, (size_t)n * 8));
+	HIP_OK(hipMemcpy(d_q, q, qoff[n], hipMemcpyHostToDevice));
+	HIP_OK(hipMemcpy(d_t, t, toff[n], hipMemcpyHostToDevice));
+	HIP_OK(hipMemcpy(d_qo, qoff, (size_t)(n + 1) * 8, hipMemcpyHostToDevice));
+	HIP_OK(hipMemcpy(d_to, toff, (size_t)(n + 1) * 8, hipMemcpyHostToDevice));
+	HIP_OK(hipMemcpy(d_w, wc.data(), (size_t)n * 4, hipMemcpyHostToDevice));
+	HIP_OK(hipMemcpy(d_h0, h0, (size_t)n * 4, hipMemcpyHostToDevice));
+	HIP_OK(hipMemcpy(d_early, early, (size_t)n * 4, hipMemcpyHostToDevice));
+	HIP_OK(hipMemcpy(d_clip, clip, (size_t)n * 4, hipMemcpyHostToDevice));
+	HIP_OK(hipMemset(d_cells, 0, (size_t)n * 8));
+	ExtParams ep;
+	memcpy(ep.mat, opt->mat, 25);
+	ep.o_del = opt->o_del; ep.e_del = opt->e_del; ep.o_ins = opt->o_ins; ep.e_ins = opt->e_ins; ep.zdrop = opt->zdrop;
+	Timer tm;
+	tm.start(st);
+	launch_extend2(st, ep, n, d_q, d_qo, d_t, d_to, d_w, d_h0, d_early, d_clip, d_out, d_cells, max_qlen);
+	double ms = tm.stop(st);
+	HIP_OK(hipGetLastError());
+	HIP_OK(hipMemcpy(cells, d_cells, (size_t)n * 8, hipMemcpyDeviceToHost));
+	HIP_OK(hipMemcpy(out6, d_out, (size_t)n * 24, hipMemcpyDeviceToHost));
+	(void)hipFree(d_q); (void)hipFree(d_t); (void)hipFree(d_qo); (void)hipFree(d_to); (void)hipFree(d_w);
+	(void)hipFree(d_h0); (void)hipFree(d_early); (void)hipFree(d_clip); (void)hipFree(d_out); (void)hipFree(d_cells);
+	if (kernel_ms) *kernel_ms = ms;
 	return 0;
 }
 
diff --git a/mpibwa_amd/csrc/ext_kernels.hip b/mpibwa_amd/csrc/ext_kernels.hip
--- a/mpibwa_amd/csrc/ext_kernels.hip
+++ b/mpibwa_amd/csrc/ext_kernels.hip
@@ -19,15 +19,51 @@
 	const uint8_t *qs = q + qoff[job];
 	const uint8_t *ts = t + toff[job];
 	const int qlen = (int)(qoff[job + 1] - qoff[job]), tlen = (int)(toff[job + 1] - toff[job]);
-	unsigned long long cells = 0;
 	for (int j = lane; j < qlen; j += 64) L.Qs[j] = qs[j];
 	__builtin_amdgcn_wave_barrier();
-	WxResult r = wave_extend(qlen, tlen, [&](int i) { return ts[i]; }, P, w[job], h0[job], L, cells);
+	WxResult r = wave_extend(qlen, tlen, [&](int i) { return ts[i]; }, P, w[job], h0[job], L);
 	if (lane == 0) {
 		int *o = out6 + (size_t)job * 6;
 		o[0] = r.score; o[1] = r.qle; o[2] = r.tle; o[3] = r.gtle; o[4] = r.gscore; o[5] = r.max_off;
-		atomicAdd(cells_total, cells);
+		atomicAdd(cells_total, (unsigned long long)r.cells);
 	}
+}
+
+__global__ void __launch_bounds__(64 * EXT_WAVES)
+extend2_kernel(WxParams P, int n, const uint8_t *__restrict__ q, const int64_t *__restrict__ qoff,
+               const uint8_t *__restrict__ t, const int64_t *__restrict__ toff, const int *__restrict__ w,
+               const int *__restrict__ h0, const int *__restrict__ early, const int *__restrict__ clip,
+               int *__restrict__ out6, unsigned long long *__restrict__ cells_out, int max_qlen)
+{
+	extern __shared__ int lds[];
+	const int wave = threadIdx.x >> 6, lane = threadIdx.x & 63;
+	const int job = blockIdx.x * EXT_WAVES + wave;
+	if (job >= n) return;
+	const WxLds L = wx_lds(lds + (size_t)wave * wx_lds_ints(max_qlen), max_qlen);
+	const uint8_t *qs = q + qoff[job];
+	const uint8_t *ts = t + toff[job];
+	const int qlen = (int)(qoff[job + 1] - qoff[job]), tlen = (int)(toff[job + 1] - toff[job]);
+	for (int j = lane; j < qlen; j += 64) L.Qs[j] = qs[j];
+	__builtin_amdgcn_wave_barrier();
+	auto tf = [&](int i) { return ts[i]; };
+	const WxResult r = __builtin_amdgcn_readfirstlane(early[job]) ? wave_extend<true>(qlen, tlen, tf, P, w[job], h0[job], L, clip[job])
+	                                                              : wave_extend<false>(qlen, tlen, tf, P, w[job], h0[job], L);
+	if (lane == 0) {
+		int *o = out6 + (size_t)job * 6;
+		o[0] = r.score; o[1] = r.qle; o[2] = r.tle; o[3] = r.gtle; o[4] = r.gscore; o[5] = r.max_off;
+		cells_out[job] = r.cells;
+	}
+}
+
+void launch_extend2(void *stream, const ExtParams &ep, int n, const uint8_t *d_q, const int64_t *d_qoff,
+                    const uint8_t *d_t, const int64_t *d_toff, const int *d_w, const int *d_h0, const int *d_early, const int *d_clip,
+                    int *d_out6, unsigned long long *d_cells, int max_qlen)
+{
+	const WxParams P = wx_params(ep);
+	size_t shmem = (size_t)EXT_WAVES * wx_lds_ints(max_qlen) * sizeof(int);
+	int n_blocks = (n + EXT_WAVES - 1) / EXT_WAVES;
+	hipLaunchKernelGGL(extend2_kernel, dim3(n_blocks), dim3(64 * EXT_WAVES), shmem, (hipStream_t)stream, P, n, d_q, d_qoff,
+	                   d_t, d_toff, d_w, d_h0, d_early, d_clip, d_out6, d_cells, max_qlen);
 }
 
 void launch_extend(void *stream, const ExtParams &ep, int n, const uint8_t *d_q, const int64_t *d_qoff,
@@ -35,9 +71,7 @@
                    int *d_out6, unsigned long long *d_cells, int max_qlen)
 {
 	(void)d_eb;
-	WxParams P;
-	for (int i = 0; i < 25; ++i) P.mat[i] = ep.mat[i];
-	P.o_del = ep.o_del; P.e_del = ep.e_del; P.o_ins = ep.o_ins; P.e_ins = ep.e_ins; P.zdrop = ep.zdrop;
+	const WxParams P = wx_params(ep);
 	size_t shmem = (size_t)EXT_WAVES * wx_lds_ints(max_qlen) * sizeof(int);
 	int n_blocks = (n + EXT_WAVES - 1) / EXT_WAVES;
 	hipLaunchKernelGGL(extend_kernel, dim3(n_blocks), dim3(64 * EXT_WAVES), shmem, (hipStream_t)stream, P, n, d_q, d_qoff,
diff --git a/mpibwa_amd/csrc/wave_ext.cuh b/mpibwa_amd/csrc/wave_ext.cuh
--- a/mpibwa_amd/csrc/wave_ext.cuh
+++ b/mpibwa_amd/csrc/wave_ext.cuh
@@ -30,6 +30,12 @@
 	asm("s_min_i32 %0, %1, %2" : "=s"(r) : "s"(a), "s"(b) : "scc");
 	return r;
 }
+__device__ __forceinline__ int wx_smax(int a, int b)
+{
+	int r;
+	asm("s_max_i32 %0, %1, %2" : "=s"(r) : "s"(a), "s"(b) : "scc");
+	return r;
+}
 __device__ __forceinline__ int wx_prev_lane(int v, int first)
 {
 	return wx_dpp<0x138, 0xf>(first, v);
@@ -38,9 +44,34 @@
 struct WxParams {
 	int8_t mat[25];
 	int o_del, e_del, o_ins, e_ins, zdrop;
+	uint32_t plo[5], phi[5];
+	int max_sc;
+	int zdrop_t;
+	int plain, sc_a, sc_b, g1;
 };
-
-struct WxResult { int score, qle, tle, gtle, gscore, max_off; };
+template <typename EP>
+inline WxParams wx_params(const EP &ep)
+{
+	WxParams X;
+	for (int i = 0; i < 25; ++i) X.mat[i] = ep.mat[i];
+	X.o_del = ep.o_del; X.e_del = ep.e_del; X.o_ins = ep.o_ins; X.e_ins = ep.e_ins; X.zdrop = ep.zdrop;
+	X.max_sc = 1;
+	for (int i = 0; i < 25; ++i) X.max_sc = ep.mat[i] > X.max_sc ? ep.mat[i] : X.max_sc;
+	for (int t = 0; t < 5; ++t) {
+		X.plo[t] = (uint32_t)(uint8_t)ep.mat[t * 5] | (uint32_t)(uint8_t)ep.mat[t * 5 + 1] << 8 | (uint32_t)(uint8_t)ep.mat[t * 5 + 2] << 16 |
+		           (uint32_t)(uint8_t)ep.mat[t * 5 + 3] << 24;
+		X.phi[t] = (uint32_t)(uint8_t)ep.mat[t * 5 + 4];
+	}
+	X.zdrop_t = ep.zdrop > 0 ? ep.zdrop : 0x7ffffffe;
+	X.sc_a = ep.mat[0]; X.sc_b = -ep.mat[1];
+	X.plain = X.sc_a > 0 && X.sc_b > 0;
+	for (int i = 0; i < 4; ++i)
+		for (int j = 0; j < 4; ++j) X.plain = X.plain && ep.mat[i * 5 + j] == (i == j ? X.sc_a : -X.sc_b);
+	X.g1 = (ep.o_del < ep.o_ins ? ep.o_del : ep.o_ins) + (ep.e_del < ep.e_ins ? ep.e_del : ep.e_ins);
+	return X;
+}
+
+struct WxResult { int score, qle, tle, gtle, gscore, max_off; unsigned int cells; };
 
 struct WxLds { int2 *HE; uint8_t *Qs; int2 *dummy; };
 __host__ __device__ inline int wx_lds_ints(int max_qlen) { return 2 * (max_qlen + 2 + 64) + (((max_qlen + 64 + 7) & ~7) >> 2) + 2; }
@@ -54,8 +85,7 @@
 }
 
 template <bool EARLY = false, typename TF>
-__device__ __forceinline__ WxResult wave_extend(int qlen, int tlen, TF tf, const WxParams &P, int w, int h0, const WxLds &L,
-                                                unsigned long long &cells, int max_sc = 1, int clip = 0x3fffffff)
+__device__ __forceinline__ WxResult wave_extend(int qlen, int tlen, TF tf, const WxParams &P, int w, int h0, const WxLds &L, int clip = 0x3fffffff)
 {
 	const int lane = threadIdx.x & 63;
 	int2 *const HE = L.HE;
@@ -64,8 +94,8 @@
 	tlen = __builtin_amdgcn_readfirstlane(tlen);
 	w = __builtin_amdgcn_readfirstlane(w);
 	h0 = __builtin_amdgcn_readfirstlane(h0);
-	max_sc = __builtin_amdgcn_readfirstlane(max_sc);
 	clip = __builtin_amdgcn_readfirstlane(clip);
+	const int max_sc = P.max_sc, zdrop_t = P.zdrop_t;
 	const int oe_del = P.o_del + P.e_del, oe_ins = P.o_ins + P.e_ins, e_del = P.e_del, e_ins = P.e_ins;
 	int lane_e = lane * e_ins;
 	asm volatile("" : "+v"(lane_e));
@@ -83,107 +113,127 @@
 	__builtin_amdgcn_wave_barrier();
 	int best = h0, best_i = -1, best_j = -1, best_ie = -1, gscore = -1, max_off = 0;
 	int beg = 0, end = qlen;
-	int tv_base = -64;
+	int hl = h0 - P.o_del;
+	unsigned int n_cells = 0;
 	int vslo = 0, vshi = 0;
-	uint32_t plo[5], phi[5];
-#pragma unroll
-	for (int t = 0; t < 5; ++t) {
-		plo[t] = (uint32_t)(uint8_t)P.mat[t * 5] | (uint32_t)(uint8_t)P.mat[t * 5 + 1] << 8 | (uint32_t)(uint8_t)P.mat[t * 5 + 2] << 16 |
-		         (uint32_t)(uint8_t)P.mat[t * 5 + 3] << 24;
-		phi[t] = (uint32_t)(uint8_t)P.mat[t * 5 + 4];
-	}
-	for (int i = 0; i < tlen; ++i) {
-		if (i - tv_base >= 64) {
-			tv_base = i;
-			const int tb = (i + lane < tlen) ? (int)tf(i + lane) : 4;
-			vslo = (int)(tb == 0 ? plo[0] : tb == 1 ? plo[1] : tb == 2 ? plo[2] : tb == 3 ? plo[3] : plo[4]);
-			vshi = (int)(tb == 0 ? phi[0] : tb == 1 ? phi[1] : tb == 2 ? phi[2] : tb == 3 ? phi[3] : phi[4]);
-		}
-		const uint32_t slo = (uint32_t)__builtin_amdgcn_readlane(vslo, i - tv_base), shi = (uint32_t)__builtin_amdgcn_readlane(vshi, i - tv_base);
-		if (beg < i - w) beg = i - w;
-		end = wx_smin(wx_smin(end, i + w + 1), qlen);
-		int hleft0 = 0;
-		if (beg == 0) { hleft0 = h0 - (P.o_del + e_del * (i + 1)); if (hleft0 < 0) hleft0 = 0; }
+	const uint32_t pl0 = P.plo[0], pl1 = P.plo[1], pl2 = P.plo[2], pl3 = P.plo[3], pl4 = P.plo[4];
+	const uint32_t ph0 = P.phi[0], ph1 = P.phi[1], ph2 = P.phi[2], ph3 = P.phi[3], ph4 = P.phi[4];
+	for (int i = 0; tlen > 0; ++i) {
+		if ((i & 63) == 0) {
+			const int ti = i + lane;
+			int tb = (int)tf(ti < tlen ? ti : tlen - 1);
+			tb = ti < tlen ? tb : 4;
+			const uint32_t m0 = -(uint32_t)(tb == 0), m1 = -(uint32_t)(tb == 1), m2 = -(uint32_t)(tb == 2), m3 = -(uint32_t)(tb == 3), m4 = -(uint32_t)(tb == 4);
+			vslo = (int)((pl0 & m0) | (pl1 & m1) | (pl2 & m2) | (pl3 & m3) | (pl4 & m4));
+			vshi = (int)((ph0 & m0) | (ph1 & m1) | (ph2 & m2) | (ph3 & m3) | (ph4 & m4));
+		}
+		const uint32_t slo = (uint32_t)__builtin_amdgcn_readlane(vslo, i & 63), shi = (uint32_t)__builtin_amdgcn_readlane(vshi, i & 63);
+		beg = wx_smax(beg, i - w);
+		end = wx_smin(end, i + w + 1);
+		hl -= e_del;
+		const int hleft0 = wx_smax(beg == 0 ? hl : 0, 0);
 		const int n_col = end - beg;
-		int lanekey = -1;
-		int A = beg * e_ins;
-		int h_carry = hleft0, h_cin = hleft0;
-		int h_strip = 0;
-		int first_nz = end, last_nz = -1;
-		const int jb = beg + lane;
-		int je = lane_e + beg * e_ins;
-		for (int s0 = 0; s0 <= n_col; s0 += 64, je += 64 * e_ins) {
-			const int j = jb + s0;
-			const bool act = j < end, wr = j <= end;
+		int rowkey, h_last, nb, ne;
+		const int nc = wx_smax(n_col, 0), jfin = wx_smax(beg, end);
+		if (__builtin_expect(n_col < 64, 1)) {
+			const int j = wx_smin(beg, end) + lane;
+			const bool act = lane < nc, wr = lane <= nc;
 			const int2 he = HE[j];
 			const int diag = he.x, e = he.y;
 			const int sc = (int)(int8_t)__builtin_amdgcn_perm(shi, slo, (uint32_t)Qs[j] | 0x0c0c0c00u);
 			const int M = (act && diag) ? diag + sc : 0;
 			int tI = M - oe_ins; tI = tI > 0 ? tI : 0;
-			const int g = tI + je;
-			const int incl = wx_scan_max(g);
+			const int incl = wx_scan_max(tI + lane_e);
 			const int excl = wx_prev_lane(incl, WX_NEG);
-			const int f = max(A, excl + e_ins) - je;
+			const int f = max(excl + e_ins, 0) - lane_e;
 			const int h = act ? max(max(M, e), f) : 0;
 			int tD = M - oe_del; tD = tD > 0 ? tD : 0;
 			const int en = act ? max(e - e_del, tD) : 0;
-			const int h_prev = wx_prev_lane(h, h_carry);
+			const int h_prev = wx_prev_lane(h, hleft0);
 			*(wr ? HE + j : L.dummy) = make_int2(h_prev, en);
-			A = max(A, __builtin_amdgcn_readlane(incl, 63) + e_ins);
-			lanekey = max(lanekey, h << 13 | j);
 			const unsigned long long nz = __builtin_amdgcn_ballot_w64((h_prev | en) != 0);
-			if (nz) {
-				const int lo = beg + s0 + __ffsll((long long)nz) - 1, hi = beg + s0 + 63 - __clzll(nz);
-				if (lo < end && lo < first_nz) first_nz = lo;
-				if (hi > last_nz) last_nz = hi;
+			nb = beg + __builtin_ctzll(nz | 1ull << nc);
+			ne = wx_smax(beg + 63 - __builtin_clzll(nz | 1ull), nb - 1);
+			rowkey = __builtin_amdgcn_readlane(wx_scan_max(h << 13 | j), 63);
+			h_last = __builtin_amdgcn_readlane(h_prev, nc);
+		} else {
+			int lanekey = -1;
+			int A = beg * e_ins;
+			int h_carry = hleft0, h_cin = hleft0;
+			int h_strip = 0;
+			int first_nz = end, last_nz = -1;
+			const int jb = beg + lane;
+			int je = lane_e + beg * e_ins;
+			for (int s0 = 0; s0 <= n_col; s0 += 64, je += 64 * e_ins) {
+				const int j = jb + s0;
+				const bool act = j < end, wr = j <= end;
+				const int2 he = HE[j];
+				const int diag = he.x, e = he.y;
+				const int sc = (int)(int8_t)__builtin_amdgcn_perm(shi, slo, (uint32_t)Qs[j] | 0x0c0c0c00u);
+				const int M = (act && diag) ? diag + sc : 0;
+				int tI = M - oe_ins; tI = tI > 0 ? tI : 0;
+				const int g = tI + je;
+				const int incl = wx_scan_max(g);
+				const int excl = wx_prev_lane(incl, WX_NEG);
+				const int f = max(A, excl + e_ins) - je;
+				const int h = act ? max(max(M, e), f) : 0;
+				int tD = M - oe_del; tD = tD > 0 ? tD : 0;
+				const int en = act ? max(e - e_del, tD) : 0;
+				const int h_prev = wx_prev_lane(h, h_carry);
+				*(wr ? HE + j : L.dummy) = make_int2(h_prev, en);
+				A = max(A, __builtin_amdgcn_readlane(incl, 63) + e_ins);
+				lanekey = max(lanekey, h << 13 | j);
+				const unsigned long long nz = __builtin_amdgcn_ballot_w64((h_prev | en) != 0);
+				if (nz) {
+					const int lo = beg + s0 + __ffsll((long long)nz) - 1, hi = beg + s0 + 63 - __clzll(nz);
+					if (lo < end && lo < first_nz) first_nz = lo;
+					if (hi > last_nz) last_nz = hi;
+				}
+				h_cin = h_carry;
+				h_carry = __builtin_amdgcn_readlane(h, 63);
+				h_strip = h;
 			}
-			h_cin = h_carry;
-			h_carry = __builtin_amdgcn_readlane(h, 63);
-			h_strip = h;
-		}
-		const int h_last = (n_col > 0 && (n_col & 63)) ? __builtin_amdgcn_readlane(h_strip, (n_col - 1) & 63) : n_col > 0 ? h_cin : hleft0;
-		int rowkey = -1;
-		if (n_col > 0) {
+			h_last = (n_col & 63) ? __builtin_amdgcn_readlane(h_strip, (n_col - 1) & 63) : h_cin;
 			rowkey = __builtin_amdgcn_readlane(wx_scan_max(lanekey), 63);
-			cells += (unsigned long long)n_col;
-		} else if (n_col < 0) {
-			if (lane == 0) HE[end] = make_int2(hleft0, 0);
-		}
+			nb = first_nz;
+			ne = last_nz >= nb ? last_nz : nb - 1;
+		}
+		n_cells += (unsigned int)nc;
 		__builtin_amdgcn_wave_barrier();
-		const int jfin = n_col > 0 ? end : beg;
-		if (jfin == qlen) {
-			if (h_last >= gscore) best_ie = i;
-			if (h_last > gscore) gscore = h_last;
-		}
-		const int rowmax = rowkey < 0 ? 0 : rowkey >> 13, rowmax_j = rowkey < 0 ? -1 : rowkey & 8191;
-		if (rowmax == 0) break;
-		if (rowmax > best) {
-			best = rowmax; best_i = i; best_j = rowmax_j;
-			int d = rowmax_j - i; d = d < 0 ? -d : d;
-			if (d > max_off) max_off = d;
-		} else if (P.zdrop > 0) {
-			int di = i - best_i, dj = rowmax_j - best_j;
-			if (di > dj) { if (best - rowmax - (di - dj) * e_del > P.zdrop) break; }
-			else { if (best - rowmax - (dj - di) * e_ins > P.zdrop) break; }
-		}
-		const int nb = first_nz;
-		const int ne = last_nz >= nb ? last_nz : nb - 1;
+		const int h_end = jfin == qlen ? h_last : -2;
+		best_ie = h_end >= gscore ? i : best_ie;
+		gscore = wx_smax(gscore, h_end);
+		const int rowmax = rowkey >> 13, rowmax_j = rowkey & 8191;
+		const bool up = rowmax > best;
+		int d = rowmax_j - i; d = d < 0 ? -d : d;
+		best_i = up ? i : best_i;
+		best_j = up ? rowmax_j : best_j;
+		max_off = wx_smax(max_off, up ? d : 0);
+		best = wx_smax(best, rowmax);
+		const int dd = (i - best_i) - (rowmax_j - best_j);
+		const int pen = (dd < 0 ? -dd : dd) * (dd > 0 ? e_del : e_ins);
+		int drop = rowmax == 0 ? 0x7fffffff : best - rowmax - pen;
 		beg = nb;
-		end = ne + 2 < qlen ? ne + 2 : qlen;
-		if (EARLY && (i & 3) == 3 && (gscore >= 0 || rowmax + (qlen - 1 - rowmax_j) * max_sc <= best - clip)) {
-			int b = WX_NEG;
-			for (int j = lane; j <= qlen; j += 64) {
-				const int2 he = HE[j];
-				const int hv = j < qlen ? he.x + (qlen - j) * max_sc : WX_NEG;
-				const int ev = he.y + (qlen - 1 - j) * max_sc;
-				b = max(b, max(hv, ev));
+		end = wx_smin(ne + 2, qlen);
+		if (EARLY && (i & 3) == 3) {
+			if (gscore >= 0 || rowmax + (qlen - 1 - rowmax_j) * max_sc <= best - clip) {
+				int b = WX_NEG;
+				for (int j = lane; j <= qlen; j += 64) {
+					const int2 he = HE[j];
+					const int hv = j < qlen ? he.x + (qlen - j) * max_sc : WX_NEG;
+					const int ev = he.y + (qlen - 1 - j) * max_sc;
+					b = max(b, max(hv, ev));
+				}
+				b = __builtin_amdgcn_readlane(wx_scan_max(b), 63);
+				if ((gscore >= 0 && b < gscore && b <= best)
+				    || (b <= best - clip && gscore <= best - clip))
+					drop = 0x7fffffff;
 			}
-			b = __builtin_amdgcn_readlane(wx_scan_max(b), 63);
-			if (gscore >= 0 && b < gscore && b <= best) break;
-			if (b <= best - clip && gscore <= best - clip) break;
-		}
+		}
+		if ((i + 1 >= tlen ? 0x7fffffff : drop) > zdrop_t) break;
 	}
 	WxResult r;
+	r.cells = n_cells;
 	r.score = best; r.qle = best_j + 1; r.tle = best_i + 1; r.gtle = best_ie + 1; r.gscore = gscore; r.max_off = max_off;
 	return r;
 }
```

Result: faster. 6.840, median of 6 (+4.7%).
